# wang-xinyu/tensorrtx

Hardware: NVIDIA B200
Metric: end_to_end_fps_yolov8n_640_b32 (pre-process + fused decode + NMS); decode+NMS us/frame alongside (higher is better)
Workload: dtype f32

## Files before the change

include/trtx_hot.h:

```cpp
#ifndef TRTX_HOT_H
#define TRTX_HOT_H

#include <stddef.h>
#include <stdint.h>

#ifdef __cplusplus
extern "C" {
#endif

#if defined(_WIN32)
#define TRTX_API __declspec(dllexport)
#else
#define TRTX_API __attribute__((visibility("default")))
#endif

typedef void* trtx_stream_t;

enum {
    TRTX_OK = 0,
    TRTX_ERR_INVALID = 1,
    TRTX_ERR_WORKSPACE = 2,
    TRTX_ERR_CUDA = 3,
    TRTX_ERR_UNSUPPORTED = 4,
};

#define TRTX_MAX_LEVELS 8

TRTX_API const char* trtx_version(void);
TRTX_API int trtx_last_cuda_error(void);
TRTX_API size_t trtx_abi_sizeof(int which);

enum {
    TRTX_YOLO_V8 = 0,
    TRTX_YOLO_V5 = 1,
    TRTX_YOLO_V3 = 2,
    TRTX_YOLO_V26 = 3,
};
enum { TRTX_F32 = 0, TRTX_F16 = 1 };

typedef struct trtx_yolo_params {
    int32_t variant;
    int32_t num_classes;
    int32_t net_w;
    int32_t net_h;
    int32_t max_out;
    int32_t det_floats;
    int32_t num_levels;
    int32_t grid_h[TRTX_MAX_LEVELS];
    int32_t grid_w[TRTX_MAX_LEVELS];
    int32_t strides[TRTX_MAX_LEVELS];
    float anchors[TRTX_MAX_LEVELS][6];
    int32_t is_seg;
    int32_t is_pose;
    int32_t is_obb;
    int32_t num_kpts;
    float kpt_thresh;
    float gate;
    int32_t in_dtype;
    int32_t tune_class_slices;
    int32_t tune_rows_in_flight;
    int32_t tune_tma_pipeline;
    int32_t tune_tma_stages;
    int32_t tune_box_prefetch;
} trtx_yolo_params;

TRTX_API int trtx_yolo_params_init_v8(trtx_yolo_params* p, int num_classes, int net_w, int net_h, int max_out,
                                      const int* strides, int num_levels);

TRTX_API size_t trtx_yolo_workspace_size(const trtx_yolo_params* p, int batch);

TRTX_API int trtx_yolo_decode_enqueue(const trtx_yolo_params* p, int batch, const void* const* inputs_dev,
                                      float* output_dev, void* workspace_dev, size_t workspace_bytes,
                                      trtx_stream_t stream);

enum {
    TRTX_BOX_LTRB = 0,
    TRTX_BOX_CXCYWH = 1,
    TRTX_BOX_RETINA = 2,
    TRTX_BOX_OBB = 3,
};
enum {
    TRTX_NMS_GREEDY = 0,
    TRTX_NMS_ONESHOT = 1,
};

#define TRTX_NMS_MAX_ROWS 2048

typedef struct trtx_nms_params {
    int32_t box_format;
    int32_t mode;
    float conf_thresh;
    float nms_thresh;
    int32_t max_det;
    int32_t class_aware;
    int32_t tie_break_x0;
    int32_t extra_floats;
    int32_t extra_offset;
} trtx_nms_params;


TRTX_API size_t trtx_nms_workspace_size(const trtx_nms_params* p, int batch, int max_rows);
TRTX_API int trtx_nms_enqueue(const trtx_nms_params* p, int batch, const float* plugin_out_dev, int max_rows,
                              int det_floats, float* compact_out_dev, int32_t* keep_index_dev, void* workspace_dev,
                              size_t workspace_bytes, trtx_stream_t stream);

TRTX_API int trtx_yolo_decode_nms_enqueue(const trtx_yolo_params* p, const trtx_nms_params* q, int batch,
                                          const void* const* inputs_dev, float* compact_out_dev,
                                          int32_t* keep_index_dev, void* workspace_dev, size_t workspace_bytes,
                                          trtx_stream_t stream);

TRTX_API int trtx_yolo_scan_enqueue(const trtx_yolo_params* p, int batch, const void* const* inputs_dev,
                                    void* workspace_dev, size_t workspace_bytes, trtx_stream_t stream);
TRTX_API int trtx_yolo_nms_after_scan_enqueue(const trtx_yolo_params* p, const trtx_nms_params* q, int batch,
                                              const void* const* inputs_dev, float* compact_out_dev,
                                              int32_t* keep_index_dev, void* workspace_dev, size_t workspace_bytes,
                                              trtx_stream_t stream);

typedef struct trtx_gather {
    int32_t world, rank, slots, slot;
    float* out_dev[8];
    uint32_t* flags_dev[8];
    uint32_t* ctrl_dev;
} trtx_gather;
TRTX_API int trtx_yolo_decode_nms_gather_enqueue(const trtx_yolo_params* p, const trtx_nms_params* q, int batch,
                                                 const void* const* inputs_dev, float* compact_out_dev,
                                                 int32_t* keep_index_dev, void* workspace_dev, size_t workspace_bytes,
                                                 const trtx_gather* gather, trtx_stream_t stream);
TRTX_API int trtx_gather_push_enqueue(const trtx_gather* gather, const float* compact_out_dev, int batch, int max_det,
                                      int extra_floats, trtx_stream_t stream);
TRTX_API int trtx_gather_wait_enqueue(const trtx_gather* gather, trtx_stream_t stream);
TRTX_API int trtx_gather_push_many_enqueue(const trtx_gather* gather, const float* const* compact_outs_dev, int n, int batch,
                                           int max_det, int extra_floats, trtx_stream_t stream);
TRTX_API int trtx_gather_wait_many_enqueue(const trtx_gather* gather, int nslots, trtx_stream_t stream);
TRTX_API int trtx_peer_alloc(size_t bytes, void** dev_ptr, unsigned char handle[64]);
TRTX_API int trtx_peer_open(const unsigned char handle[64], void** dev_ptr);
TRTX_API int trtx_peer_close(void* dev_ptr);
TRTX_API int trtx_peer_free(void* dev_ptr);

enum {
    TRTX_RETINA_FACE = 0,
    TRTX_RETINA_ANTICOV = 1,
};
typedef struct trtx_retina_params {
    int32_t in_h, in_w;
    float gate;
    int32_t variant;
} trtx_retina_params;

TRTX_API int trtx_retina_total_priors(const trtx_retina_params* p);
TRTX_API size_t trtx_retina_workspace_size(const trtx_retina_params* p, int batch);
TRTX_API int trtx_retina_decode_enqueue(const trtx_retina_params* p, int batch, const void* const* inputs_dev,
                                        float* output_dev, void* workspace_dev, size_t workspace_bytes,
                                        trtx_stream_t stream);

TRTX_API int64_t trtx_rpn_decode(int batch, const float* scores_dev, const float* deltas_dev, float* out_scores_dev,
                                 float* out_boxes_dev, int height, int width, int image_height, int image_width,
                                 float stride, const float* anchors_host, int num_anchors, int top_n,
                                 void* workspace_dev, size_t workspace_bytes, trtx_stream_t stream);
TRTX_API int64_t trtx_rpn_nms(int batch, const float* scores_dev, const float* boxes_dev, float* out_boxes_dev,
                              int pre_nms_topk, int post_nms_topk, float nms_thresh, void* workspace_dev,
                              size_t workspace_bytes, trtx_stream_t stream);
TRTX_API int64_t trtx_predictor_decode(int batch, const float* scores_dev, const float* deltas_dev,
                                       const float* proposals_dev, float* out_scores_dev, float* out_boxes_dev,
                                       float* out_classes_dev, int num_boxes, int num_classes, int image_height,
                                       int image_width, const float* bbox_reg_weights_host, void* workspace_dev,
                                       size_t workspace_bytes, trtx_stream_t stream);
TRTX_API int64_t trtx_batched_nms(int nms_method, int batch, const float* scores_dev, const float* boxes_dev,
                                  const float* classes_dev, float* out_scores_dev, float* out_boxes_dev,
                                  float* out_classes_dev, int count, int detections_per_im, float nms_thresh,
                                  void* workspace_dev, size_t workspace_bytes, trtx_stream_t stream);

typedef struct trtx_image_desc {
    const uint8_t* data_dev;
    int32_t width, height;
    int32_t pitch;
    int32_t reserved;
} trtx_image_desc;

TRTX_API int trtx_preprocess_batch_enqueue(const trtx_image_desc* images_host, int batch, void* dst_dev, int dst_w,
                                           int dst_h, int out_dtype, trtx_stream_t stream);
TRTX_API void trtx_letterbox_matrix(int src_w, int src_h, int dst_w, int dst_h, float d2s[6]);
TRTX_API int trtx_get_rect(int variant, int net_w, int net_h, int img_w, int img_h, const float bbox[4], int rect[4]);

TRTX_API int trtx_get_rect_adapt_landmark(int net_w, int net_h, int img_w, int img_h, const float bbox[4], float* lmk,
                                          int num_kpts, int rect[4]);
TRTX_API int trtx_retina_get_rect_adapt_landmark(int input_w, int input_h, int img_w, int img_h, const float bbox[4], float lmk[10],
                                                 int rect[4]);
TRTX_API int trtx_process_decode_ptr_host(const float* decode_ptr_host, int bbox_element, int count, float* rows_out);
TRTX_API int trtx_process_decode_ptr_host_obb(const float* decode_ptr_host, int bbox_element, int count, float* rows_out);
TRTX_API int trtx_scale_mask_rect(int net_w, int net_h, int img_w, int img_h, int rect[4]);
TRTX_API int trtx_scale_mask_enqueue(const float* masks_dev, int n, int net_w, int net_h, int img_w, int img_h, float* out_dev,
                                     trtx_stream_t stream);

TRTX_API int trtx_roi_align(int batch, const float* rois_dev, const float* features_dev, float* out_dev, int pooler_resolution,
                            float spatial_scale, int sampling_ratio, int num_proposals, int out_channels, int feature_h,
                            int feature_w, trtx_stream_t stream);
#define TRTX_ROI_WINDOW 0
#define TRTX_ROI_DIRECT 1
TRTX_API int trtx_roi_align_ex(int batch, const float* rois_dev, const float* features_dev, float* out_dev, int pooler_resolution,
                               float spatial_scale, int sampling_ratio, int num_proposals, int out_channels, int feature_h,
                               int feature_w, int mode, trtx_stream_t stream);
TRTX_API int trtx_mask_rcnn_inference(int batch, const float* indices_dev, const float* masks_dev, float* out_dev,
                                      int detections_per_im, int output_size, int num_classes, trtx_stream_t stream);

TRTX_API int trtx_calib_letterbox_rect(int src_w, int src_h, int net_w, int net_h, int rect[4]);
TRTX_API int trtx_calib_letterbox_host(const uint8_t* bgr, int src_w, int src_h, size_t src_pitch, int net_w, int net_h, float* out_chw);

typedef struct trtx_mask_params {
    int32_t variant;
    int32_t net_w, net_h;
    int32_t mask_w, mask_h;
    int32_t num_coeffs;
    int32_t row_floats;
    int32_t coeff_offset;
    int32_t max_masks;
} trtx_mask_params;

TRTX_API int trtx_process_mask_enqueue(const trtx_mask_params* p, int batch, const float* proto_dev, const float* dets_dev,
                                       int max_rows, float* masks_dev, trtx_stream_t stream);

#ifdef __cplusplus
}
#endif
#endif
```

tensorrtx_b200/_lib.py:

```python
from __future__ import annotations

import ctypes as C
import os
from pathlib import Path

MAX_LEVELS = 8

OK, ERR_INVALID, ERR_WORKSPACE, ERR_CUDA, ERR_UNSUPPORTED = range(5)
YOLO_V8, YOLO_V5, YOLO_V3, YOLO_V26 = 0, 1, 2, 3
F32, F16 = 0, 1
BOX_LTRB, BOX_CXCYWH, BOX_RETINA, BOX_OBB = 0, 1, 2, 3
NMS_GREEDY, NMS_ONESHOT = 0, 1
ROI_WINDOW, ROI_DIRECT = 0, 1
RETINA_FACE, RETINA_ANTICOV = 0, 1

_ERR = {1: "TRTX_ERR_INVALID", 2: "TRTX_ERR_WORKSPACE", 3: "TRTX_ERR_CUDA", 4: "TRTX_ERR_UNSUPPORTED"}


class TrtxError(RuntimeError):
    pass


class YoloParams(C.Structure):
    _fields_ = [
        ("variant", C.c_int32),
        ("num_classes", C.c_int32),
        ("net_w", C.c_int32),
        ("net_h", C.c_int32),
        ("max_out", C.c_int32),
        ("det_floats", C.c_int32),
        ("num_levels", C.c_int32),
        ("grid_h", C.c_int32 * MAX_LEVELS),
        ("grid_w", C.c_int32 * MAX_LEVELS),
        ("strides", C.c_int32 * MAX_LEVELS),
        ("anchors", (C.c_float * 6) * MAX_LEVELS),
        ("is_seg", C.c_int32),
        ("is_pose", C.c_int32),
        ("is_obb", C.c_int32),
        ("num_kpts", C.c_int32),
        ("kpt_thresh", C.c_float),
        ("gate", C.c_float),
        ("in_dtype", C.c_int32),
        ("tune_class_slices", C.c_int32),
        ("tune_rows_in_flight", C.c_int32),
        ("tune_tma_pipeline", C.c_int32),
        ("tune_tma_stages", C.c_int32),
        ("tune_box_prefetch", C.c_int32),
    ]


class NmsParams(C.Structure):
    _fields_ = [
        ("box_format", C.c_int32),
        ("mode", C.c_int32),
        ("conf_thresh", C.c_float),
        ("nms_thresh", C.c_float),
        ("max_det", C.c_int32),
        ("class_aware", C.c_int32),
        ("tie_break_x0", C.c_int32),
        ("extra_floats", C.c_int32),
        ("extra_offset", C.c_int32),
    ]


class Gather(C.Structure):
    _fields_ = [("world", C.c_int32), ("rank", C.c_int32), ("slots", C.c_int32), ("slot", C.c_int32),
                ("out_dev", C.c_void_p * 8), ("flags_dev", C.c_void_p * 8), ("ctrl_dev", C.c_void_p)]


class RetinaParams(C.Structure):
    _fields_ = [("in_h", C.c_int32), ("in_w", C.c_int32), ("gate", C.c_float), ("variant", C.c_int32)]


class ImageDesc(C.Structure):
    _fields_ = [
        ("data_dev", C.c_void_p),
        ("width", C.c_int32),
        ("height", C.c_int32),
        ("pitch", C.c_int32),
        ("reserved", C.c_int32),
    ]


class MaskParams(C.Structure):
    _fields_ = [(n, C.c_int32) for n in ("variant", "net_w", "net_h", "mask_w", "mask_h", "num_coeffs", "row_floats",
                                         "coeff_offset", "max_masks")]


LIB_PATH = Path(os.environ.get("TRTX_LIB") or Path(__file__).resolve().parent / "lib" / "libtrtx_hot.so")

_vp, _sz, _i, _f = C.c_void_p, C.c_size_t, C.c_int, C.c_float
_pp = C.POINTER(C.c_void_p)
SYMBOLS = {
    "trtx_version": (C.c_char_p, []),
    "trtx_last_cuda_error": (_i, []),
    "trtx_yolo_params_init_v8": (_i, [C.POINTER(YoloParams), _i, _i, _i, _i, C.POINTER(C.c_int), _i]),
    "trtx_yolo_workspace_size": (_sz, [C.POINTER(YoloParams), _i]),
    "trtx_yolo_decode_enqueue": (_i, [C.POINTER(YoloParams), _i, _pp, _vp, _vp, _sz, _vp]),
    "trtx_nms_workspace_size": (_sz, [C.POINTER(NmsParams), _i, _i]),
    "trtx_nms_enqueue": (_i, [C.POINTER(NmsParams), _i, _vp, _i, _i, _vp, _vp, _vp, _sz, _vp]),
    "trtx_yolo_decode_nms_enqueue": (_i, [C.POINTER(YoloParams), C.POINTER(NmsParams), _i, _pp, _vp, _vp, _vp, _sz, _vp]),
    "trtx_yolo_scan_enqueue": (_i, [C.POINTER(YoloParams), _i, _pp, _vp, _sz, _vp]),
    "trtx_yolo_nms_after_scan_enqueue": (_i, [C.POINTER(YoloParams), C.POINTER(NmsParams), _i, _pp, _vp, _vp, _vp, _sz, _vp]),
    "trtx_retina_total_priors": (_i, [C.POINTER(RetinaParams)]),
    "trtx_retina_workspace_size": (_sz, [C.POINTER(RetinaParams), _i]),
    "trtx_retina_decode_enqueue": (_i, [C.POINTER(RetinaParams), _i, _pp, _vp, _vp, _sz, _vp]),
    "trtx_rpn_decode": (C.c_int64, [_i, _vp, _vp, _vp, _vp, _i, _i, _i, _i, _f, C.POINTER(C.c_float), _i, _i, _vp, _sz, _vp]),
    "trtx_rpn_nms": (C.c_int64, [_i, _vp, _vp, _vp, _i, _i, _f, _vp, _sz, _vp]),
    "trtx_predictor_decode": (C.c_int64, [_i, _vp, _vp, _vp, _vp, _vp, _vp, _i, _i, _i, _i, C.POINTER(C.c_float), _vp, _sz, _vp]),
    "trtx_batched_nms": (C.c_int64, [_i, _i, _vp, _vp, _vp, _vp, _vp, _vp, _i, _i, _f, _vp, _sz, _vp]),
    "trtx_preprocess_batch_enqueue": (_i, [C.POINTER(ImageDesc), _i, _vp, _i, _i, _i, _vp]),
    "trtx_get_rect": (_i, [_i, _i, _i, _i, _i, C.POINTER(C.c_float), C.POINTER(C.c_int)]),
    "trtx_roi_align": (_i, [_i, _vp, _vp, _vp, _i, C.c_float, _i, _i, _i, _i, _i, _vp]),
    "trtx_calib_letterbox_rect": (_i, [_i, _i, _i, _i, C.POINTER(C.c_int)]),
    "trtx_calib_letterbox_host": (_i, [_vp, _i, _i, C.c_size_t, _i, _i, _vp]),
    "trtx_roi_align_ex": (_i, [_i, _vp, _vp, _vp, _i, C.c_float, _i, _i, _i, _i, _i, _i, _vp]),
    "trtx_mask_rcnn_inference": (_i, [_i, _vp, _vp, _vp, _i, _i, _i, _vp]),
    "trtx_process_mask_enqueue": (_i, [C.POINTER(MaskParams), _i, _vp, _vp, _i, _vp, _vp]),
    "trtx_letterbox_matrix": (None, [_i, _i, _i, _i, C.POINTER(C.c_float)]),
    "trtx_abi_sizeof": (_sz, [_i]),
    "trtx_get_rect_adapt_landmark": (_i, [_i, _i, _i, _i, C.POINTER(C.c_float), C.POINTER(C.c_float), _i, C.POINTER(C.c_int)]),
    "trtx_retina_get_rect_adapt_landmark": (_i, [_i, _i, _i, _i, C.POINTER(C.c_float), C.POINTER(C.c_float), C.POINTER(C.c_int)]),
    "trtx_process_decode_ptr_host": (_i, [C.POINTER(C.c_float), _i, _i, C.POINTER(C.c_float)]),
    "trtx_process_decode_ptr_host_obb": (_i, [C.POINTER(C.c_float), _i, _i, C.POINTER(C.c_float)]),
    "trtx_scale_mask_rect": (_i, [_i, _i, _i, _i, C.POINTER(C.c_int)]),
    "trtx_scale_mask_enqueue": (_i, [_vp, _i, _i, _i, _i, _i, _vp, _vp]),
    "trtx_yolo_decode_nms_gather_enqueue": (_i, [C.POINTER(YoloParams), C.POINTER(NmsParams), _i, _pp, _vp, _vp, _vp, _sz,
                                                 C.POINTER(Gather), _vp]),
    "trtx_gather_wait_enqueue": (_i, [C.POINTER(Gather), _vp]),
    "trtx_gather_push_enqueue": (_i, [C.POINTER(Gather), _vp, _i, _i, _i, _vp]),
    "trtx_gather_push_many_enqueue": (_i, [C.POINTER(Gather), _pp, _i, _i, _i, _i, _vp]),
    "trtx_gather_wait_many_enqueue": (_i, [C.POINTER(Gather), _i, _vp]),
    "trtx_peer_alloc": (_i, [_sz, C.POINTER(C.c_void_p), C.POINTER(C.c_ubyte)]),
    "trtx_peer_open": (_i, [C.POINTER(C.c_ubyte), C.POINTER(C.c_void_p)]),
    "trtx_peer_close": (_i, [_vp]),
    "trtx_peer_free": (_i, [_vp]),
}

_lib = None


def load() -> C.CDLL:
    global _lib
    if _lib is not None:
        return _lib
    if not LIB_PATH.exists():
        raise TrtxError(
            f"{LIB_PATH} is missing: build it with `python -m tensorrtx_b200.build` "
            "(or __graft_entry__.build()). There is no CPU/PyTorch fallback for this path."
        )
    lib = C.CDLL(str(LIB_PATH))
    for name, (res, args) in SYMBOLS.items():
        fn = getattr(lib, name)
        fn.restype = res
        fn.argtypes = args
    for which, st in enumerate((YoloParams, NmsParams, RetinaParams, ImageDesc, MaskParams)):
        if lib.trtx_abi_sizeof(which) != C.sizeof(st):
            raise TrtxError(f"{LIB_PATH} was built from a different trtx_hot.h: sizeof({st.__name__}) = "
                            f"{lib.trtx_abi_sizeof(which)} in the library, {C.sizeof(st)} in the binding (rebuild)")
    _lib = lib
    return lib


def check(rc: int, what: str) -> None:
    if rc != 0:
        extra = ""
        if rc == ERR_CUDA:
            extra = f" (cudaError {load().trtx_last_cuda_error()})"
        raise TrtxError(f"{what} failed: {_ERR.get(rc, rc)}{extra}")


def ptr_array(ptrs) -> "C.Array":
    arr = (C.c_void_p * len(ptrs))()
    for i, p in enumerate(ptrs):
        arr[i] = p
    return arr
```

tensorrtx_b200/csrc/common.cuh:

```cuda
#pragma once
#include <cuda_fp16.h>
#include <cuda_runtime.h>
#include <stdint.h>

#include "trtx_hot.h"

namespace trtx {

constexpr int kWarp = 32;
constexpr size_t kAlign = 256;

__host__ __device__ inline size_t align_up(size_t v, size_t a = kAlign) { return (v + a - 1) / a * a; }

extern thread_local int g_last_cuda_error;
inline int check_launch() {
    cudaError_t e = cudaGetLastError();
    if (e != cudaSuccess) {
        g_last_cuda_error = (int)e;
        return TRTX_ERR_CUDA;
    }
    return TRTX_OK;
}

__device__ __forceinline__ float4 ldg_stream_f4(const float* p) {
    float4 r;
    asm volatile("ld.global.nc.L1::no_allocate.v4.f32 {%0,%1,%2,%3}, [%4];"
                 : "=f"(r.x), "=f"(r.y), "=f"(r.z), "=f"(r.w)
                 : "l"(p));
    return r;
}
__device__ __forceinline__ float ldg_stream_f1(const float* p) {
    float r;
    asm volatile("ld.global.nc.L1::no_allocate.f32 %0, [%1];" : "=f"(r) : "l"(p));
    return r;
}
__device__ __forceinline__ float4 ldg_stream_h4(const __half* p) {
    uint32_t a, b;
    asm volatile("ld.global.nc.L1::no_allocate.v2.u32 {%0,%1}, [%2];" : "=r"(a), "=r"(b) : "l"(p));
    __half2 h0 = *reinterpret_cast<__half2*>(&a);
    __half2 h1 = *reinterpret_cast<__half2*>(&b);
    float2 f0 = __half22float2(h0), f1 = __half22float2(h1);
    return make_float4(f0.x, f0.y, f1.x, f1.y);
}
__device__ __forceinline__ uint4 ldg_stream_h8(const __half* p) {
    uint4 r;
    asm volatile("ld.global.nc.L1::no_allocate.v4.u32 {%0,%1,%2,%3}, [%4];" : "=r"(r.x), "=r"(r.y), "=r"(r.z), "=r"(r.w) : "l"(p));
    return r;
}
__device__ __forceinline__ float ldg_stream_h1(const __half* p) {
    unsigned short r;
    asm volatile("ld.global.nc.L1::no_allocate.u16 %0, [%1];" : "=h"(r) : "l"(p));
    return __half2float(__ushort_as_half(r));
}

template <typename T>
struct Elem;
template <>
struct Elem<float> {
    static __device__ __forceinline__ float4 ld4(const float* p) { return ldg_stream_f4(p); }
    static __device__ __forceinline__ float ld1(const float* p) { return ldg_stream_f1(p); }
    static __device__ __forceinline__ float ld1_cached(const float* p) { return __ldg(p); }
};
template <>
struct Elem<__half> {
    static __device__ __forceinline__ float4 ld4(const __half* p) { return ldg_stream_h4(p); }
    static __device__ __forceinline__ float ld1(const __half* p) { return ldg_stream_h1(p); }
    static __device__ __forceinline__ float ld1_cached(const __half* p) { return __half2float(__ldg(p)); }
};

__device__ __forceinline__ float logist(float x) { return 1.0f / (1.0f + expf(-x)); }

__device__ __forceinline__ uint32_t float_key(float f) {
    uint32_t b = __float_as_uint(f);
    return (b & 0x80000000u) ? ~b : (b | 0x80000000u);
}

__device__ __forceinline__ int warp_excl_scan(int v, int lane, int* total) {
    int x = v;
#pragma unroll
    for (int d = 1; d < 32; d <<= 1) {
        int y = __shfl_up_sync(0xffffffffu, x, d);
        if (lane >= d) x += y;
    }
    *total = __shfl_sync(0xffffffffu, x, 31);
    return x - v;
}

}
```

tensorrtx_b200/csrc/nms.cu:

```cuda
#include <string.h>

#include "yolo_layout.cuh"

namespace trtx {

#ifdef TRTX_NMS_PROBE
static thread_local long long* t_nms_stamps = nullptr;
#define TRTX_STAMP(k) do { if (a.dbg && threadIdx.x == 0) a.dbg[blockIdx.x * 16 + (k)] = clock64(); } while (0)
#else
#define TRTX_STAMP(k) do { } while (0)
#endif

constexpr int kNmsThreads = 1024;
constexpr int kMaxSort = TRTX_NMS_MAX_ROWS;
constexpr int kClassBins = kNmsThreads;
constexpr int kMaxBucket = 256;
constexpr int kShortSeg = 96;

struct NmsArgs {
    const float* rows;
    int max_rows;
    int det_floats;
    int from_tiles;
    int tiles_per_image, slots_per_image, tile_slots;
    int num_levels;
    int lv_tile_begin[TRTX_MAX_LEVELS];
    int lv_slot_begin[TRTX_MAX_LEVELS];
    const int* tile_count;
    const float4* cand;
    uint2* list;
    int list_stride;
    int box_format, mode, class_aware, tie_break_x0;
    float conf_thresh, nms_thresh;
    int pre_topk;
    int max_det;
    int extra_floats, extra_offset;
#ifdef TRTX_NMS_PROBE
    long long* dbg;
#endif
    float* out;
    int32_t* keep_index;
    struct Gather {
        float* out[8];
        unsigned* flags[8];
        unsigned* ctrl;
        int world, rank, slots, slot;
    } g;
};

__device__ __forceinline__ unsigned ld_relaxed_sys(const unsigned* p) {
    unsigned v;
    asm volatile("ld.relaxed.sys.global.u32 %0, [%1];" : "=r"(v) : "l"(p) : "memory");
    return v;
}
__device__ __forceinline__ void st_relaxed_sys(unsigned* p, unsigned v) {
    asm volatile("st.relaxed.sys.global.u32 [%0], %1;" ::"l"(p), "r"(v) : "memory");
}

__device__ __forceinline__ float iou_oneshot(const float4 a, const float4 b) {
    float cl = fmaxf(a.x, b.x), ct = fmaxf(a.y, b.y), cr = fminf(a.z, b.z), cb = fminf(a.w, b.w);
    float c_area = __fmul_rn(fmaxf(__fsub_rn(cr, cl), 0.0f), fmaxf(__fsub_rn(cb, ct), 0.0f));
    if (c_area == 0.0f) return 0.0f;
    float a_area = __fmul_rn(fmaxf(0.0f, __fsub_rn(a.z, a.x)), fmaxf(0.0f, __fsub_rn(a.w, a.y)));
    float b_area = __fmul_rn(fmaxf(0.0f, __fsub_rn(b.z, b.x)), fmaxf(0.0f, __fsub_rn(b.w, b.y)));
    return __fdiv_rn(c_area, __fsub_rn(__fadd_rn(a_area, b_area), c_area));
}
__device__ __forceinline__ void obb_cov_host(float w, float h, float r, float& a, float& b, float& c) {
    const float A = (float)((double)__fmul_rn(w, w) / 12.0), B = (float)((double)__fmul_rn(h, h) / 12.0);
    const float cr = cosf(r), sr = sinf(r);
    const float cr2 = __fmul_rn(cr, cr), sr2 = __fmul_rn(sr, sr);
    a = __fadd_rn(__fmul_rn(A, cr2), __fmul_rn(B, sr2));
    b = __fadd_rn(__fmul_rn(A, sr2), __fmul_rn(B, cr2));
    c = __fmul_rn(__fmul_rn(__fsub_rn(A, B), cr), sr);
}
__device__ __forceinline__ float obb_probiou_host(const float4 p1, float c1, const float4 p2, float c2) {
    const float eps = 1e-7;
    const float x1 = p1.x, y1 = p1.y, a1 = p1.z, b1 = p1.w, x2 = p2.x, y2 = p2.y, a2 = p2.z, b2 = p2.w;
    const float sa = __fadd_rn(a1, a2), sb = __fadd_rn(b1, b2), sc = __fadd_rn(c1, c2);
    const double dy = (double)__fsub_rn(y1, y2), dx = (double)__fsub_rn(x1, x2), dc = (double)sc;
    const double py = __dmul_rn(dy, dy), px = __dmul_rn(dx, dx), pc = __dmul_rn(dc, dc);
    const double den = __dadd_rn(__dsub_rn((double)__fmul_rn(sa, sb), pc), (double)eps);
    const float t1 = (float)__ddiv_rn(__dadd_rn(__dmul_rn((double)sa, py), __dmul_rn((double)sb, px)), den);
    const float t2 = (float)__ddiv_rn((double)__fmul_rn(__fmul_rn(sc, __fsub_rn(x2, x1)), __fsub_rn(y1, y2)), den);
    const float s1 = sqrtf(fmaxf(__fsub_rn(__fmul_rn(a1, b1), __fmul_rn(c1, c1)), 0.0f));
    const float s2 = sqrtf(fmaxf(__fsub_rn(__fmul_rn(a2, b2), __fmul_rn(c2, c2)), 0.0f));
    const float d3 = __fadd_rn(__fmul_rn(__fmul_rn(4.0f, s1), s2), eps);
    const float t3 = (float)log(__dadd_rn(__ddiv_rn(__dsub_rn((double)__fmul_rn(sa, sb), pc), (double)d3), (double)eps));
    float bd = __fadd_rn(__fadd_rn(__fmul_rn(0.25f, t1), __fmul_rn(0.5f, t2)), __fmul_rn(0.5f, t3));
    bd = fmaxf(fminf(bd, 100.0f), eps);
    const float hd = (float)sqrt(__dadd_rn(__dsub_rn(1.0, (double)expf(-bd)), (double)eps));
    return __fsub_rn(1.0f, hd);
}
__device__ __forceinline__ void obb_cov_dev(float w, float h, float r, float& a, float& b, float& c) {
    float a_val = w * w / 12.0f;
    float b_val = h * h / 12.0f;
    float cos_r = cosf(r);
    float sin_r = sinf(r);
    a = a_val * cos_r * cos_r + b_val * sin_r * sin_r;
    b = a_val * sin_r * sin_r + b_val * cos_r * cos_r;
    c = (a_val - b_val) * sin_r * cos_r;
}
__device__ __forceinline__ float obb_probiou_dev(const float4 p1, float c1, const float4 p2, float c2) {
    const float eps = 1e-7;
    const float cx1 = p1.x, cy1 = p1.y, a1 = p1.z, b1 = p1.w, cx2 = p2.x, cy2 = p2.y, a2 = p2.z, b2 = p2.w;
    float t1 = ((a1 + a2) * powf(cy1 - cy2, 2) + (b1 + b2) * powf(cx1 - cx2, 2)) /
               ((a1 + a2) * (b1 + b2) - powf(c1 + c2, 2) + eps);
    float t2 = ((c1 + c2) * (cx2 - cx1) * (cy1 - cy2)) / ((a1 + a2) * (b1 + b2) - powf(c1 + c2, 2) + eps);
    float t3 = logf(((a1 + a2) * (b1 + b2) - powf(c1 + c2, 2)) /
                            (4 * sqrtf(fmaxf(a1 * b1 - c1 * c1, 0.0f)) * sqrtf(fmaxf(a2 * b2 - c2 * c2, 0.0f)) + eps) +
                    eps);
    float bd = 0.25f * t1 + 0.5f * t2 + 0.5f * t3;
    bd = fmaxf(fminf(bd, 100.0f), eps);
    float hd = sqrtf(1.0f - expf(-bd) + eps);
    return 1 - hd;
}

__device__ __forceinline__ float4 to_corners(int fmt, const float4 b) {
    if (fmt != TRTX_BOX_CXCYWH) return b;
    const float hw = __fmul_rn(b.z, 0.5f), hh = __fmul_rn(b.w, 0.5f);
    return make_float4(__fsub_rn(b.x, hw), __fsub_rn(b.y, hh), __fadd_rn(b.x, hw), __fadd_rn(b.y, hh));
}
__device__ __forceinline__ float box_area(int fmt, const float4 b) {
    if (fmt == TRTX_BOX_CXCYWH) return __fmul_rn(b.z, b.w);
    return __fmul_rn(__fsub_rn(b.z, b.x), __fsub_rn(b.w, b.y));
}
struct IouTest {
    float thr;
    bool obb;
    bool retina;
    bool zero_hit;
    bool fast_ok;
};
__device__ __forceinline__ bool overlaps(const IouTest& q, const float4 l, float la, const float4 r, float ra) {
    if (q.obb) return obb_probiou_host(l, la, r, ra) >= q.thr;
    const float ib0 = l.x < r.x ? r.x : l.x;
    const float ib1 = r.z < l.z ? r.z : l.z;
    const float ib2 = l.y < r.y ? r.y : l.y;
    const float ib3 = r.w < l.w ? r.w : l.w;
    if (ib2 > ib3 || ib0 > ib1) return q.zero_hit;
    const float inter = __fmul_rn(__fsub_rn(ib1, ib0), __fsub_rn(ib3, ib2));
    float denom = __fsub_rn(__fadd_rn(la, ra), inter);
    if (q.retina) denom = __fadd_rn(denom, 0.000001f);
    const float t = __fmaf_rn(-q.thr, denom, inter);
    if (q.fast_ok && denom > 0.0f && fabsf(t) > __fmul_rn(1e-5f, denom)) return t > 0.0f;
    return __fdiv_rn(inter, denom) > q.thr;
}

struct Row {
    float4 box;
    float conf;
    float cls;
    int anchor;
};
__device__ __forceinline__ Row fetch_row(const NmsArgs& a, int b, uint32_t id) {
    Row r;
    if (a.from_tiles) {
        const float4* c = a.cand + 2 * ((size_t)b * a.slots_per_image + id);
        r.box = c[0];
        float4 m = c[1];
        r.conf = m.x;
        r.cls = m.y;
        r.anchor = __float_as_int(m.z);
    } else {
        const float* p = a.rows + (size_t)b * (1 + (size_t)a.max_rows * a.det_floats) + 1 + (size_t)id * a.det_floats;
        r.box = make_float4(p[0], p[1], p[2], p[3]);
        r.conf = p[4];
        r.cls = a.box_format == TRTX_BOX_RETINA ? 0.0f : p[5];
        r.anchor = (int)id;
    }
    return r;
}

__device__ __forceinline__ void pick_bucket(const int* hist, bool descending, int* need_io, int* bucket_out) {
    int need = *need_io, c = 0, d;
    if (descending) {
        for (d = 255; d > 0; --d) {
            if (c + hist[d] >= need) break;
            c += hist[d];
        }
    } else {
        for (d = 0; d < 255; ++d) {
            if (c + hist[d] >= need) break;
            c += hist[d];
        }
    }
    *need_io = need - c;
    *bucket_out = d;
}

__device__ __forceinline__ int seg_units(int m) {
    const int G = (m + 6) >> 3;
    return G * (m - 1) - 4 * G * (G - 1);
}

__global__ void __launch_bounds__(kNmsThreads, 1) nms_kernel(const __grid_constant__ NmsArgs a) {
    extern __shared__ __align__(16) unsigned char smem_raw[];
    const int S = a.pre_topk <= 1024 ? 1024 : kMaxSort;
    float4* u_box = reinterpret_cast<float4*>(smem_raw);
    float4* s_box = u_box + S;
    unsigned long long* k64 = reinterpret_cast<unsigned long long*>(s_box + S);
    float* u_conf = reinterpret_cast<float*>(k64 + S);
    int* u_cls = reinterpret_cast<int*>(u_conf + S);
    uint32_t* u_id = reinterpret_cast<uint32_t*>(u_cls + S);
    float* s_conf = reinterpret_cast<float*>(u_id + S);
    int* s_cls = reinterpret_cast<int*>(s_conf + S);
    uint32_t* s_id = reinterpret_cast<uint32_t*>(s_cls + S);
    int* s_seg = reinterpret_cast<int*>(s_id + S);
    int* s_long = s_seg + S;
    unsigned short* s_pos = reinterpret_cast<unsigned short*>(s_long + S / 2);
    unsigned char* s_keep = reinterpret_cast<unsigned char*>(s_pos + S);
    unsigned short* s_unit = reinterpret_cast<unsigned short*>(s_keep + S);
    float* s_area = reinterpret_cast<float*>(s_unit + S * (kShortSeg / 8));
    int* s_tpre = reinterpret_cast<int*>(s_area + S);
    unsigned short* s_krow = reinterpret_cast<unsigned short*>(u_box);
    unsigned* s_mask = reinterpret_cast<unsigned*>(u_conf);
    int* s_rowseg = reinterpret_cast<int*>(k64);
    unsigned long long* k_hi = reinterpret_cast<unsigned long long*>(s_box);
    unsigned long long* k_lo = k_hi + S;

    __shared__ int s_hist[256];
    __shared__ int s_chist[kClassBins], s_cstart[kClassBins];
    __shared__ int s_n, s_need, s_bucket, s_nkept, s_nshort, s_nmed, s_nlong, s_cursor, s_bad, s_nunit;
    __shared__ unsigned s_rem;
    __shared__ unsigned s_sup[32];
    __shared__ int s_wsum[32];

    const int b = blockIdx.x;
    const int tid = threadIdx.x, lane = tid & 31, warp = tid >> 5;
    uint2* list = a.list + (size_t)b * a.list_stride;

    TRTX_STAMP(0);
    if (tid == 0) {
        s_n = 0;
        s_bad = 0;
    }
    auto stash = [&](const Row& r, uint32_t id) {
        const int pos = atomicAdd(&s_n, 1);
        list[pos] = make_uint2(float_key(r.conf), id);
        if (pos < S) {
            const int c = a.class_aware ? (int)r.cls : 0;
            u_box[pos] = r.box;
            u_conf[pos] = r.conf;
            u_cls[pos] = c;
            u_id[pos] = id;
            if (c < 0 || c > 0xffff) s_bad = 1;
        }
    };
    if (a.from_tiles) {
        const int T = a.tiles_per_image;
        const int* cnt = a.tile_count + (size_t)b * T;
        int carry = 0;
        for (int base = 0; base < T; base += kNmsThreads) {
            const int t = base + tid;
            const int v = t < T ? cnt[t] : 0;
            int tot;
            const int ex = warp_excl_scan(v, lane, &tot);
            if (lane == 0) s_wsum[warp] = tot;
            __syncthreads();
            if (warp == 0) {
                int w = s_wsum[lane], wt;
                const int wex = warp_excl_scan(w, lane, &wt);
                s_wsum[lane] = wex;
                if (lane == 0) s_need = wt;
            }
            __syncthreads();
            if (t < T) s_tpre[t] = carry + s_wsum[warp] + ex;
            carry += s_need;
            __syncthreads();
        }
        if (tid == 0) s_tpre[T] = carry;
        __syncthreads();
        const int n_in = min(carry, a.pre_topk);
        for (int r = tid; r < n_in; r += kNmsThreads) {
            int lo = 0, hi = T;
            while (hi - lo > 1) {
                const int mid = (lo + hi) >> 1;
                if (s_tpre[mid] <= r) lo = mid; else hi = mid;
            }
            const int t = lo;
            int l = 0;
            while (l + 1 < a.num_levels && t >= a.lv_tile_begin[l + 1]) ++l;
            const uint32_t id = a.lv_slot_begin[l] + (uint32_t)(t - a.lv_tile_begin[l]) * a.tile_slots + (uint32_t)(r - s_tpre[t]);
            const Row row = fetch_row(a, b, id);
            if (a.mode == TRTX_NMS_ONESHOT ? row.conf >= a.conf_thresh : row.conf > a.conf_thresh) stash(row, id);
        }
    } else {
        __syncthreads();
        const float* img = a.rows + (size_t)b * (1 + (size_t)a.max_rows * a.det_floats);
        int n_in = (int)img[0];
        n_in = max(0, min(n_in, a.max_rows));
        for (int i = tid; i < n_in; i += kNmsThreads) {
            const Row row = fetch_row(a, b, (uint32_t)i);
            if (a.mode == TRTX_NMS_ONESHOT ? row.conf >= a.conf_thresh : row.conf > a.conf_thresh) stash(row, (uint32_t)i);
        }
    }
    __syncthreads();
    const int n_valid = s_n;
    const int M = min(n_valid, a.pre_topk);

    if (n_valid > a.pre_topk) {
        uint32_t key_cut = 0, id_cut = 0xffffffffu;
        uint32_t prefix = 0, mask = 0;
        if (tid == 0) s_need = a.pre_topk;
        for (int pass = 0; pass < 4; ++pass) {
            const int shift = 24 - 8 * pass;
            if (tid < 256) s_hist[tid] = 0;
            __syncthreads();
            for (int i = tid; i < n_valid; i += kNmsThreads) {
                uint32_t k = list[i].x;
                if ((k & mask) == prefix) atomicAdd(&s_hist[(k >> shift) & 255], 1);
            }
            __syncthreads();
            if (tid == 0) {
                int need = s_need, d;
                pick_bucket(s_hist, true, &need, &d);
                s_need = need;
                s_bucket = d;
            }
            __syncthreads();
            prefix |= (uint32_t)s_bucket << shift;
            mask |= 255u << shift;
        }
        key_cut = prefix;
        const int need_eq = s_need;
        uint32_t ip = 0, im = 0;
        __syncthreads();
        if (tid == 0) s_need = need_eq;
        for (int pass = 0; pass < 4; ++pass) {
            const int shift = 24 - 8 * pass;
            if (tid < 256) s_hist[tid] = 0;
            __syncthreads();
            for (int i = tid; i < n_valid; i += kNmsThreads) {
                uint2 e = list[i];
                if (e.x == key_cut && (e.y & im) == ip) atomicAdd(&s_hist[(e.y >> shift) & 255], 1);
            }
            __syncthreads();
            if (tid == 0) {
                int need = s_need, d;
                pick_bucket(s_hist, false, &need, &d);
                s_need = need;
                s_bucket = d;
            }
            __syncthreads();
            ip |= (uint32_t)s_bucket << shift;
            im |= 255u << shift;
        }
        id_cut = ip;
        if (tid == 0) {
            s_n = 0;
            s_bad = 0;
        }
        __syncthreads();
        for (int i = tid; i < n_valid; i += kNmsThreads) {
            const uint2 e = list[i];
            if (e.x > key_cut || (e.x == key_cut && e.y <= id_cut)) {
                const Row r = fetch_row(a, b, e.y);
                const int pos = atomicAdd(&s_n, 1);
                const int c = a.class_aware ? (int)r.cls : 0;
                u_box[pos] = r.box;
                u_conf[pos] = r.conf;
                u_cls[pos] = c;
                u_id[pos] = e.y;
                if (c < 0 || c > 0xffff) s_bad = 1;
            }
        }
        __syncthreads();
    }

    TRTX_STAMP(1);
    int S_eff = 32;
    while (S_eff < M) S_eff <<= 1;
    bool generic = s_bad != 0;
    bool bucketed = false;
    if (!generic) {
        unsigned long long* kb = reinterpret_cast<unsigned long long*>(s_box);
        s_chist[tid] = 0;
        __syncthreads();
        bool big = false;
        for (int base = 0; base < M; base += kNmsThreads) {
            const int i = base + tid;
            const int c = i < M ? u_cls[i] : -1;
            const unsigned peers = __match_any_sync(0xffffffffu, c);
            const int leader = __ffs(peers) - 1;
            int first = 0;
            if (c >= kClassBins) big = true;
            if (lane == leader && c >= 0 && c < kClassBins) first = atomicAdd(&s_chist[c], __popc(peers));
            first = __shfl_sync(0xffffffffu, first, leader);
            if (i < M) s_pos[i] = (unsigned short)(first + __popc(peers & ((1u << lane) - 1u)));
        }
        __syncthreads();
        const int h = s_chist[tid];
        int tot;
        const int ex = warp_excl_scan(h, lane, &tot);
        if (lane == 0) s_wsum[warp] = tot;
        if (!__syncthreads_or(big || h > kMaxBucket ? 1 : 0)) {
            if (warp == 0) {
                int w = s_wsum[lane], wt;
                const int wex = warp_excl_scan(w, lane, &wt);
                s_wsum[lane] = wex;
            }
            __syncthreads();
            s_cstart[tid] = s_wsum[warp] + ex;
            __syncthreads();
            for (int i = tid; i < M; i += kNmsThreads) {
                const int c = u_cls[i];
                kb[s_cstart[c] + s_pos[i]] =
                    ((unsigned long long)(uint32_t)c << 48) | ((unsigned long long)(uint32_t)(~float_key(u_conf[i])) << 16) | (uint32_t)i;
            }
            __syncthreads();
            for (int p = tid; p < M; p += kNmsThreads) {
                const unsigned long long mk = kb[p];
                const int c = (int)(mk >> 48);
                const int s0 = s_cstart[c], m = s_chist[c];
                int rank = 0;
#pragma unroll 4
                for (int k = 0; k < m; ++k) rank += kb[s0 + k] < mk ? 1 : 0;
                k64[s0 + rank] = mk;
            }
            __syncthreads();
            bool tie = false;
            for (int i = tid; i < M; i += kNmsThreads)
                if (i > 0 && (k64[i] >> 16) == (k64[i - 1] >> 16)) tie = true;
            generic = __syncthreads_or(tie ? 1 : 0) != 0;
            bucketed = !generic;
        }
    }
    if (!generic && !bucketed) {
        for (int i = tid; i < S_eff; i += kNmsThreads)
            k64[i] = i < M ? ((unsigned long long)(uint32_t)u_cls[i] << 48) | ((unsigned long long)(uint32_t)(~float_key(u_conf[i])) << 16) | (uint32_t)i
                           : ~0ull;
        __syncthreads();
        if (S_eff <= kNmsThreads) {
            unsigned long long* ex = reinterpret_cast<unsigned long long*>(s_box);
            unsigned long long mk = tid < S_eff ? k64[tid] : ~0ull;
            int pp = 0;
            for (int k = 2; k <= S_eff; k <<= 1) {
                for (int jj = k >> 1; jj > 0; jj >>= 1) {
                    unsigned long long ok;
                    if (jj >= 32) {
                        ex[pp * kNmsThreads + tid] = mk;
                        __syncthreads();
                        ok = ex[pp * kNmsThreads + (tid ^ jj)];
                        pp ^= 1;
                    } else {
                        ok = __shfl_xor_sync(0xffffffffu, mk, jj);
                    }
                    const bool want_min = (((tid & k) == 0) == ((tid & jj) == 0));
                    if (want_min == (ok < mk)) mk = ok;
                }
            }
            __syncthreads();
            if (tid < S_eff) k64[tid] = mk;
            __syncthreads();
        } else {
            for (int k = 2; k <= S_eff; k <<= 1) {
                for (int jj = k >> 1; jj > 0; jj >>= 1) {
                    for (int i = tid; i < S_eff; i += kNmsThreads) {
                        const int ixj = i ^ jj;
                        if (ixj > i) {
                            const unsigned long long x = k64[i], y = k64[ixj];
                            if ((x > y) == ((i & k) == 0)) {
                                k64[i] = y;
                                k64[ixj] = x;
                            }
                        }
                    }
                    __syncthreads();
                }
            }
        }
        bool tie = false;
        for (int i = tid; i < M; i += kNmsThreads)
            if (i > 0 && (k64[i] >> 16) == (k64[i - 1] >> 16)) tie = true;
        generic = __syncthreads_or(tie ? 1 : 0) != 0;
    }
    if (generic) {
        for (int i = tid; i < S_eff; i += kNmsThreads) {
            if (i < M) {
                k_hi[i] = ((unsigned long long)(uint32_t)u_cls[i] << 32) | (uint32_t)(~float_key(u_conf[i]));
                k_lo[i] = ((unsigned long long)(a.tie_break_x0 ? float_key(u_box[i].x) : 0u) << 32) | u_id[i];
            } else {
                k_hi[i] = ~0ull;
                k_lo[i] = ~0ull;
            }
            s_pos[i] = (unsigned short)i;
        }
        __syncthreads();
        for (int k = 2; k <= S_eff; k <<= 1) {
            for (int jj = k >> 1; jj > 0; jj >>= 1) {
                for (int i = tid; i < S_eff; i += kNmsThreads) {
                    const int ixj = i ^ jj;
                    if (ixj > i) {
                        const unsigned long long ah = k_hi[i], al = k_lo[i], bh = k_hi[ixj], bl = k_lo[ixj];
                        const bool gt = ah > bh || (ah == bh && al > bl);
                        if (gt == ((i & k) == 0)) {
                            k_hi[i] = bh;
                            k_lo[i] = bl;
                            k_hi[ixj] = ah;
                            k_lo[ixj] = al;
                            const unsigned short t0 = s_pos[i];
                            s_pos[i] = s_pos[ixj];
                            s_pos[ixj] = t0;
                        }
                    }
                }
                __syncthreads();
            }
        }
        for (int i = tid; i < M; i += kNmsThreads) k64[i] = s_pos[i];
        __syncthreads();
    }

    TRTX_STAMP(2);
    const bool greedy = a.mode == TRTX_NMS_GREEDY;
    IouTest iq;
    iq.thr = a.nms_thresh;
    iq.obb = a.box_format == TRTX_BOX_OBB;
    iq.retina = a.box_format == TRTX_BOX_RETINA;
    iq.zero_hit = 0.0f > a.nms_thresh;
    iq.fast_ok = fabsf(a.nms_thresh) <= 4.0f;
    for (int i = tid; i < M; i += kNmsThreads) {
        const int pos = (int)(k64[i] & 0xffffull);
        const float4 bx = u_box[pos];
        if (a.box_format == TRTX_BOX_OBB) {
            const float ang = a.rows[(size_t)b * (1 + (size_t)a.max_rows * a.det_floats) + 1 + (size_t)u_id[pos] * a.det_floats +
                                     a.extra_offset];
            float ca, cb, cc;
            if (greedy)
                obb_cov_host(bx.z, bx.w, ang, ca, cb, cc);
            else
                obb_cov_dev(bx.z, bx.w, ang, ca, cb, cc);
            s_box[i] = make_float4(bx.x, bx.y, ca, cb);
            s_area[i] = cc;
        } else if (greedy) {
            s_box[i] = to_corners(a.box_format, bx);
            s_area[i] = box_area(a.box_format, bx);
        } else {
            s_box[i] = bx;
        }
        s_conf[i] = u_conf[pos];
        s_cls[i] = u_cls[pos];
        s_id[i] = u_id[pos];
        s_keep[i] = 0;
    }
    if (tid == 0) {
        s_nkept = 0;
        s_rem = 0;
        s_nshort = 0;
        s_nmed = 0;
        s_nlong = 0;
        s_cursor = 0;
        s_nunit = 0;
    }
    __syncthreads();
    TRTX_STAMP(8);

    const int R = 7 + a.extra_floats;
    float* o = a.out + (size_t)b * (1 + (size_t)a.max_det * R);
    int32_t* oidx = a.keep_index ? a.keep_index + (size_t)b * a.max_det : nullptr;
    const int gworld = a.g.world;
    const size_t goff = gworld ? ((size_t)a.g.slot * gworld * gridDim.x + (size_t)a.g.rank * gridDim.x + b) * (1 + (size_t)a.max_det * R) : 0;

    if (greedy) {
        if (bucketed) {
            for (int i = tid; i < M; i += kNmsThreads) {
                const int c = s_cls[i], m = s_chist[c];
                s_rowseg[i] = m > kShortSeg ? 0 : ((s_cstart[c] << 16) | m);
            }
            const int m = s_chist[tid], p0 = s_cstart[tid];
            if (m > kShortSeg)
                s_long[atomicAdd(&s_nlong, 1)] = (p0 << 16) | m;
            else if (m > 32)
                s_seg[S - 1 - atomicAdd(&s_nmed, 1)] = (p0 << 16) | m;
            else if (m > 0)
                s_seg[atomicAdd(&s_nshort, 1)] = (p0 << 16) | m;
            if (m > 1 && m <= kShortSeg) s_pos[p0] = (unsigned short)atomicAdd(&s_nunit, seg_units(m));
        } else
        for (int i = tid; i < M; i += kNmsThreads) {
            if (i == 0 || s_cls[i] != s_cls[i - 1]) {
                int e = i + 1;
                while (e < M && s_cls[e] == s_cls[i]) ++e;
                const int m = e - i;
                for (int r = i; r < e; ++r) s_rowseg[r] = m > kShortSeg ? 0 : ((i << 16) | m);
                if (m > kShortSeg)
                    s_long[atomicAdd(&s_nlong, 1)] = (i << 16) | m;
                else if (m > 32)
                    s_seg[S - 1 - atomicAdd(&s_nmed, 1)] = (i << 16) | m;
                else
                    s_seg[atomicAdd(&s_nshort, 1)] = (i << 16) | m;
                if (m > 1 && m <= kShortSeg) s_pos[i] = (unsigned short)atomicAdd(&s_nunit, seg_units(m));
            }
        }
        __syncthreads();
        TRTX_STAMP(3);
        const int n_long = s_nlong;
        for (int ls = 0; ls < n_long; ++ls) {
            const int p0 = s_long[ls] >> 16, m = s_long[ls] & 0xffff;
            int n_kept = 0;
            for (int c0 = 0; c0 < m; c0 += 32) {
                const int nchunk = min(32, m - c0);
                const int P = 32 * n_kept;
                for (int p = tid; p < P; p += kNmsThreads) {
                    const int i = p & 31, k = p >> 5;
                    const int kr = s_krow[k];
                    if (i < nchunk && overlaps(iq, s_box[kr], s_area[kr], s_box[p0 + c0 + i], s_area[p0 + c0 + i]))
                        atomicOr(&s_rem, 1u << i);
                }
                {
                    const int i = warp, jx = lane;
                    bool hit = false;
                    if (i < nchunk && jx < i)
                        hit = overlaps(iq, s_box[p0 + c0 + jx], s_area[p0 + c0 + jx], s_box[p0 + c0 + i], s_area[p0 + c0 + i]);
                    const unsigned mm = __ballot_sync(0xffffffffu, hit);
                    if (lane == 0) s_sup[i] = mm;
                }
                __syncthreads();
                if (warp == 0) {
                    const unsigned my = s_sup[lane];
                    unsigned alive = ~s_rem & (nchunk == 32 ? 0xffffffffu : ((1u << nchunk) - 1u));
                    for (unsigned rem = alive; rem != 0u;) {
                        const int jx = __ffs(rem) - 1;
                        const unsigned kill = __ballot_sync(0xffffffffu, (my >> jx) & 1u);
                        alive &= ~kill;
                        rem = alive & ~((2u << jx) - 1u);
                    }
                    if ((alive >> lane) & 1u) {
                        const int pos = n_kept + __popc(alive & ((1u << lane) - 1u));
                        s_krow[pos] = (unsigned short)(p0 + c0 + lane);
                        s_keep[p0 + c0 + lane] = 1;
                    }
                    if (lane == 0) {
                        s_nkept = n_kept + __popc(alive);
                        s_rem = 0;
                    }
                }
                __syncthreads();
                n_kept = s_nkept;
            }
        }
        TRTX_STAMP(4);
        for (int i = tid; i < M; i += kNmsThreads) {
            const int rs = s_rowseg[i];
            if (rs == 0) continue;
            const int p0 = rs >> 16, m = rs & 0xffff, li = i - p0;
#pragma unroll
            for (int w = 0; w < kShortSeg / 32; ++w) s_mask[i * (kShortSeg / 32) + w] = 0u;
            const int ub = s_pos[p0] + li - 1;
            for (int g = 0; g * 8 < li; ++g)
                s_unit[ub + g * (m - 1) - 4 * g * (g - 1) - 8 * g] = (unsigned short)((i << 4) | g);
        }
        __syncthreads();
        TRTX_STAMP(9);
        {
            const int n_unit = s_nunit;
            unsigned char* mask_bytes = reinterpret_cast<unsigned char*>(s_mask);
            for (int u = tid; u < n_unit; u += kNmsThreads) {
                const int e = s_unit[u], i = e >> 4, g = e & 15;
                const int p0 = s_rowseg[i] >> 16, li = i - p0;
                const float4 bi = s_box[i];
                const float ai = s_area[i];
                unsigned bits = 0u;
#pragma unroll
                for (int k = 0; k < 8; ++k) {
                    const int jx = g * 8 + k;
                    if (jx < li && overlaps(iq, s_box[p0 + jx], s_area[p0 + jx], bi, ai)) bits |= 1u << k;
                }
                mask_bytes[i * (kShortSeg / 8) + g] = (unsigned char)bits;
            }
        }
        __syncthreads();
        TRTX_STAMP(7);
        const int n_short = s_nshort, n_med = s_nmed;
        for (;;) {
            int sidx = 0;
            if (lane == 0) sidx = atomicAdd(&s_cursor, 1);
            sidx = __shfl_sync(0xffffffffu, sidx, 0);
            if (sidx >= n_med + n_short) break;
            const int ent = sidx < n_med ? s_seg[S - 1 - sidx] : s_seg[sidx - n_med];
            const int p0 = ent >> 16, m = ent & 0xffff;
            unsigned kept[kShortSeg / 32] = {0u, 0u, 0u};
#pragma unroll
            for (int c = 0; c < kShortSeg / 32; ++c) {
                if (c * 32 >= m) break;
                const int nchunk = min(32, m - c * 32);
                const bool in = lane < nchunk;
                const int row = p0 + c * 32 + lane;
                unsigned mw[kShortSeg / 32] = {0u, 0u, 0u};
                if (in) {
#pragma unroll
                    for (int w = 0; w <= c; ++w) mw[w] = s_mask[row * (kShortSeg / 32) + w];
                }
                bool removed = false;
#pragma unroll
                for (int w = 0; w < c; ++w) removed |= (mw[w] & kept[w]) != 0u;
                unsigned alive = __ballot_sync(0xffffffffu, in && !removed);
                const unsigned mymask = mw[c];
                for (unsigned rem = alive; rem != 0u;) {
                    const int jx = __ffs(rem) - 1;
                    const unsigned kill = __ballot_sync(0xffffffffu, (mymask >> jx) & 1u);
                    alive &= ~kill;
                    rem = alive & ~((2u << jx) - 1u);
                }
                kept[c] = alive;
                if ((alive >> lane) & 1u) s_keep[row] = 1;
            }
        }
        __syncthreads();
    } else {
        for (int i = tid; i < M; i += kNmsThreads) {
            const int ci = s_cls[i];
            const float4 bi = s_box[i];
            bool keep = true;
            for (int jx = i - 1; jx >= 0 && s_cls[jx] == ci; --jx) {
                if (iq.obb ? obb_probiou_dev(bi, s_area[i], s_box[jx], s_area[jx]) > a.nms_thresh
                           : iou_oneshot(bi, s_box[jx]) > a.nms_thresh) {
                    keep = false;
                    break;
                }
            }
            s_keep[i] = keep ? 1 : 0;
        }
        __syncthreads();
    }

    TRTX_STAMP(5);
    int carry = 0;
    for (int base = 0; base < M; base += kNmsThreads) {
        const int i = base + tid;
        const bool emit = i < M && (a.mode == TRTX_NMS_ONESHOT || s_keep[i]);
        const unsigned bal = __ballot_sync(0xffffffffu, emit);
        if (lane == 0) s_wsum[warp] = __popc(bal);
        __syncthreads();
        if (warp == 0) {
            int v = s_wsum[lane], tot;
            const int ex = warp_excl_scan(v, lane, &tot);
            s_wsum[lane] = ex;
            if (lane == 0) s_nkept = tot;
        }
        __syncthreads();
        const int k = carry + s_wsum[warp] + __popc(bal & ((1u << lane) - 1u));
        if (emit && k < a.max_det) {
            const float4 bx = a.box_format == TRTX_BOX_OBB || (greedy && a.box_format == TRTX_BOX_CXCYWH)
                                  ? fetch_row(a, b, s_id[i]).box
                                  : s_box[i];
            float* row = o + 1 + (size_t)k * R;
            row[0] = bx.x;
            row[1] = bx.y;
            row[2] = bx.z;
            row[3] = bx.w;
            row[4] = s_conf[i];
            row[5] = (float)s_cls[i];
            row[6] = s_keep[i] ? 1.0f : 0.0f;
            if (oidx) oidx[k] = a.from_tiles ? __float_as_int(a.cand[2 * ((size_t)b * a.slots_per_image + s_id[i]) + 1].z)
                                             : (int)s_id[i];
            if (a.extra_floats && !a.from_tiles) {
                const float* src = a.rows + (size_t)b * (1 + (size_t)a.max_rows * a.det_floats) + 1 +
                                   (size_t)s_id[i] * a.det_floats + a.extra_offset;
                for (int e = 0; e < a.extra_floats; ++e) row[7 + e] = src[e];
            }
        }
        carry += s_nkept;
        __syncthreads();
    }
    const int n_rows_out = min(carry, a.max_det);
    if (tid == 0) o[0] = (float)n_rows_out;
    for (int i = n_rows_out * R + tid; i < a.max_det * R; i += kNmsThreads) o[1 + i] = 0.0f;
    if (oidx)
        for (int i = n_rows_out + tid; i < a.max_det; i += kNmsThreads) oidx[i] = -1;
    if (gworld) {
        __syncthreads();
        const int live = 1 + n_rows_out * R;
        for (int p = 0; p < gworld; ++p) {
            float* dstp = a.g.out[p] + goff;
            for (int i = tid; i < live; i += kNmsThreads) dstp[i] = i == 0 ? (float)n_rows_out : o[i];
        }
        __syncthreads();
        if (tid == 0) {
            __threadfence();
            if (atomicAdd(&a.g.ctrl[1], 1u) == gridDim.x - 1) {
                a.g.ctrl[1] = 0u;
                __threadfence_system();
                const size_t fi = (size_t)a.g.rank * a.g.slots + a.g.slot;
                const unsigned v = *reinterpret_cast<volatile unsigned*>(a.g.flags[a.g.rank] + fi) + 1u;
                for (int p = 0; p < gworld; ++p) st_relaxed_sys(a.g.flags[p] + fi, v);
            }
        }
    }
    TRTX_STAMP(6);
}

__global__ void __launch_bounds__(64) gather_wait_kernel(NmsArgs::Gather g, int nslots) {
    const int lane = threadIdx.x;
    const unsigned* fl = g.flags[g.rank];
    bool ok = true;
    if (lane < g.world * nslots) {
        const int r = lane / nslots, sl = g.slot + lane - r * nslots;
        const unsigned expected = ld_relaxed_sys(fl + (size_t)g.rank * g.slots + sl);
        const unsigned* f = fl + (size_t)r * g.slots + sl;
        const long long t0 = clock64();
        while ((int)(ld_relaxed_sys(f) - expected) < 0) {
            __nanosleep(200);
            if (clock64() - t0 > 4000000000ll) {
                ok = false;
                break;
            }
        }
    }
    if (!ok) g.ctrl[2] = 1u;
}

struct PushSrc {
    const float* src[8];
    int n;
};
__global__ void __launch_bounds__(256) gather_copy_kernel(NmsArgs::Gather g, PushSrc ps, int batch, int cols, int max_det, int R) {
    const int tid = threadIdx.x;
    const int w = blockIdx.x;
    const int k = w / batch, b = w - k * batch;
    const float* src = ps.src[k] + (size_t)b * cols;
    const int n = min(max((int)src[0], 0), max_det);
    const int live = 1 + n * R;
    const size_t off = (((size_t)(g.slot + k) * g.world + g.rank) * batch + b) * cols;
    constexpr int U = 4;
    for (int i0 = tid; i0 < live; i0 += 256 * U) {
        float v[U];
#pragma unroll
        for (int u = 0; u < U; ++u) v[u] = (i0 + u * 256 < live) ? src[i0 + u * 256] : 0.0f;
        for (int p = 0; p < g.world; ++p) {
            float* dst = g.out[p] + off;
#pragma unroll
            for (int u = 0; u < U; ++u)
                if (i0 + u * 256 < live) dst[i0 + u * 256] = v[u];
        }
    }
}
__global__ void __launch_bounds__(64) gather_publish_kernel(NmsArgs::Gather g, int nslots) {
    const int lane = threadIdx.x;
    if (lane >= g.world * nslots) return;
    const int p = lane / nslots, k = lane - p * nslots;
    const size_t fi = (size_t)g.rank * g.slots + g.slot + k;
    const unsigned v = ld_relaxed_sys(g.flags[g.rank] + fi) + 1u;
    __syncwarp();
    __syncthreads();
    st_relaxed_sys(g.flags[p] + fi, v);
}

static size_t nms_smem_bytes(int pre_topk, int tiles = 0) {
    const size_t S = pre_topk <= 1024 ? 1024 : kMaxSort;
    return S * (16 + 16 + 8 + 6 * 4 + 4 + 2 + 2 + 1 + 2 * (kShortSeg / 8) + 4) + 64 + sizeof(int) * (size_t)(tiles + 1);
}

static int nms_validate(const trtx_nms_params* q) {
    if (!q) return TRTX_ERR_INVALID;
    if (q->box_format < 0 || q->box_format > TRTX_BOX_OBB) return TRTX_ERR_INVALID;
    if (q->box_format == TRTX_BOX_OBB && q->extra_floats < 1) return TRTX_ERR_INVALID;
    if (q->mode != TRTX_NMS_GREEDY && q->mode != TRTX_NMS_ONESHOT) return TRTX_ERR_INVALID;
    if (q->max_det <= 0 || q->extra_floats < 0 || q->extra_offset < 0) return TRTX_ERR_INVALID;
    return TRTX_OK;
}

static int nms_launch(NmsArgs& a, int batch, cudaStream_t st) {
#ifdef TRTX_NMS_PROBE
    a.dbg = t_nms_stamps;
#endif
    if (a.pre_topk > kMaxSort) return TRTX_ERR_UNSUPPORTED;
    const size_t smem = nms_smem_bytes(a.pre_topk, a.from_tiles ? a.tiles_per_image : 0);
    constexpr size_t kMaxDynSmem = (227 - 20) * 1024;
    if (smem > kMaxDynSmem) return TRTX_ERR_UNSUPPORTED;
    cudaFuncSetAttribute(nms_kernel, cudaFuncAttributeMaxDynamicSharedMemorySize, (int)kMaxDynSmem);
    nms_kernel<<<batch, kNmsThreads, smem, st>>>(a);
    return check_launch();
}

}

using namespace trtx;

extern "C" {

#ifdef TRTX_NMS_PROBE
TRTX_API int trtx_probe_set_nms_stamps(void* p) {
    t_nms_stamps = static_cast<long long*>(p);
    return TRTX_OK;
}
#endif

TRTX_API size_t trtx_nms_workspace_size(const trtx_nms_params* p, int batch, int max_rows) {
    if (nms_validate(p) || batch <= 0 || max_rows <= 0) return 0;
    return align_up(sizeof(uint2) * (size_t)batch * max_rows);
}

TRTX_API int trtx_nms_enqueue(const trtx_nms_params* p, int batch, const float* plugin_out_dev, int max_rows,
                              int det_floats, float* compact_out_dev, int32_t* keep_index_dev, void* workspace_dev,
                              size_t workspace_bytes, trtx_stream_t stream) {
    int rc = nms_validate(p);
    if (rc) return rc;
    if (batch <= 0 || max_rows <= 0 || det_floats < 5 || !plugin_out_dev || !compact_out_dev || !workspace_dev)
        return TRTX_ERR_INVALID;
    if (p->extra_floats && p->extra_offset + p->extra_floats > det_floats) return TRTX_ERR_INVALID;
    if (p->box_format != TRTX_BOX_RETINA && det_floats < 6) return TRTX_ERR_INVALID;
    if (workspace_bytes < trtx_nms_workspace_size(p, batch, max_rows)) return TRTX_ERR_WORKSPACE;
    NmsArgs a{};
    a.rows = plugin_out_dev;
    a.max_rows = max_rows;
    a.det_floats = det_floats;
    a.from_tiles = 0;
    a.list = static_cast<uint2*>(workspace_dev);
    a.list_stride = max_rows;
    a.box_format = p->box_format;
    a.mode = p->mode;
    a.class_aware = p->class_aware && p->box_format != TRTX_BOX_RETINA;
    a.tie_break_x0 = p->tie_break_x0;
    a.conf_thresh = p->conf_thresh;
    a.nms_thresh = p->nms_thresh;
    a.pre_topk = max_rows < kMaxSort ? max_rows : kMaxSort;
    a.max_det = p->max_det;
    a.extra_floats = p->extra_floats;
    a.extra_offset = p->extra_offset;
    a.out = compact_out_dev;
    a.keep_index = keep_index_dev;
    return nms_launch(a, batch, static_cast<cudaStream_t>(stream));
}

static int fill_gather(const trtx_gather* g, NmsArgs::Gather* o) {
    memset(o, 0, sizeof(*o));
    if (!g) return TRTX_OK;
    if (g->world < 1 || g->world > 8 || g->rank < 0 || g->rank >= g->world || g->slots < 1 || g->slot < 0 || g->slot >= g->slots ||
        !g->ctrl_dev)
        return TRTX_ERR_INVALID;
    for (int r = 0; r < g->world; ++r) {
        if (!g->out_dev[r] || !g->flags_dev[r]) return TRTX_ERR_INVALID;
        o->out[r] = g->out_dev[r];
        o->flags[r] = g->flags_dev[r];
    }
    o->ctrl = g->ctrl_dev;
    o->world = g->world;
    o->rank = g->rank;
    o->slots = g->slots;
    o->slot = g->slot;
    return TRTX_OK;
}

static int yolo_nms_tiles(const trtx_yolo_params* p, const trtx_nms_params* q, int batch, const YoloArgs& ya,
                          const YoloLayout& L, float* compact_out_dev, int32_t* keep_index_dev, void* workspace_dev,
                          cudaStream_t st, const trtx_gather* gather = nullptr) {
    if (q->box_format == TRTX_BOX_OBB) return TRTX_ERR_UNSUPPORTED;
    NmsArgs a{};
    a.from_tiles = 1;
    a.tiles_per_image = L.tiles_per_image;
    a.slots_per_image = L.slots_per_image;
    a.tile_slots = L.tile_cells * L.apc;
    a.num_levels = p->num_levels;
    for (int l = 0; l < p->num_levels; ++l) {
        a.lv_tile_begin[l] = L.level_tile_begin[l];
        a.lv_slot_begin[l] = L.level_slot_begin[l];
    }
    a.tile_count = ya.tile_count;
    a.cand = ya.cand;
    a.list = reinterpret_cast<uint2*>(static_cast<char*>(workspace_dev) + L.off_list);
    a.list_stride = L.slots_per_image;
    a.box_format = q->box_format;
    a.mode = q->mode;
    a.class_aware = q->class_aware;
    a.tie_break_x0 = q->tie_break_x0;
    a.conf_thresh = q->conf_thresh;
    a.nms_thresh = q->nms_thresh;
    a.pre_topk = p->max_out;
    a.max_det = q->max_det;
    a.out = compact_out_dev;
    a.keep_index = keep_index_dev;
    const int rc = fill_gather(gather, &a.g);
    if (rc) return rc;
    return nms_launch(a, batch, st);
}

TRTX_API int trtx_yolo_decode_nms_enqueue(const trtx_yolo_params* p, const trtx_nms_params* q, int batch,
                                          const void* const* inputs_dev, float* compact_out_dev,
                                          int32_t* keep_index_dev, void* workspace_dev, size_t workspace_bytes,
                                          trtx_stream_t stream) {
    int rc = nms_validate(q);
    if (rc) return rc;
    if (!compact_out_dev) return TRTX_ERR_INVALID;
    if (q->extra_floats) return TRTX_ERR_UNSUPPORTED;
    YoloArgs ya;
    YoloLayout L;
    rc = yolo_fill_args(p, batch, inputs_dev, workspace_dev, workspace_bytes, &ya, &L);
    if (rc) return rc;
    if (p->max_out > kMaxSort) return TRTX_ERR_UNSUPPORTED;
    cudaStream_t st = static_cast<cudaStream_t>(stream);
    rc = yolo_scan_launch(ya, L, p->in_dtype, batch, st);
    if (rc) return rc;
    return yolo_nms_tiles(p, q, batch, ya, L, compact_out_dev, keep_index_dev, workspace_dev, st);
}

TRTX_API int trtx_yolo_decode_nms_gather_enqueue(const trtx_yolo_params* p, const trtx_nms_params* q, int batch,
                                                 const void* const* inputs_dev, float* compact_out_dev, int32_t* keep_index_dev,
                                                 void* workspace_dev, size_t workspace_bytes, const trtx_gather* gather,
                                                 trtx_stream_t stream) {
    int rc = nms_validate(q);
    if (rc) return rc;
    if (!compact_out_dev || !gather) return TRTX_ERR_INVALID;
    if (q->extra_floats) return TRTX_ERR_UNSUPPORTED;
    YoloArgs ya;
    YoloLayout L;
    rc = yolo_fill_args(p, batch, inputs_dev, workspace_dev, workspace_bytes, &ya, &L);
    if (rc) return rc;
    if (p->max_out > kMaxSort) return TRTX_ERR_UNSUPPORTED;
    cudaStream_t st = static_cast<cudaStream_t>(stream);
    rc = yolo_scan_launch(ya, L, p->in_dtype, batch, st);
    if (rc) return rc;
    return yolo_nms_tiles(p, q, batch, ya, L, compact_out_dev, keep_index_dev, workspace_dev, st, gather);
}

TRTX_API int trtx_gather_wait_many_enqueue(const trtx_gather* gather, int nslots, trtx_stream_t stream) {
    NmsArgs::Gather g;
    int rc = fill_gather(gather, &g);
    if (rc || !gather) return rc ? rc : TRTX_ERR_INVALID;
    if (nslots < 1 || nslots > 8 || gather->slot + nslots > gather->slots) return TRTX_ERR_INVALID;
    gather_wait_kernel<<<1, 64, 0, static_cast<cudaStream_t>(stream)>>>(g, nslots);
    return check_launch();
}
TRTX_API int trtx_gather_wait_enqueue(const trtx_gather* gather, trtx_stream_t stream) {
    return trtx_gather_wait_many_enqueue(gather, 1, stream);
}

TRTX_API int trtx_gather_push_many_enqueue(const trtx_gather* gather, const float* const* compact_outs_dev, int n, int batch, int max_det,
                                           int extra_floats, trtx_stream_t stream) {
    NmsArgs::Gather g;
    int rc = fill_gather(gather, &g);
    if (rc || !gather || !compact_outs_dev || batch <= 0 || max_det <= 0 || extra_floats < 0) return rc ? rc : TRTX_ERR_INVALID;
    if (n < 1 || n > 8 || gather->slot + n > gather->slots) return TRTX_ERR_INVALID;
    PushSrc ps{};
    ps.n = n;
    for (int k = 0; k < n; ++k) {
        if (!compact_outs_dev[k]) return TRTX_ERR_INVALID;
        ps.src[k] = compact_outs_dev[k];
    }
    if (n * g.world > 64) return TRTX_ERR_UNSUPPORTED;
    const int R = 7 + extra_floats;
    const int work = n * batch;
    gather_copy_kernel<<<work, 256, 0, static_cast<cudaStream_t>(stream)>>>(g, ps, batch, 1 + max_det * R, max_det, R);
    gather_publish_kernel<<<1, 64, 0, static_cast<cudaStream_t>(stream)>>>(g, n);
    return check_launch();
}
TRTX_API int trtx_gather_push_enqueue(const trtx_gather* gather, const float* compact_out_dev, int batch, int max_det,
                                      int extra_floats, trtx_stream_t stream) {
    return trtx_gather_push_many_enqueue(gather, &compact_out_dev, 1, batch, max_det, extra_floats, stream);
}

TRTX_API int trtx_peer_alloc(size_t bytes, void** dev_ptr, unsigned char handle[64]) {
    if (!bytes || !dev_ptr || !handle) return TRTX_ERR_INVALID;
    static_assert(sizeof(cudaIpcMemHandle_t) == 64, "IPC handle size");
    void* p = nullptr;
    cudaError_t e = cudaMalloc(&p, bytes);
    if (e == cudaSuccess) e = cudaMemset(p, 0, bytes);
    cudaIpcMemHandle_t h;
    if (e == cudaSuccess) e = cudaIpcGetMemHandle(&h, p);
    if (e != cudaSuccess) {
        g_last_cuda_error = (int)e;
        if (p) cudaFree(p);
        return TRTX_ERR_CUDA;
    }
    memcpy(handle, &h, 64);
    *dev_ptr = p;
    return TRTX_OK;
}
TRTX_API int trtx_peer_open(const unsigned char handle[64], void** dev_ptr) {
    if (!handle || !dev_ptr) return TRTX_ERR_INVALID;
    cudaIpcMemHandle_t h;
    memcpy(&h, handle, 64);
    const cudaError_t e = cudaIpcOpenMemHandle(dev_ptr, h, cudaIpcMemLazyEnablePeerAccess);
    if (e != cudaSuccess) {
        g_last_cuda_error = (int)e;
        return TRTX_ERR_CUDA;
    }
    return TRTX_OK;
}
TRTX_API int trtx_peer_close(void* dev_ptr) { return cudaIpcCloseMemHandle(dev_ptr) == cudaSuccess ? TRTX_OK : TRTX_ERR_CUDA; }
TRTX_API int trtx_peer_free(void* dev_ptr) { return cudaFree(dev_ptr) == cudaSuccess ? TRTX_OK : TRTX_ERR_CUDA; }

TRTX_API int trtx_yolo_scan_enqueue(const trtx_yolo_params* p, int batch, const void* const* inputs_dev,
                                    void* workspace_dev, size_t workspace_bytes, trtx_stream_t stream) {
    YoloArgs ya;
    YoloLayout L;
    int rc = yolo_fill_args(p, batch, inputs_dev, workspace_dev, workspace_bytes, &ya, &L);
    if (rc) return rc;
    return yolo_scan_launch(ya, L, p->in_dtype, batch, static_cast<cudaStream_t>(stream));
}

TRTX_API int trtx_yolo_nms_after_scan_enqueue(const trtx_yolo_params* p, const trtx_nms_params* q, int batch,
                                              const void* const* inputs_dev, float* compact_out_dev,
                                              int32_t* keep_index_dev, void* workspace_dev, size_t workspace_bytes,
                                              trtx_stream_t stream) {
    int rc = nms_validate(q);
    if (rc) return rc;
    if (!compact_out_dev) return TRTX_ERR_INVALID;
    if (q->extra_floats) return TRTX_ERR_UNSUPPORTED;
    YoloArgs ya;
    YoloLayout L;
    rc = yolo_fill_args(p, batch, inputs_dev, workspace_dev, workspace_bytes, &ya, &L);
    if (rc) return rc;
    if (p->max_out > kMaxSort) return TRTX_ERR_UNSUPPORTED;
    return yolo_nms_tiles(p, q, batch, ya, L, compact_out_dev, keep_index_dev, workspace_dev,
                          static_cast<cudaStream_t>(stream));
}

}
```

tensorrtx_b200/csrc/preprocess.cu:

```cuda
#include <limits.h>
#include <math.h>
#include <string.h>

#include "tma.cuh"

namespace trtx {

constexpr int kMaxImagesPerLaunch = 128;

struct PreImage {
    const uint8_t* src;
    int sw, sh, pitch;
    int dst_idx;
    float m[6];
};
struct PreArgs {
    PreImage img[kMaxImagesPerLaunch];
    int dw, dh;
};

__device__ __forceinline__ float div255(float x) {
    const float r = 1.0f / 255.0f;
    const float q0 = __fmul_rn(x, r);
    return __fmaf_rn(__fmaf_rn(-255.0f, q0, x), r, q0);
}


__device__ __forceinline__ float u8_to_float_alu(uint32_t i) { return __uint_as_float(0x4B000000u | i) - 8388608.0f; }

constexpr int kRowsPerThread = 4;

template <typename OutT>
__global__ void __launch_bounds__(256, 8) letterbox_kernel(const __grid_constant__ PreArgs a, OutT* __restrict__ dst) {
    constexpr int R = kRowsPerThread;
    const int b = blockIdx.z;
    const PreImage& im = a.img[b];
    const int dx = blockIdx.x * blockDim.x + threadIdx.x;
    const int dy0 = (blockIdx.y * blockDim.y + threadIdx.y) * R;
    if (dx >= a.dw || dy0 >= a.dh) return;
    const size_t area = (size_t)a.dw * a.dh;
    OutT* base = dst + (size_t)im.dst_idx * 3 * area + (size_t)dy0 * a.dw + dx;
    const float cv = 128.0f;
    const uint8_t* __restrict__ img = im.src;
    const int sw = im.sw, sh = im.sh;

    const float src_x = im.m[0] * (float)dx + im.m[1] * (float)dy0 + im.m[2] + 0.5f;
    const bool x_out = src_x <= -1 || src_x >= sw;
    const int x_low = (int)floorf(src_x);
    const int x_high = x_low + 1;
    const float lx = src_x - (float)x_low, hx = 1 - lx;
    const bool xl = x_low >= 0, xh = x_high < sw;
    const float xm = im.m[3] * (float)dx;

    auto emit = [&](int r, float c0, float c1, float c2) {
        OutT* o = base + (size_t)r * a.dw;
        if constexpr (sizeof(OutT) == 4) {
            o[0] = div255(c2);
            o[area] = div255(c1);
            o[2 * area] = div255(c0);
        } else {
            o[0] = __float2half_rn(div255(c2));
            o[area] = __float2half_rn(div255(c1));
            o[2 * area] = __float2half_rn(div255(c0));
        }
    };

    float src_y[R];
    int y_low[R];
#pragma unroll
    for (int r = 0; r < R; ++r) {
        src_y[r] = xm + im.m[4] * (float)(dy0 + r) + im.m[5] + 0.5f;
        y_low[r] = (int)floorf(src_y[r]);
    }
    bool fast = dy0 + R <= a.dh && xl && xh && y_low[0] >= 0 && y_low[0] + R < sh;
#pragma unroll
    for (int r = 1; r < R; ++r) fast = fast && y_low[r] == y_low[0] + r;
    if (fast) {
        const uint8_t* p = img + (size_t)y_low[0] * (size_t)im.pitch + (uint32_t)x_low * 3u;
        float t[R + 1][6];
#pragma unroll
        for (int s = 0; s <= R; ++s) {
#pragma unroll
            for (int k = 0; k < 6; ++k) {
                const uint32_t v = __ldg(p + k);
                t[s][k] = ((s * 6 + k) & 1) ? u8_to_float_alu(v) : (float)v;
            }
            p += im.pitch;
        }
#pragma unroll
        for (int r = 0; r < R; ++r) {
            const float ly = src_y[r] - (float)y_low[r], hy = 1 - ly;
            const float w1 = hy * hx, w2 = hy * lx, w3 = ly * hx, w4 = ly * lx;
            emit(r, w1 * t[r][0] + w2 * t[r][3] + w3 * t[r + 1][0] + w4 * t[r + 1][3],
                 w1 * t[r][1] + w2 * t[r][4] + w3 * t[r + 1][1] + w4 * t[r + 1][4],
                 w1 * t[r][2] + w2 * t[r][5] + w3 * t[r + 1][2] + w4 * t[r + 1][5]);
        }
        return;
    }

    const uint32_t o1 = (uint32_t)min(max(x_low, 0), sw - 1) * 3u, o2 = (uint32_t)min(max(x_high, 0), sw - 1) * 3u;
#pragma unroll
    for (int r = 0; r < R; ++r) {
        if (dy0 + r >= a.dh) break;
        float c0 = cv, c1 = cv, c2 = cv;
        if (!(x_out || src_y[r] <= -1 || src_y[r] >= sh)) {
            const int y_high = y_low[r] + 1;
            const float ly = src_y[r] - (float)y_low[r], hy = 1 - ly;
            const float w1 = hy * hx, w2 = hy * lx, w3 = ly * hx, w4 = ly * lx;
            const bool r0ok = y_low[r] >= 0, r1ok = y_high < sh;
            const uint32_t row0 = (uint32_t)max(y_low[r], 0) * (uint32_t)im.pitch;
            const uint32_t row1 = (uint32_t)min(y_high, sh - 1) * (uint32_t)im.pitch;
            const bool k1 = r0ok && xl, k2 = r0ok && xh, k3 = r1ok && xl, k4 = r1ok && xh;
            const uint8_t* p1 = img + (row0 + o1);
            const uint8_t* p2 = img + (row0 + o2);
            const uint8_t* p3 = img + (row1 + o1);
            const uint8_t* p4 = img + (row1 + o2);
            float v1[3], v2[3], v3[3], v4[3];
#pragma unroll
            for (int k = 0; k < 3; ++k) {
                const float t1 = (float)(uint32_t)__ldg(p1 + k);
                const float t2 = (float)(uint32_t)__ldg(p2 + k);
                const float t3 = (float)(uint32_t)__ldg(p3 + k);
                const float t4 = (float)(uint32_t)__ldg(p4 + k);
                v1[k] = k1 ? t1 : cv;
                v2[k] = k2 ? t2 : cv;
                v3[k] = k3 ? t3 : cv;
                v4[k] = k4 ? t4 : cv;
            }
            c0 = w1 * v1[0] + w2 * v2[0] + w3 * v3[0] + w4 * v4[0];
            c1 = w1 * v1[1] + w2 * v2[1] + w3 * v3[1] + w4 * v4[1];
            c2 = w1 * v1[2] + w2 * v2[2] + w3 * v3[2] + w4 * v4[2];
        }
        emit(r, c0, c1, c2);
    }
}


constexpr int kUnitTW = 64;
constexpr int kUnitBoxBytes = 208;
constexpr int kMaxUnitImages = 64;

struct UnitImage {
    int ox, oy;
    int sw, sh;
    int map, z;
    int dst_idx;
    float lx, ly;
};
struct alignas(64) UnitArgs {
    CUtensorMap map[kMaxUnitImages];
    UnitImage img[kMaxUnitImages];
    int dw, dh;
};

template <typename OutT, int WARPS>
__global__ void __launch_bounds__(WARPS * 32) letterbox_unit_kernel(const __grid_constant__ UnitArgs a, OutT* __restrict__ dst) {
    constexpr int TW = kUnitTW, TH = WARPS * 8, BOXW = kUnitBoxBytes, ROWS = TH + 1;
    __shared__ __align__(128) uint8_t box[ROWS * BOXW];
    __shared__ uint64_t bar;
    const int tid = threadIdx.x;
    const UnitImage& im = a.img[blockIdx.z];
    const int dx0 = blockIdx.x * TW, dy0 = blockIdx.y * TH;
    const int sx0 = dx0 + im.ox, sy0 = dy0 + im.oy;
    const int sw = im.sw, sh = im.sh;
    const bool all_out = sx0 + TW < 0 || sx0 >= sw || sy0 + TH < 0 || sy0 >= sh;
    const bool interior = sx0 >= 0 && sx0 + TW < sw && sy0 >= 0 && sy0 + TH < sh;

    if (tid == 0) {
        mbar_init(&bar, 1);
        mbar_fence_init();
    }
    __syncthreads();
    if (!all_out) {
        if (tid == 0) {
            mbar_arrive_expect_tx(&bar, ROWS * BOXW);
            tma_load_3d(box, &a.map[im.map], sx0 * 3, sy0, im.z, &bar);
        }
        mbar_wait(&bar, 0);
        if (!interior) {
            for (int i = tid; i < ROWS * (TW + 1); i += WARPS * 32) {
                const int r = i / (TW + 1), c = i - r * (TW + 1);
                const int y = sy0 + r, x = sx0 + c;
                if (y < 0 || y >= sh || x < 0 || x >= sw) {
                    uint8_t* q = box + r * BOXW + c * 3;
                    q[0] = 128;
                    q[1] = 128;
                    q[2] = 128;
                }
            }
            __syncthreads();
        }
    } else {
        for (int i = tid; i < ROWS * BOXW / 4; i += WARPS * 32) reinterpret_cast<uint32_t*>(box)[i] = 0x80808080u;
        __syncthreads();
    }

    const int lane = tid & 31, warp = tid >> 5;
    const int k = lane & 15;
    const int r0 = warp * 8 + (lane >> 4) * 4;
    const int dx = dx0 + 4 * k;
    if (dx >= a.dw) return;
    const float lx = im.lx, ly = im.ly, hx = 1 - lx, hy = 1 - ly;
    const float w1 = hy * hx, w2 = hy * lx, w3 = ly * hx, w4 = ly * lx;
    const size_t area = (size_t)a.dw * a.dh;
    OutT* o = dst + (size_t)im.dst_idx * 3 * area + (size_t)(dy0 + r0) * a.dw + dx;
    const uint8_t* p = box + r0 * BOXW + 12 * k;

    auto load_row = [&](const uint8_t* q, float (&t)[15]) {
        uint32_t w[4];
#pragma unroll
        for (int j = 0; j < 4; ++j) w[j] = reinterpret_cast<const uint32_t*>(q)[j];
#pragma unroll
        for (int i = 0; i < 15; ++i)
            t[i] = __uint_as_float(__byte_perm(w[i >> 2], 0x4B000000u, 0x7650u + (i & 3))) - 8388608.0f;
    };
    float top[15], bot[15];
    load_row(p, top);
    const int rows = a.dh - (dy0 + r0);
#pragma unroll
    for (int r = 0; r < 4; ++r) {
        load_row(p + (r + 1) * BOXW, bot);
        if (r < rows) {
            float v[3][4];
#pragma unroll
            for (int j = 0; j < 4; ++j)
#pragma unroll
                for (int c = 0; c < 3; ++c)
                    v[c][j] = div255(w1 * top[3 * j + c] + w2 * top[3 * j + 3 + c] + w3 * bot[3 * j + c] + w4 * bot[3 * j + 3 + c]);
            OutT* orow = o + (size_t)r * a.dw;
#pragma unroll
            for (int c = 0; c < 3; ++c) {
                OutT* q = orow + (size_t)(2 - c) * area;
                if constexpr (sizeof(OutT) == 4) {
                    *reinterpret_cast<float4*>(q) = make_float4(v[c][0], v[c][1], v[c][2], v[c][3]);
                } else {
                    const __half2 h0 = __floats2half2_rn(v[c][0], v[c][1]), h1 = __floats2half2_rn(v[c][2], v[c][3]);
                    uint2 u;
                    u.x = *reinterpret_cast<const uint32_t*>(&h0);
                    u.y = *reinterpret_cast<const uint32_t*>(&h1);
                    *reinterpret_cast<uint2*>(q) = u;
                }
            }
        }
#pragma unroll
        for (int i = 0; i < 15; ++i) top[i] = bot[i];
    }
}

static bool unit_scale_image(const trtx_image_desc& d, const float m[6], UnitImage* u) {
    if (!(m[0] == 1.0f && m[4] == 1.0f && m[1] == 0.0f && m[3] == 0.0f)) return false;
    const float tx = m[2] + 0.5f, ty = m[5] + 0.5f;
    if (!(fabsf(tx) < 1048576.0f && fabsf(ty) < 1048576.0f)) return false;
    if (2.0f * tx != rintf(2.0f * tx) || 2.0f * ty != rintf(2.0f * ty)) return false;
    if (reinterpret_cast<uintptr_t>(d.data_dev) % 16 != 0 || d.pitch % 16 != 0) return false;
    u->ox = (int)floorf(tx);
    u->oy = (int)floorf(ty);
    if (u->ox % 16 != 0) return false;
    u->lx = tx - floorf(tx);
    u->ly = ty - floorf(ty);
    u->sw = d.width;
    u->sh = d.height;
    return true;
}

static bool encode_image_map(CUtensorMap* map, const uint8_t* base, int sw, int sh, int pitch, int n, size_t image_stride,
                             int box_rows) {
    EncodeTiledFn enc = tma_encoder();
    if (!enc) return false;
    const cuuint64_t gdim[3] = {(cuuint64_t)sw * 3u, (cuuint64_t)sh, (cuuint64_t)n};
    const cuuint64_t gstr[2] = {(cuuint64_t)pitch, (cuuint64_t)image_stride};
    const cuuint32_t bdim[3] = {(cuuint32_t)kUnitBoxBytes, (cuuint32_t)box_rows, 1u};
    const cuuint32_t estr[3] = {1u, 1u, 1u};
    return enc(map, CU_TENSOR_MAP_DATA_TYPE_UINT8, 3, const_cast<uint8_t*>(base), gdim, gstr, bdim, estr,
               CU_TENSOR_MAP_INTERLEAVE_NONE, CU_TENSOR_MAP_SWIZZLE_NONE, CU_TENSOR_MAP_L2_PROMOTION_L2_128B,
               CU_TENSOR_MAP_FLOAT_OOB_FILL_NONE) == CUDA_SUCCESS;
}

constexpr int kUnitWarps = 4;

static int launch_unit(const trtx_image_desc* const* d, UnitImage* u, int n, void* dst, int dw, int dh, int out_dtype,
                       cudaStream_t st) {
    UnitArgs a;
    a.dw = dw;
    a.dh = dh;
    constexpr int box_rows = kUnitWarps * 8 + 1;
    bool uniform = n > 1;
    const ptrdiff_t step = n > 1 ? d[1]->data_dev - d[0]->data_dev : 0;
    for (int i = 1; i < n && uniform; ++i)
        uniform = d[i]->width == d[0]->width && d[i]->height == d[0]->height && d[i]->pitch == d[0]->pitch &&
                  d[i]->data_dev - d[i - 1]->data_dev == step;
    uniform = uniform && step > 0 && step % 16 == 0 && (size_t)step >= (size_t)d[0]->pitch * (size_t)d[0]->height;
    if (uniform) {
        if (!encode_image_map(&a.map[0], d[0]->data_dev, d[0]->width, d[0]->height, d[0]->pitch, n, (size_t)step, box_rows))
            return TRTX_ERR_UNSUPPORTED;
    }
    for (int i = 0; i < n; ++i) {
        if (uniform) {
            u[i].map = 0;
            u[i].z = i;
        } else {
            if (!encode_image_map(&a.map[i], d[i]->data_dev, d[i]->width, d[i]->height, d[i]->pitch, 1,
                                  (size_t)d[i]->pitch * (size_t)d[i]->height, box_rows))
                return TRTX_ERR_UNSUPPORTED;
            u[i].map = i;
            u[i].z = 0;
        }
        a.img[i] = u[i];
    }
    dim3 grid((dw + kUnitTW - 1) / kUnitTW, (dh + kUnitWarps * 8 - 1) / (kUnitWarps * 8), n);
    if (out_dtype == TRTX_F32)
        letterbox_unit_kernel<float, kUnitWarps><<<grid, kUnitWarps * 32, 0, st>>>(a, static_cast<float*>(dst));
    else
        letterbox_unit_kernel<__half, kUnitWarps><<<grid, kUnitWarps * 32, 0, st>>>(a, static_cast<__half*>(dst));
    return check_launch();
}

}

using namespace trtx;

extern "C" {

TRTX_API void trtx_letterbox_matrix(int sw, int sh, int dw, int dh, float d2s[6]) {
    float a = dh / (float)sh, b = dw / (float)sw;
    float scale = a < b ? a : b;
    float s2d[6];
    s2d[0] = scale;
    s2d[1] = 0;
    s2d[2] = (float)(-scale * sw * 0.5 + dw * 0.5);
    s2d[3] = 0;
    s2d[4] = scale;
    s2d[5] = (float)(-scale * sh * 0.5 + dh * 0.5);
    float p0 = s2d[0] * s2d[4], p1 = s2d[1] * s2d[3];
    float det = p0 - p1;
    double D = (double)det;
    D = D != 0 ? 1. / D : 0;
    float Df = (float)D;
    float fA11 = s2d[4] * Df, fA22 = s2d[0] * Df, fA12 = (-s2d[1]) * Df, fA21 = (-s2d[3]) * Df;
    double A11 = fA11, A22 = fA22, A12 = fA12, A21 = fA21;
    double b1 = -A11 * s2d[2] - A12 * s2d[5];
    double b2 = -A21 * s2d[2] - A22 * s2d[5];
    d2s[0] = (float)A11;
    d2s[1] = (float)A12;
    d2s[2] = (float)b1;
    d2s[3] = (float)A21;
    d2s[4] = (float)A22;
    d2s[5] = (float)b2;
}

TRTX_API int trtx_get_rect(int variant, int net_w, int net_h, int img_w, int img_h, const float bbox[4], int rect[4]) {
    if (!bbox || !rect || net_w <= 0 || net_h <= 0 || img_w <= 0 || img_h <= 0) return TRTX_ERR_INVALID;
    if (variant != TRTX_YOLO_V8 && variant != TRTX_YOLO_V5) return TRTX_ERR_INVALID;
    float l, r, t, b;
    const float r_w = (float)(net_w / (img_w * 1.0));
    const float r_h = (float)(net_h / (img_h * 1.0));
    const bool by_w = r_h > r_w;
    const float ratio = by_w ? r_w : r_h;
    const float pad = by_w ? (net_h - r_w * img_h) / 2 : (net_w - r_h * img_w) / 2;
    if (variant == TRTX_YOLO_V8) {
        l = bbox[0];
        r = bbox[2];
        t = bbox[1];
        b = bbox[3];
    } else {
        l = bbox[0] - bbox[2] / 2.f;
        r = bbox[0] + bbox[2] / 2.f;
        t = bbox[1] - bbox[3] / 2.f;
        b = bbox[1] + bbox[3] / 2.f;
    }
    if (by_w) {
        t = t - pad;
        b = b - pad;
    } else {
        l = l - pad;
        r = r - pad;
    }
    l = l / ratio;
    r = r / ratio;
    t = t / ratio;
    b = b / ratio;
    if (variant == TRTX_YOLO_V8) {
        l = 0.0f > l ? 0.0f : l;
        t = 0.0f > t ? 0.0f : t;
        const int rw = (int)round((double)(r - l)), rl = (int)round((double)l);
        const int rh = (int)round((double)(b - t)), rt = (int)round((double)t);
        const int width = rw < img_w - rl ? rw : img_w - rl, height = rh < img_h - rt ? rh : img_h - rt;
        rect[0] = rl;
        rect[1] = rt;
        rect[2] = width > 0 ? width : 0;
        rect[3] = height > 0 ? height : 0;
    } else {
        rect[0] = (int)round((double)l);
        rect[1] = (int)round((double)t);
        rect[2] = (int)round((double)(r - l));
        rect[3] = (int)round((double)(b - t));
    }
    return TRTX_OK;
}

TRTX_API int trtx_get_rect_adapt_landmark(int net_w, int net_h, int img_w, int img_h, const float bbox[4], float* lmk,
                                          int num_kpts, int rect[4]) {
    if (!bbox || !rect || (num_kpts > 0 && !lmk) || num_kpts < 0 || net_w <= 0 || net_h <= 0 || img_w <= 0 || img_h <= 0)
        return TRTX_ERR_INVALID;
    float l, r, t, b;
    const float r_w = (float)(net_w / (img_w * 1.0));
    const float r_h = (float)(net_h / (img_h * 1.0));
    if (r_h > r_w) {
        l = bbox[0] / r_w;
        r = bbox[2] / r_w;
        t = (bbox[1] - (net_h - r_w * img_h) / 2) / r_w;
        b = (bbox[3] - (net_h - r_w * img_h) / 2) / r_w;
        for (int i = 0; i < num_kpts * 3; i += 3) {
            lmk[i] /= r_w;
            lmk[i + 1] = (lmk[i + 1] - (net_h - r_w * img_h) / 2) / r_w;
        }
    } else {
        l = (bbox[0] - (net_w - r_h * img_w) / 2) / r_h;
        r = (bbox[2] - (net_w - r_h * img_w) / 2) / r_h;
        t = bbox[1] / r_h;
        b = bbox[3] / r_h;
        for (int i = 0; i < num_kpts * 3; i += 3) {
            lmk[i] = (lmk[i] - (net_w - r_h * img_w) / 2) / r_h;
            lmk[i + 1] /= r_h;
        }
    }
    l = 0.0f > l ? 0.0f : l;
    t = 0.0f > t ? 0.0f : t;
    const int rw = (int)round((double)(r - l)), rl = (int)round((double)l);
    const int rh = (int)round((double)(b - t)), rt = (int)round((double)t);
    const int width = rw < img_w - rl ? rw : img_w - rl, height = rh < img_h - rt ? rh : img_h - rt;
    rect[0] = rl;
    rect[1] = rt;
    rect[2] = width > 0 ? width : 0;
    rect[3] = height > 0 ? height : 0;
    return TRTX_OK;
}

TRTX_API int trtx_retina_get_rect_adapt_landmark(int input_w, int input_h, int img_w, int img_h, const float bbox[4], float lmk[10],
                                                 int rect[4]) {
    if (!bbox || !lmk || !rect || input_w <= 0 || input_h <= 0 || img_w <= 0 || img_h <= 0) return TRTX_ERR_INVALID;
    int l, r, t, b;
    float r_w = input_w / (img_w * 1.0);
    float r_h = input_h / (img_h * 1.0);
    if (r_h > r_w) {
        l = bbox[0] / r_w;
        r = bbox[2] / r_w;
        t = (bbox[1] - (input_h - r_w * img_h) / 2) / r_w;
        b = (bbox[3] - (input_h - r_w * img_h) / 2) / r_w;
        for (int i = 0; i < 10; i += 2) {
            lmk[i] /= r_w;
            lmk[i + 1] = (lmk[i + 1] - (input_h - r_w * img_h) / 2) / r_w;
        }
    } else {
        l = (bbox[0] - (input_w - r_h * img_w) / 2) / r_h;
        r = (bbox[2] - (input_w - r_h * img_w) / 2) / r_h;
        t = bbox[1] / r_h;
        b = bbox[3] / r_h;
        for (int i = 0; i < 10; i += 2) {
            lmk[i] = (lmk[i] - (input_w - r_h * img_w) / 2) / r_h;
            lmk[i + 1] /= r_h;
        }
    }
    rect[0] = l, rect[1] = t, rect[2] = r - l, rect[3] = b - t;
    return TRTX_OK;
}

TRTX_API int trtx_process_decode_ptr_host(const float* decode_ptr_host, int bbox_element, int count, float* rows_out) {
    if (!decode_ptr_host || !rows_out || bbox_element < 7 || count < 0) return -TRTX_ERR_INVALID;
    int n = 0;
    for (int i = 0; i < count; ++i) {
        const float* p = decode_ptr_host + 1 + (size_t)i * bbox_element;
        if ((int)p[6] == 1) {
            for (int k = 0; k < 6; ++k) rows_out[(size_t)n * 6 + k] = p[k];
            ++n;
        }
    }
    return n;
}

TRTX_API int trtx_process_decode_ptr_host_obb(const float* decode_ptr_host, int bbox_element, int count, float* rows_out) {
    if (!decode_ptr_host || !rows_out || bbox_element < 8 || count < 0) return -TRTX_ERR_INVALID;
    int n = 0;
    for (int i = 0; i < count; ++i) {
        const float* p = decode_ptr_host + 1 + (size_t)i * bbox_element;
        if ((int)p[6] == 1) {
            for (int k = 0; k < 6; ++k) rows_out[(size_t)n * 7 + k] = p[k];
            rows_out[(size_t)n * 7 + 6] = p[7];
            ++n;
        }
    }
    return n;
}

TRTX_API int trtx_preprocess_batch_enqueue(const trtx_image_desc* images_host, int batch, void* dst_dev, int dst_w,
                                           int dst_h, int out_dtype, trtx_stream_t stream) {
    if (!images_host || batch <= 0 || !dst_dev || dst_w <= 0 || dst_h <= 0) return TRTX_ERR_INVALID;
    if (out_dtype != TRTX_F32 && out_dtype != TRTX_F16) return TRTX_ERR_INVALID;
    cudaStream_t st = static_cast<cudaStream_t>(stream);
    for (int i = 0; i < batch; ++i) {
        const trtx_image_desc& d = images_host[i];
        if (!d.data_dev || d.width <= 0 || d.height <= 0 || d.pitch < 3 * d.width) return TRTX_ERR_INVALID;
    }
    const bool unit_ok = dst_w % 4 == 0 && reinterpret_cast<uintptr_t>(dst_dev) % 16 == 0;
    PreArgs g;
    g.dw = dst_w;
    g.dh = dst_h;
    int ng = 0;
    const trtx_image_desc* ud[kMaxUnitImages];
    UnitImage uu[kMaxUnitImages];
    int nu = 0;
    auto flush_general = [&]() -> int {
        if (!ng) return TRTX_OK;
        constexpr int R = kRowsPerThread;
        dim3 block(128, 2, 1);
        dim3 grid((dst_w + 127) / 128, (dst_h + 2 * R - 1) / (2 * R), ng);
        if (out_dtype == TRTX_F32)
            letterbox_kernel<float><<<grid, block, 0, st>>>(g, static_cast<float*>(dst_dev));
        else
            letterbox_kernel<__half><<<grid, block, 0, st>>>(g, static_cast<__half*>(dst_dev));
        ng = 0;
        return check_launch();
    };
    auto add_general = [&](int i) -> int {
        const trtx_image_desc& d = images_host[i];
        PreImage& im = g.img[ng++];
        im.src = d.data_dev;
        im.sw = d.width;
        im.sh = d.height;
        im.pitch = d.pitch;
        im.dst_idx = i;
        trtx_letterbox_matrix(d.width, d.height, dst_w, dst_h, im.m);
        return ng == kMaxImagesPerLaunch ? flush_general() : TRTX_OK;
    };
    auto flush_unit = [&]() -> int {
        if (!nu) return TRTX_OK;
        int rc = launch_unit(ud, uu, nu, dst_dev, dst_w, dst_h, out_dtype, st);
        if (rc == TRTX_ERR_UNSUPPORTED) {
            rc = TRTX_OK;
            for (int j = 0; j < nu && rc == TRTX_OK; ++j) rc = add_general(uu[j].dst_idx);
        }
        nu = 0;
        return rc;
    };
    for (int i = 0; i < batch; ++i) {
        const trtx_image_desc& d = images_host[i];
        float m[6];
        trtx_letterbox_matrix(d.width, d.height, dst_w, dst_h, m);
        int rc = TRTX_OK;
        if (unit_ok && unit_scale_image(d, m, &uu[nu])) {
            ud[nu] = &d;
            uu[nu].dst_idx = i;
            if (++nu == kMaxUnitImages) rc = flush_unit();
        } else {
            rc = add_general(i);
        }
        if (rc) return rc;
    }
    int rc = flush_unit();
    if (rc) return rc;
    return flush_general();
}

}
```

tensorrtx_b200/csrc/yolo_decode.cu:

```cuda
#include <math.h>

#include "yolo_layout.cuh"

namespace trtx {

thread_local int g_last_cuda_error = 0;

template <typename T, int VEC, int U>
__device__ __forceinline__ void scan_classes(const T* __restrict__ row0, size_t g, int nrows, int cls0, Best<VEC>& s) {
    const T* p = row0;
#pragma unroll 1
    for (int r = 0; r < nrows; r += U) {
        if constexpr (VEC == 4) {
            float4 v[U];
#pragma unroll
            for (int u = 0; u < U; ++u) {
                if (r + u < nrows)
                    v[u] = Elem<T>::ld4(p + (size_t)u * g);
                else
                    v[u] = make_float4(-INFINITY, -INFINITY, -INFINITY, -INFINITY);
            }
            float4 m = v[0];
#pragma unroll
            for (int u = 1; u < U; ++u) {
                m.x = fmaxf(m.x, v[u].x);
                m.y = fmaxf(m.y, v[u].y);
                m.z = fmaxf(m.z, v[u].z);
                m.w = fmaxf(m.w, v[u].w);
            }
#if defined(TRTX_SCAN_PROBE) && TRTX_SCAN_PROBE == 2
            if (true) {
                s.bx[0] = fmaxf(s.bx[0], m.x), s.bx[1] = fmaxf(s.bx[1], m.y), s.bx[2] = fmaxf(s.bx[2], m.z), s.bx[3] = fmaxf(s.bx[3], m.w);
                p += (size_t)U * g;
                continue;
            }
#endif
            if (!((m.x > s.bx[0]) | (m.y > s.bx[1]) | (m.z > s.bx[2]) | (m.w > s.bx[3]))) {
                p += (size_t)U * g;
                continue;
            }
            if (m.x > s.bx[0]) {
#pragma unroll
                for (int u = 0; u < U; ++u) update_one<VEC>(s, 0, v[u].x, cls0 + r + u);
            }
            if (m.y > s.bx[1]) {
#pragma unroll
                for (int u = 0; u < U; ++u) update_one<VEC>(s, 1, v[u].y, cls0 + r + u);
            }
            if (m.z > s.bx[2]) {
#pragma unroll
                for (int u = 0; u < U; ++u) update_one<VEC>(s, 2, v[u].z, cls0 + r + u);
            }
            if (m.w > s.bx[3]) {
#pragma unroll
                for (int u = 0; u < U; ++u) update_one<VEC>(s, 3, v[u].w, cls0 + r + u);
            }
        } else {
            float v[U];
#pragma unroll
            for (int u = 0; u < U; ++u) v[u] = (r + u < nrows) ? Elem<T>::ld1(p + (size_t)u * g) : -INFINITY;
            float m = v[0];
#pragma unroll
            for (int u = 1; u < U; ++u) m = fmaxf(m, v[u]);
            if (m > s.bx[0]) {
#pragma unroll
                for (int u = 0; u < U; ++u) update_one<VEC>(s, 0, v[u], cls0 + r + u);
            }
        }
        p += (size_t)U * g;
    }
}

__device__ __forceinline__ __half2 u32_as_h2(uint32_t u) { return *reinterpret_cast<__half2*>(&u); }

template <int U>
__device__ __forceinline__ void scan_classes_h8(const __half* __restrict__ row0, size_t g, int nrows, int cls0, Best<8>& s) {
    __half2 bxh[4];
#pragma unroll
    for (int k = 0; k < 4; ++k) bxh[k] = __halves2half2(__float2half_rd(s.bx[2 * k]), __float2half_rd(s.bx[2 * k + 1]));
    const __half* p = row0;
#pragma unroll 1
    for (int r = 0; r < nrows; r += U) {
        uint4 v[U];
#pragma unroll
        for (int u = 0; u < U; ++u) {
            if (r + u < nrows)
                v[u] = ldg_stream_h8(p + (size_t)u * g);
            else
                v[u] = make_uint4(0xFC00FC00u, 0xFC00FC00u, 0xFC00FC00u, 0xFC00FC00u);
        }
        __half2 m[4] = {u32_as_h2(v[0].x), u32_as_h2(v[0].y), u32_as_h2(v[0].z), u32_as_h2(v[0].w)};
#pragma unroll
        for (int u = 1; u < U; ++u) {
            m[0] = __hmax2(m[0], u32_as_h2(v[u].x));
            m[1] = __hmax2(m[1], u32_as_h2(v[u].y));
            m[2] = __hmax2(m[2], u32_as_h2(v[u].z));
            m[3] = __hmax2(m[3], u32_as_h2(v[u].w));
        }
        unsigned hit[4];
#pragma unroll
        for (int k = 0; k < 4; ++k) hit[k] = __hgt2_mask(m[k], bxh[k]);
        p += (size_t)U * g;
        if (!(hit[0] | hit[1] | hit[2] | hit[3])) continue;
#pragma unroll
        for (int k = 0; k < 4; ++k) {
            if (!hit[k]) continue;
            if (hit[k] & 0xffffu) {
#pragma unroll
                for (int u = 0; u < U; ++u) {
                    const uint32_t w = k == 0 ? v[u].x : (k == 1 ? v[u].y : (k == 2 ? v[u].z : v[u].w));
                    update_one<8>(s, 2 * k, __low2float(u32_as_h2(w)), cls0 + r + u);
                }
            }
            if (hit[k] >> 16) {
#pragma unroll
                for (int u = 0; u < U; ++u) {
                    const uint32_t w = k == 0 ? v[u].x : (k == 1 ? v[u].y : (k == 2 ? v[u].z : v[u].w));
                    update_one<8>(s, 2 * k + 1, __high2float(u32_as_h2(w)), cls0 + r + u);
                }
            }
            bxh[k] = __halves2half2(__float2half_rd(s.bx[2 * k]), __float2half_rd(s.bx[2 * k + 1]));
        }
    }
}

template <typename T, int VEC, int SLICES, int U>
__global__ void __launch_bounds__(32 * SLICES) yolo_v8_scan_kernel(const __grid_constant__ YoloArgs a) {
    constexpr int TILE = 32 * VEC;
    __shared__ float s_m[SLICES > 1 ? SLICES - 1 : 1][TILE];
    __shared__ float s_m2[SLICES > 1 ? SLICES - 1 : 1][TILE];
    __shared__ int s_c[SLICES > 1 ? SLICES - 1 : 1][TILE];

    const int b = blockIdx.x / a.tiles_per_image;
    const int t = blockIdx.x - b * a.tiles_per_image;
    int l = 0;
    while (l + 1 < a.num_levels && t >= a.lv[l + 1].tile_begin) ++l;
    const LevelArg& L = a.lv[l];
    const int tile = t - L.tile_begin;
    const int lane = threadIdx.x & 31;
    const int warp = threadIdx.x >> 5;
    const int a0 = tile * TILE + lane * VEC;
    const size_t g = (size_t)L.g;
    const bool active = a0 < L.g;
    const T* base = reinterpret_cast<const T*>(L.in) + (size_t)b * a.C * g;

    Best<VEC> s;
#pragma unroll
    for (int j = 0; j < VEC; ++j) {
        s.bx[j] = a.x_lo;
        s.b2[j] = a.x_lo;
        s.bc[j] = 0;
    }
    const int per = (a.nc + SLICES - 1) / SLICES;
    const int c0 = warp * per;
    const int c1 = min(a.nc, c0 + per);
    float d[4][VEC];
#pragma unroll
    for (int k = 0; k < 4; ++k)
#pragma unroll
        for (int j = 0; j < VEC; ++j) d[k][j] = 0.0f;
    auto load_box = [&]() {
#pragma unroll
        for (int k = 0; k < 4; ++k) {
            if constexpr (VEC == 8) {
                const uint4 v = ldg_stream_h8(reinterpret_cast<const __half*>(base) + (size_t)k * g + a0);
                const float2 f0 = __half22float2(u32_as_h2(v.x)), f1 = __half22float2(u32_as_h2(v.y));
                const float2 f2 = __half22float2(u32_as_h2(v.z)), f3 = __half22float2(u32_as_h2(v.w));
                d[k][0] = f0.x, d[k][1] = f0.y, d[k][2] = f1.x, d[k][3] = f1.y;
                d[k][4] = f2.x, d[k][5] = f2.y, d[k][6] = f3.x, d[k][7] = f3.y;
            } else if constexpr (VEC == 4) {
                float4 v = Elem<T>::ld4(base + (size_t)k * g + a0);
                d[k][0] = v.x;
                d[k][1] = v.y;
                d[k][2] = v.z;
                d[k][3] = v.w;
            } else {
                d[k][0] = Elem<T>::ld1(base + (size_t)k * g + a0);
            }
        }
    };
    if (warp == 0 && active) {
        if (a.prefetch_box == 3) {
            load_box();
        } else if (a.prefetch_box == 2) {
#pragma unroll
            for (int k = 0; k < 4; ++k) asm volatile("prefetch.global.L2 [%0];" ::"l"(base + (size_t)k * g + a0));
        }
    }
    if (active && c1 > c0) {
        if constexpr (VEC == 8)
            scan_classes_h8<U>(reinterpret_cast<const __half*>(base) + (size_t)(4 + c0) * g + a0, g, c1 - c0, c0, s);
        else
            scan_classes<T, VEC, U>(base + (size_t)(4 + c0) * g + a0, g, c1 - c0, c0, s);
    }

    if constexpr (SLICES > 1) {
        bool mine = false;
#pragma unroll
        for (int j = 0; j < VEC; ++j) mine |= s.bx[j] > a.x_lo || !(0.0f < a.gate);
        if (warp > 0) {
#pragma unroll
            for (int j = 0; j < VEC; ++j) {
                s_m[warp - 1][lane * VEC + j] = s.bx[j];
                s_m2[warp - 1][lane * VEC + j] = s.b2[j];
                s_c[warp - 1][lane * VEC + j] = s.bc[j];
            }
        }
        int any = __syncthreads_or(mine ? 1 : 0);
        if (!any) {
            if (threadIdx.x == 0) a.tile_count[(size_t)b * a.tiles_per_image + t] = 0;
            return;
        }
        if (warp > 0) return;
#pragma unroll
        for (int w = 1; w < SLICES; ++w) {
#pragma unroll
            for (int j = 0; j < VEC; ++j)
                merge_one<VEC>(s, j, s_m[w - 1][lane * VEC + j], s_m2[w - 1][lane * VEC + j], s_c[w - 1][lane * VEC + j]);
        }
    }

    float bp[VEC];
    unsigned flags = 0;
#pragma unroll
    for (int j = 0; j < VEC; ++j) {
        bp[j] = 0.0f;
        if (active && (a0 + j < L.g)) {
            if (s.bx[j] > a.x_lo) {
                const T* cls_row0 = base + (size_t)4 * g + a0 + j;
                bp[j] = finish_best(s.bx[j], s.b2[j], s.bc[j], a.gate, [&](int i) { return Elem<T>::ld1(cls_row0 + (size_t)i * g); });
            }
            if (!(bp[j] < a.gate)) flags |= 1u << j;
        }
    }
    int total;
    int off = warp_excl_scan(__popc(flags), lane, &total);
    if (lane == 0) a.tile_count[(size_t)b * a.tiles_per_image + t] = total;
#if defined(TRTX_SCAN_PROBE) && TRTX_SCAN_PROBE == 1
    flags = 0;
#endif
    if (flags) {
        if (a.prefetch_box != 3) load_box();
        const size_t slot0 = (size_t)b * a.slots_per_image + L.slot_begin + (size_t)tile * TILE;
        const float fs = (float)L.stride;
        const int row0 = a0 / L.gw, col0 = a0 - row0 * L.gw;
#pragma unroll
        for (int j = 0; j < VEC; ++j) {
            if (flags & (1u << j)) {
                const int e = a0 + j;
                int row = row0, col = col0 + j;
                while (col >= L.gw) {
                    col -= L.gw;
                    ++row;
                }
                float x1 = ((float)col + 0.5f - d[0][j]) * fs;
                float y1 = ((float)row + 0.5f - d[1][j]) * fs;
                float x2 = ((float)col + 0.5f + d[2][j]) * fs;
                float y2 = ((float)row + 0.5f + d[3][j]) * fs;
                store_record(a.cand, slot0 + off, x1, y1, x2, y2, bp[j], s.bc[j], L.slot_begin + e);
                ++off;
            }
        }
    }
}

template <typename T, int VEC, int U>
__global__ void __launch_bounds__(128) yolo_v5_scan_kernel(const __grid_constant__ YoloArgs a) {
    constexpr int TILE = 32 * VEC;
    constexpr int SLICES = 4;
    __shared__ float s_obj[3][TILE];
    __shared__ float s_m[SLICES - 1][TILE];
    __shared__ float s_m2[SLICES - 1][TILE];
    __shared__ int s_c[SLICES - 1][TILE];
    __shared__ float s_fp[3][TILE];
    __shared__ int s_fc[3][TILE];
    __shared__ int s_anyk[3];

    const int b = blockIdx.x / a.tiles_per_image;
    const int t = blockIdx.x - b * a.tiles_per_image;
    int l = 0;
    while (l + 1 < a.num_levels && t >= a.lv[l + 1].tile_begin) ++l;
    const LevelArg& L = a.lv[l];
    const int tile = t - L.tile_begin;
    const int lane = threadIdx.x & 31;
    const int warp = threadIdx.x >> 5;
    const int a0 = tile * TILE + lane * VEC;
    const size_t g = (size_t)L.g;
    const bool active = a0 < L.g;
    const int ilen = a.info_len;
    const T* base = reinterpret_cast<const T*>(L.in) + (size_t)b * a.C * g;

    if (threadIdx.x < 3) s_anyk[threadIdx.x] = 0;
    __syncthreads();
    if (warp < 3) {
        float x[VEC];
#pragma unroll
        for (int j = 0; j < VEC; ++j) x[j] = -INFINITY;
        if (active) {
            const T* p = base + ((size_t)warp * ilen + 4) * g + a0;
            if constexpr (VEC == 4) {
                float4 v = Elem<T>::ld4(p);
                x[0] = v.x;
                x[1] = v.y;
                x[2] = v.z;
                x[3] = v.w;
            } else {
                x[0] = Elem<T>::ld1(p);
            }
        }
        bool anyp = false;
#pragma unroll
        for (int j = 0; j < VEC; ++j) {
            float pr = 0.0f;
            bool pass = false;
            if (active && (a0 + j < L.g) && x[j] > a.x_lo) {
                pr = logist(x[j]);
                pass = !(pr < a.gate);
            }
            s_obj[warp][lane * VEC + j] = pass ? pr : -1.0f;
            anyp |= pass;
        }
        if (__any_sync(0xffffffffu, anyp) && lane == 0) s_anyk[warp] = 1;
    }
    __syncthreads();
    const int anyk0 = s_anyk[0], anyk1 = s_anyk[1], anyk2 = s_anyk[2];
    if (!(anyk0 | anyk1 | anyk2)) {
        if (threadIdx.x == 0) a.tile_count[(size_t)b * a.tiles_per_image + t] = 0;
        return;
    }
    const int per = (a.nc + SLICES - 1) / SLICES;
    const int c0 = warp * per;
    const int c1 = min(a.nc, c0 + per);
#pragma unroll 1
    for (int k = 0; k < 3; ++k) {
        const int anyk = k == 0 ? anyk0 : (k == 1 ? anyk1 : anyk2);
        if (!anyk) continue;
        Best<VEC> s;
#pragma unroll
        for (int j = 0; j < VEC; ++j) {
            s.bx[j] = (s_obj[k][lane * VEC + j] >= 0.0f) ? -INFINITY : INFINITY;
            s.b2[j] = s.bx[j];
            s.bc[j] = 0;
        }
        if (active && c1 > c0)
            scan_classes<T, VEC, U>(base + ((size_t)k * ilen + 5 + c0) * g + a0, g, c1 - c0, c0, s);
        if (warp > 0) {
#pragma unroll
            for (int j = 0; j < VEC; ++j) {
                s_m[warp - 1][lane * VEC + j] = s.bx[j];
                s_m2[warp - 1][lane * VEC + j] = s.b2[j];
                s_c[warp - 1][lane * VEC + j] = s.bc[j];
            }
        }
        __syncthreads();
        if (warp == 0) {
#pragma unroll
            for (int w = 1; w < SLICES; ++w) {
#pragma unroll
                for (int j = 0; j < VEC; ++j)
                    merge_one<VEC>(s, j, s_m[w - 1][lane * VEC + j], s_m2[w - 1][lane * VEC + j], s_c[w - 1][lane * VEC + j]);
            }
#pragma unroll
            for (int j = 0; j < VEC; ++j) {
                float P = 0.0f;
                if (s_obj[k][lane * VEC + j] >= 0.0f && s.bx[j] > -INFINITY) {
                    const T* cls_row0 = base + ((size_t)k * ilen + 5) * g + a0 + j;
                    P = finish_best(s.bx[j], s.b2[j], s.bc[j], 0.0f, [&](int i) { return Elem<T>::ld1(cls_row0 + (size_t)i * g); });
                }
                s_fp[k][lane * VEC + j] = P;
                s_fc[k][lane * VEC + j] = s.bc[j];
            }
        }
        __syncthreads();
    }
    if (warp > 0) return;
    const bool v3 = a.variant == TRTX_YOLO_V3;
    unsigned flags = 0;
#pragma unroll
    for (int j = 0; j < VEC; ++j)
#pragma unroll
        for (int k = 0; k < 3; ++k)
            if (s_obj[k][lane * VEC + j] >= 0.0f && !(v3 && s_fp[k][lane * VEC + j] < a.gate)) flags |= 1u << (j * 3 + k);
    int total;
    int off = warp_excl_scan(__popc(flags), lane, &total);
    if (lane == 0) a.tile_count[(size_t)b * a.tiles_per_image + t] = total;
    if (flags) {
        const size_t slot0 = (size_t)b * a.slots_per_image + L.slot_begin + (size_t)tile * TILE * 3;
#pragma unroll
        for (int j = 0; j < VEC; ++j) {
#pragma unroll
            for (int k = 0; k < 3; ++k) {
                if (flags & (1u << (j * 3 + k))) {
                    const int e = a0 + j;
                    const int row = e / L.gw, col = e - row * L.gw;
                    const T* ck = base + (size_t)k * ilen * g + e;
                    if (v3) {
                        const float fs = (float)L.stride;
                        const float bx = ((float)col + logist(Elem<T>::ld1_cached(ck))) * fs;
                        const float by = ((float)row + logist(Elem<T>::ld1_cached(ck + g))) * fs;
                        const float bw = expf(Elem<T>::ld1_cached(ck + 2 * g)) * L.anc[2 * k];
                        const float bh = expf(Elem<T>::ld1_cached(ck + 3 * g)) * L.anc[2 * k + 1];
                        store_record(a.cand, slot0 + off, bx, by, bw, bh, s_obj[k][lane * VEC + j], s_fc[k][lane * VEC + j],
                                     L.slot_begin + e * 3 + k, s_fp[k][lane * VEC + j]);
                        ++off;
                        continue;
                    }
                    float t0 = logist(Elem<T>::ld1_cached(ck));
                    float t1 = logist(Elem<T>::ld1_cached(ck + g));
                    float t2 = logist(Elem<T>::ld1_cached(ck + 2 * g));
                    float t3 = logist(Elem<T>::ld1_cached(ck + 3 * g));
                    float cx = ((float)col - 0.5f + 2.0f * t0) * (float)a.net_w / (float)L.gw;
                    float cy = ((float)row - 0.5f + 2.0f * t1) * (float)a.net_h / (float)L.gh;
                    float w = 2.0f * t2;
                    w = w * w * L.anc[2 * k];
                    float h = 2.0f * t3;
                    h = h * h * L.anc[2 * k + 1];
                    float conf = s_obj[k][lane * VEC + j] * s_fp[k][lane * VEC + j];
                    store_record(a.cand, slot0 + off, cx, cy, w, h, conf, s_fc[k][lane * VEC + j],
                                 L.slot_begin + e * 3 + k);
                    ++off;
                }
            }
        }
    }
}

template <int VEC>
__global__ void __launch_bounds__(128) yolo26_gather_kernel(const __grid_constant__ YoloArgs a, int batch, int warps_per_cta) {
    extern __shared__ float s_rows[];
    const int lane = threadIdx.x & 31, warp = threadIdx.x >> 5;
    const int gw = blockIdx.x * warps_per_cta + warp;
    if (warp >= warps_per_cta || gw >= batch * a.tiles_per_image) return;
    const int b = gw / a.tiles_per_image, t = gw - b * a.tiles_per_image;
    const LevelArg& L = a.lv[0];
    const int C = a.C, Cp = C | 1;
    float* rows = s_rows + (size_t)warp * 32 * Cp;
    const int a0 = t * 32;
    const int n = min(32, L.g - a0);
    const float* src = static_cast<const float*>(L.in) + ((size_t)b * L.g + a0) * C;
    const int total = n * C;
    if constexpr (VEC == 4) {
        constexpr int U = 7;
        for (int i0 = lane; i0 < total / 4; i0 += 32 * U) {
            float4 v[U];
#pragma unroll
            for (int u = 0; u < U; ++u)
                if (i0 + 32 * u < total / 4) v[u] = ldg_stream_f4(src + 4 * (size_t)(i0 + 32 * u));
#pragma unroll
            for (int u = 0; u < U; ++u) {
                const int e = 4 * (i0 + 32 * u);
                if (e < total) {
                    const int r = e / C, c = e - r * C;
                    float* q = rows + r * Cp + c;
                    q[0] = v[u].x;
                    q[1] = v[u].y;
                    q[2] = v[u].z;
                    q[3] = v[u].w;
                }
            }
        }
    } else {
        for (int e = lane; e < total; e += 32) {
            const int r = e / C, c = e - r * C;
            rows[r * Cp + c] = ldg_stream_f1(src + e);
        }
    }
    __syncwarp();
    float score = 0.0f;
    int cls = -1;
    const float* mine = rows + lane * Cp;
    if (lane < n) {
        for (int c = 0; c < a.nc; ++c) {
            const float conf = mine[4 + c];
            if (conf > score) {
                score = conf;
                cls = c;
            }
        }
    }
    const bool keep = lane < n && !(score < a.gate);
    const unsigned bal = __ballot_sync(0xffffffffu, keep);
    if (lane == 0) a.tile_count[(size_t)b * a.tiles_per_image + t] = __popc(bal);
    if (keep) {
        const size_t slot = (size_t)b * a.slots_per_image + a0 + __popc(bal & ((1u << lane) - 1u));
        store_record(a.cand, slot, mine[0], mine[1], mine[2], mine[3], score, cls, a0 + lane, a.is_obb ? mine[4 + a.nc] : 0.0f);
    }
}

template <typename T>
__device__ void write_extras_v8(const YoloArgs& a, int b, int anchor_id, float* det) {
    int l = 0;
    while (l + 1 < a.num_levels && anchor_id >= a.lv[l + 1].slot_begin) ++l;
    const LevelArg& L = a.lv[l];
    const int e = anchor_id - L.slot_begin;
    const size_t g = (size_t)L.g;
    const T* cur = reinterpret_cast<const T*>(L.in) + (size_t)b * a.C * g + e;
    const int row = e / L.gw, col = e - row * L.gw;
    const int nc = a.nc, nk = a.num_kpts;
    if (a.is_seg) {
        for (int k = 0; k < 32; ++k)
            det[6 + k] = Elem<T>::ld1_cached(cur + (size_t)(4 + nc + (a.is_pose ? nk * 3 : 0) + (a.is_obb ? 1 : 0) + k) * g);
    }
    if (a.is_pose) {
        float* kp = det + 6 + 32;
        for (int k = 0; k < nk; ++k) {
            const size_t base = (size_t)(4 + nc + (a.is_seg ? 32 : 0) + (a.is_obb ? 1 : 0) + k * 3);
            float kc = logist(Elem<T>::ld1_cached(cur + (base + 2) * g));
            float kx = (float)(((double)Elem<T>::ld1_cached(cur + base * g) * 2.0 + col) * L.stride);
            float ky = (float)(((double)Elem<T>::ld1_cached(cur + (base + 1) * g) * 2.0 + row) * L.stride);
            bool inside = kx >= det[0] && kx <= det[2] && ky >= det[1] && ky <= det[3];
            if (kc < a.kpt_thresh || !inside) {
                kp[k * 3] = -1;
                kp[k * 3 + 1] = -1;
                kp[k * 3 + 2] = -1;
            } else {
                kp[k * 3] = kx;
                kp[k * 3 + 1] = ky;
                kp[k * 3 + 2] = kc;
            }
        }
    }
    if (a.is_obb) {
        const double pi = 3.14159265358979323846;
        float d0 = Elem<T>::ld1_cached(cur), d1 = Elem<T>::ld1_cached(cur + g);
        float d2 = Elem<T>::ld1_cached(cur + 2 * g), d3 = Elem<T>::ld1_cached(cur + 3 * g);
        float ain = Elem<T>::ld1_cached(cur + (size_t)(4 + nc + (a.is_seg ? 32 : 0) + (a.is_pose ? nk * 3 : 0)) * g);
        double angle = (double)(logist(ain) - 0.25f) * pi;
        double cos1 = cos(angle), sin1 = sin(angle);
        float xf = (d2 - d0) / 2;
        float yf = (d3 - d1) / 2;
        double x = xf * cos1 - yf * sin1;
        double y = xf * sin1 + yf * cos1;
        det[0] = (float)(((double)((float)col + 0.5f) + x) * L.stride);
        det[1] = (float)(((double)((float)row + 0.5f) + y) * L.stride);
        det[2] = (d0 + d2) * L.stride;
        det[3] = (d1 + d3) * L.stride;
        det[a.det_floats - 1] = (float)angle;
    }
}

template <typename T>
__device__ void write_extras_v5(const YoloArgs& a, int b, int anchor_id, float* det) {
    if (!a.is_seg) return;
    int l = 0;
    while (l + 1 < a.num_levels && anchor_id >= a.lv[l + 1].slot_begin) ++l;
    const LevelArg& L = a.lv[l];
    const int local = anchor_id - L.slot_begin;
    const int e = local / 3, k = local - e * 3;
    const size_t g = (size_t)L.g;
    const T* ck = reinterpret_cast<const T*>(L.in) + (size_t)b * a.C * g + (size_t)k * a.info_len * g + e;
    for (int i = 0; i < 32; ++i) det[6 + i] = Elem<T>::ld1_cached(ck + (size_t)(i + 5 + a.nc) * g);
}

template <typename T>
__global__ void __launch_bounds__(256) yolo_pack_rows_kernel(const __grid_constant__ YoloArgs a, float* __restrict__ out) {
    extern __shared__ int s_prefix[];
    const int b = blockIdx.x;
    const int T_ = a.tiles_per_image;
    const int lane = threadIdx.x & 31, warp = threadIdx.x >> 5, nwarps = blockDim.x >> 5;
    const int* cnt = a.tile_count + (size_t)b * T_;
    if (warp == 0) {
        int carry = 0;
        for (int base = 0; base < T_; base += 32) {
            int v = (base + lane < T_) ? cnt[base + lane] : 0;
            int tot;
            int ex = warp_excl_scan(v, lane, &tot);
            if (base + lane < T_) s_prefix[base + lane] = carry + ex;
            carry += tot;
        }
        if (lane == 0) s_prefix[T_] = carry;
    }
    __syncthreads();
    const int total = s_prefix[T_];
    const int out_elem = 1 + a.max_out * a.det_floats;
    float* o = out + (size_t)b * out_elem;
    if (threadIdx.x == 0) o[0] = (float)min(total, a.max_out);
    if (a.variant == TRTX_YOLO_V26)
        for (int i = min(total, a.max_out) * a.det_floats + threadIdx.x; i < a.max_out * a.det_floats; i += blockDim.x) o[1 + i] = 0.0f;
    const int tile_slots = a.tile_cells * a.apc;
    for (int t = warp; t < T_; t += nwarps) {
        const int n = s_prefix[t + 1] - s_prefix[t];
        if (n == 0) continue;
        int l = 0;
        while (l + 1 < a.num_levels && t >= a.lv[l + 1].tile_begin) ++l;
        const size_t slot0 =
                (size_t)b * a.slots_per_image + a.lv[l].slot_begin + (size_t)(t - a.lv[l].tile_begin) * tile_slots;
        for (int j = lane; j < n; j += 32) {
            const int rank = s_prefix[t] + j;
            if (rank >= a.max_out) continue;
            float4 r0 = a.cand[2 * (slot0 + j)];
            float4 r1 = a.cand[2 * (slot0 + j) + 1];
            float* det = o + 1 + (size_t)rank * a.det_floats;
            det[0] = r0.x;
            det[1] = r0.y;
            det[2] = r0.z;
            det[3] = r0.w;
            det[4] = r1.x;
            det[5] = r1.y;
            const int anchor_id = __float_as_int(r1.z);
            if (a.variant == TRTX_YOLO_V8) {
                if (a.is_seg | a.is_pose | a.is_obb) write_extras_v8<T>(a, b, anchor_id, det);
            } else if (a.variant == TRTX_YOLO_V5) {
                write_extras_v5<T>(a, b, anchor_id, det);
            } else if (a.variant == TRTX_YOLO_V3) {
                det[6] = r1.w;
            } else {
                for (int f = 6; f < a.det_floats; ++f) det[f] = 0.0f;
                if (a.is_obb) det[a.det_floats - 1] = r1.w;
            }
        }
    }
}

int yolo_pick_vec(const trtx_yolo_params* p, const void* const* inputs_dev) {
    if (p->in_dtype == TRTX_F16 && p->variant == TRTX_YOLO_V8) {
        bool ok8 = true;
        for (int l = 0; l < p->num_levels && ok8; ++l)
            ok8 = (p->grid_h[l] * p->grid_w[l]) % 8 == 0 && !(inputs_dev && reinterpret_cast<uintptr_t>(inputs_dev[l]) % 16 != 0);
        if (ok8) return 8;
    }
    const size_t need = (p->in_dtype == TRTX_F16) ? 8 : 16;
    for (int l = 0; l < p->num_levels; ++l) {
        int g = p->grid_h[l] * p->grid_w[l];
        if (g % 4 != 0) return 1;
        if (inputs_dev && (reinterpret_cast<uintptr_t>(inputs_dev[l]) % need) != 0) return 1;
    }
    return 4;
}

static int validate(const trtx_yolo_params* p, int batch) {
    if (!p || batch <= 0) return TRTX_ERR_INVALID;
    if (p->variant < TRTX_YOLO_V8 || p->variant > TRTX_YOLO_V26) return TRTX_ERR_INVALID;
    if (p->num_levels <= 0 || p->num_levels > TRTX_MAX_LEVELS) return TRTX_ERR_INVALID;
    if (p->num_classes <= 0 || p->max_out <= 0 || p->det_floats < 6) return TRTX_ERR_INVALID;
    if (p->in_dtype != TRTX_F32 && p->in_dtype != TRTX_F16) return TRTX_ERR_INVALID;
    for (int l = 0; l < p->num_levels; ++l)
        if (p->grid_h[l] <= 0 || p->grid_w[l] <= 0) return TRTX_ERR_INVALID;
    if (p->variant == TRTX_YOLO_V8) {
        int need = 6 + (p->is_seg || p->is_pose || p->is_obb ? 32 : 0);
        if (p->is_pose) need = 6 + 32 + p->num_kpts * 3;
        if (p->is_obb) need = (need > 7 ? need : 7);
        if (p->det_floats < need) return TRTX_ERR_INVALID;
        if (p->is_pose && p->num_kpts <= 0) return TRTX_ERR_INVALID;
    } else if (p->variant == TRTX_YOLO_V5) {
        if (p->is_seg && p->det_floats < 38) return TRTX_ERR_INVALID;
        if (p->is_pose || p->is_obb) return TRTX_ERR_UNSUPPORTED;
    } else if (p->variant == TRTX_YOLO_V3) {
        if (p->det_floats < 7) return TRTX_ERR_INVALID;
        if (p->is_seg || p->is_pose || p->is_obb) return TRTX_ERR_UNSUPPORTED;
        for (int l = 0; l < p->num_levels; ++l)
            if (p->strides[l] <= 0) return TRTX_ERR_INVALID;
    } else {
        if (p->num_levels != 1 || p->in_dtype != TRTX_F32) return TRTX_ERR_UNSUPPORTED;
        if (p->is_seg || p->is_pose) return TRTX_ERR_UNSUPPORTED;
        if (p->is_obb && p->det_floats < 7) return TRTX_ERR_INVALID;
    }
    return TRTX_OK;
}

int yolo_fill_args(const trtx_yolo_params* p, int batch, const void* const* inputs_dev, void* workspace_dev,
                   size_t workspace_bytes, YoloArgs* a, YoloLayout* Lo) {
    int rc = validate(p, batch);
    if (rc) return rc;
    if (!inputs_dev || !workspace_dev) return TRTX_ERR_INVALID;
    for (int l = 0; l < p->num_levels; ++l)
        if (!inputs_dev[l]) return TRTX_ERR_INVALID;
    const int vec = p->variant == TRTX_YOLO_V26 ? 1 : yolo_pick_vec(p, inputs_dev);
    if (p->tune_class_slices < 0 || p->tune_rows_in_flight < 0 || p->tune_tma_stages < 0 || p->tune_box_prefetch < 0 ||
        p->tune_box_prefetch > 3 || (p->tune_tma_pipeline != 0 && p->tune_tma_pipeline != 1))
        return TRTX_ERR_INVALID;
    const bool pipe = p->tune_tma_pipeline && p->variant == TRTX_YOLO_V8 && vec >= 4 && yolo_pipe_supported(p, inputs_dev);
    YoloLayout L = yolo_layout(p, batch, pipe ? 1 : vec);
    L.pipe = pipe ? 1 : 0;
    L.slices = p->tune_class_slices ? p->tune_class_slices : 2;
    L.unroll = p->tune_rows_in_flight ? p->tune_rows_in_flight : (vec == 8 ? 10 : 5);
    L.pipe_stages = p->tune_tma_stages;
    if (workspace_bytes < L.total_bytes) return TRTX_ERR_WORKSPACE;
    if (reinterpret_cast<uintptr_t>(workspace_dev) % 16 != 0) return TRTX_ERR_INVALID;
    memset(a, 0, sizeof(*a));
    for (int l = 0; l < p->num_levels; ++l) {
        LevelArg& v = a->lv[l];
        v.in = inputs_dev[l];
        v.gh = p->grid_h[l];
        v.gw = p->grid_w[l];
        v.g = v.gh * v.gw;
        v.stride = p->strides[l];
        v.tile_begin = L.level_tile_begin[l];
        v.slot_begin = L.level_slot_begin[l];
        for (int i = 0; i < 6; ++i) v.anc[i] = p->anchors[l][i];
    }
    a->num_levels = p->num_levels;
    a->variant = p->variant;
    a->tiles_per_image = L.tiles_per_image;
    a->slots_per_image = L.slots_per_image;
    a->tile_cells = L.tile_cells;
    a->apc = L.apc;
    a->nc = p->num_classes;
    if (p->variant == TRTX_YOLO_V8) {
        a->info_len = 4 + p->num_classes + (p->is_seg ? 32 : 0) + (p->is_pose ? p->num_kpts * 3 : 0) + (p->is_obb ? 1 : 0);
        a->C = a->info_len;
    } else if (p->variant == TRTX_YOLO_V26) {
        a->info_len = 4 + p->num_classes + (p->is_obb ? 1 : 0);
        a->C = a->info_len;
    } else if (p->variant == TRTX_YOLO_V3) {
        a->info_len = 5 + p->num_classes;
        a->C = 3 * a->info_len;
    } else {
        a->info_len = 5 + p->num_classes + (p->is_seg ? 32 : 0);
        a->C = 3 * a->info_len;
    }
    a->net_w = p->net_w;
    a->net_h = p->net_h;
    a->max_out = p->max_out;
    a->det_floats = p->det_floats;
    a->is_seg = p->is_seg;
    a->is_pose = p->is_pose;
    a->is_obb = p->is_obb;
    a->num_kpts = p->num_kpts;
    a->kpt_thresh = p->kpt_thresh;
    a->gate = p->gate;
    if (p->gate <= 0.0f)
        a->x_lo = -INFINITY;
    else if (p->gate >= 1.0f)
        a->x_lo = 10.0f;
    else
        a->x_lo = logf(p->gate / (1.0f - p->gate)) - 0.05f;
    a->prefetch_box = p->tune_box_prefetch ? p->tune_box_prefetch : 2;
    a->tile_count = reinterpret_cast<int*>(static_cast<char*>(workspace_dev) + L.off_tile_count);
    a->cand = reinterpret_cast<float4*>(static_cast<char*>(workspace_dev) + L.off_cand);
    *Lo = L;
    return TRTX_OK;
}

template <typename T, int VEC>
static int launch_v8(const YoloArgs& a, const YoloLayout& L, int grid, cudaStream_t st) {
#define TRTX_V8_CASE(S, UU)                                                        \
    if (L.slices == S && L.unroll == UU) {                                         \
        yolo_v8_scan_kernel<T, VEC, S, UU><<<grid, 32 * S, 0, st>>>(a);            \
        return TRTX_OK;                                                            \
    }
    TRTX_V8_CASE(1, 8)
    TRTX_V8_CASE(1, 16)
    TRTX_V8_CASE(2, 4)
    TRTX_V8_CASE(2, 5)
    TRTX_V8_CASE(2, 8)
    TRTX_V8_CASE(2, 10)
    TRTX_V8_CASE(2, 20)
    TRTX_V8_CASE(4, 4)
    TRTX_V8_CASE(4, 5)
    TRTX_V8_CASE(4, 10)
    TRTX_V8_CASE(4, 20)
    TRTX_V8_CASE(8, 5)
    TRTX_V8_CASE(8, 10)
#undef TRTX_V8_CASE
    return TRTX_ERR_UNSUPPORTED;
}

int yolo_scan_launch(const YoloArgs& a, const YoloLayout& L, int in_dtype, int batch, cudaStream_t st) {
    const int grid = batch * L.tiles_per_image;
    if (L.pipe) {
        const int rc = yolo_scan_pipe_launch(a, L, in_dtype, batch, st);
        if (rc != TRTX_ERR_UNSUPPORTED) return rc;
    }
    if (a.variant == TRTX_YOLO_V26) {
        const int Cp = a.C | 1;
        int wpc = 4;
        while (wpc > 1 && (size_t)wpc * 32 * Cp * sizeof(float) > 200 * 1024) wpc >>= 1;
        const size_t smem = (size_t)wpc * 32 * Cp * sizeof(float);
        if (smem > 200 * 1024) return TRTX_ERR_UNSUPPORTED;
        const bool v4 = a.C % 4 == 0 && reinterpret_cast<uintptr_t>(a.lv[0].in) % 16 == 0;
        auto kern = v4 ? yolo26_gather_kernel<4> : yolo26_gather_kernel<1>;
        if (smem > 48 * 1024) cudaFuncSetAttribute(kern, cudaFuncAttributeMaxDynamicSharedMemorySize, (int)smem);
        kern<<<(grid + wpc - 1) / wpc, 128, smem, st>>>(a, batch, wpc);
    } else if (a.variant == TRTX_YOLO_V8) {
        int rc;
        if (in_dtype == TRTX_F32)
            rc = L.vec == 4 ? launch_v8<float, 4>(a, L, grid, st) : launch_v8<float, 1>(a, L, grid, st);
        else
            rc = L.vec == 8 ? launch_v8<__half, 8>(a, L, grid, st)
                            : (L.vec == 4 ? launch_v8<__half, 4>(a, L, grid, st) : launch_v8<__half, 1>(a, L, grid, st));
        if (rc) return rc;
    } else {
        if (in_dtype == TRTX_F32) {
            if (L.vec == 4)
                yolo_v5_scan_kernel<float, 4, 10><<<grid, 128, 0, st>>>(a);
            else
                yolo_v5_scan_kernel<float, 1, 10><<<grid, 128, 0, st>>>(a);
        } else {
            if (L.vec == 4)
                yolo_v5_scan_kernel<__half, 4, 10><<<grid, 128, 0, st>>>(a);
            else
                yolo_v5_scan_kernel<__half, 1, 10><<<grid, 128, 0, st>>>(a);
        }
    }
    return check_launch();
}

}

using namespace trtx;

extern "C" {

TRTX_API const char* trtx_version(void) { return "trtx_hot 0.1 (sm_100a)"; }
TRTX_API int trtx_last_cuda_error(void) { return g_last_cuda_error; }
TRTX_API size_t trtx_abi_sizeof(int which) {
    switch (which) {
        case 0: return sizeof(trtx_yolo_params);
        case 1: return sizeof(trtx_nms_params);
        case 2: return sizeof(trtx_retina_params);
        case 3: return sizeof(trtx_image_desc);
        case 4: return sizeof(trtx_mask_params);
        default: return 0;
    }
}

TRTX_API int trtx_yolo_params_init_v8(trtx_yolo_params* p, int num_classes, int net_w, int net_h, int max_out,
                                      const int* strides, int num_levels) {
    if (!p || !strides || num_levels <= 0 || num_levels > TRTX_MAX_LEVELS) return TRTX_ERR_INVALID;
    memset(p, 0, sizeof(*p));
    p->variant = TRTX_YOLO_V8;
    p->num_classes = num_classes;
    p->net_w = net_w;
    p->net_h = net_h;
    p->max_out = max_out;
    p->det_floats = 90;
    p->num_levels = num_levels;
    for (int i = 0; i < num_levels; ++i) {
        if (strides[i] <= 0) return TRTX_ERR_INVALID;
        p->strides[i] = strides[i];
        p->grid_h[i] = net_h / strides[i];
        p->grid_w[i] = net_w / strides[i];
    }
    p->num_kpts = 17;
    p->gate = 0.1f;
    p->in_dtype = TRTX_F32;
    return TRTX_OK;
}

TRTX_API size_t trtx_yolo_workspace_size(const trtx_yolo_params* p, int batch) {
    if (validate(p, batch)) return 0;
    return yolo_layout(p, batch, 1).total_bytes;
}

TRTX_API int trtx_yolo_decode_enqueue(const trtx_yolo_params* p, int batch, const void* const* inputs_dev,
                                      float* output_dev, void* workspace_dev, size_t workspace_bytes,
                                      trtx_stream_t stream) {
    if (!output_dev) return TRTX_ERR_INVALID;
    YoloArgs a;
    YoloLayout L;
    int rc = yolo_fill_args(p, batch, inputs_dev, workspace_dev, workspace_bytes, &a, &L);
    if (rc) return rc;
    cudaStream_t st = static_cast<cudaStream_t>(stream);
    rc = yolo_scan_launch(a, L, p->in_dtype, batch, st);
    if (rc) return rc;
    const size_t smem = sizeof(int) * (size_t)(L.tiles_per_image + 1);
    if (smem > 200 * 1024) return TRTX_ERR_UNSUPPORTED;
    if (p->in_dtype == TRTX_F32) {
        if (smem > 48 * 1024)
            cudaFuncSetAttribute(yolo_pack_rows_kernel<float>, cudaFuncAttributeMaxDynamicSharedMemorySize, (int)smem);
        yolo_pack_rows_kernel<float><<<batch, 256, smem, st>>>(a, output_dev);
    } else {
        if (smem > 48 * 1024)
            cudaFuncSetAttribute(yolo_pack_rows_kernel<__half>, cudaFuncAttributeMaxDynamicSharedMemorySize, (int)smem);
        yolo_pack_rows_kernel<__half><<<batch, 256, smem, st>>>(a, output_dev);
    }
    return check_launch();
}

}
```

tensorrtx_b200/csrc/yolo_layout.cuh:

```cuda
#pragma once
#include "common.cuh"

namespace trtx {

struct LevelArg {
    const void* in;
    int g;
    int gw;
    int gh;
    int stride;
    int tile_begin;
    int slot_begin;
    float anc[6];
};

struct YoloArgs {
    LevelArg lv[TRTX_MAX_LEVELS];
    int num_levels;
    int variant;
    int tiles_per_image;
    int slots_per_image;
    int tile_cells;
    int apc;
    int C;
    int info_len;
    int nc;
    int net_w, net_h;
    int max_out, det_floats;
    int is_seg, is_pose, is_obb, num_kpts;
    float kpt_thresh;
    float gate;
    float x_lo;
    int prefetch_box;
    int* tile_count;
    float4* cand;
};

struct YoloLayout {
    int vec;
    int pipe;
    int slices, unroll, pipe_stages;
    int tile_cells;
    int apc;
    int tiles_per_image;
    int slots_per_image;
    int level_tile_begin[TRTX_MAX_LEVELS];
    int level_slot_begin[TRTX_MAX_LEVELS];
    size_t off_tile_count;
    size_t off_cand;
    size_t off_list;
    size_t total_bytes;
};

inline YoloLayout yolo_layout(const trtx_yolo_params* p, int batch, int vec) {
    YoloLayout L{};
    L.vec = vec;
    L.tile_cells = 32 * vec;
    L.apc = (p->variant == TRTX_YOLO_V5 || p->variant == TRTX_YOLO_V3) ? 3 : 1;
    int tiles = 0, slots = 0;
    for (int l = 0; l < p->num_levels; ++l) {
        int g = p->grid_h[l] * p->grid_w[l];
        L.level_tile_begin[l] = tiles;
        L.level_slot_begin[l] = slots;
        tiles += (g + L.tile_cells - 1) / L.tile_cells;
        slots += g * L.apc;
    }
    L.tiles_per_image = tiles;
    L.slots_per_image = slots;
    L.off_tile_count = 0;
    L.off_cand = align_up(sizeof(int) * (size_t)batch * tiles);
    L.off_list = L.off_cand + align_up(sizeof(float4) * 2 * (size_t)batch * slots);
    L.total_bytes = L.off_list + align_up(sizeof(uint2) * (size_t)batch * slots);
    return L;
}

template <int VEC>
struct Best {
    float bx[VEC];
    float b2[VEC];
    int bc[VEC];
};

template <int VEC>
__device__ __forceinline__ void update_one(Best<VEC>& s, int j, float x, int cls) {
    const bool up = x > s.bx[j];
    s.b2[j] = up ? s.bx[j] : s.b2[j];
    s.bc[j] = up ? cls : s.bc[j];
    s.bx[j] = up ? x : s.bx[j];
}

template <int VEC>
__device__ __forceinline__ void merge_one(Best<VEC>& s, int j, float m, float m2, int c) {
    if (m > s.bx[j]) {
        s.b2[j] = fmaxf(s.bx[j], m2);
        s.bx[j] = m;
        s.bc[j] = c;
    }
}

template <typename LoadRow>
__device__ __forceinline__ float finish_best(float bx, float b2, int& cls, float gate, LoadRow ld) {
    const float P = logist(bx), P2 = logist(b2);
    if (P < gate) return P;
    if (P == 0.0f) {
        cls = 0;
        return P;
    }
    if (P2 == P) {
        for (int i = 0; i < cls; ++i) {
            if (logist(ld(i)) == P) {
                cls = i;
                break;
            }
        }
    }
    return P;
}

__device__ __forceinline__ void store_record(float4* cand, size_t slot, float b0, float b1, float b2, float b3,
                                             float conf, int cls, int anchor_id, float spare = 0.0f) {
    cand[2 * slot] = make_float4(b0, b1, b2, b3);
    cand[2 * slot + 1] = make_float4(conf, (float)cls, __int_as_float(anchor_id), spare);
}

int yolo_pick_vec(const trtx_yolo_params* p, const void* const* inputs_dev);
int yolo_fill_args(const trtx_yolo_params* p, int batch, const void* const* inputs_dev, void* workspace_dev,
                   size_t workspace_bytes, YoloArgs* a, YoloLayout* L);
int yolo_scan_launch(const YoloArgs& a, const YoloLayout& L, int in_dtype, int batch, cudaStream_t stream);
int yolo_scan_pipe_launch(const YoloArgs& a, const YoloLayout& L, int in_dtype, int batch, cudaStream_t stream);
bool yolo_pipe_supported(const trtx_yolo_params* p, const void* const* inputs_dev);

}
```

tensorrtx_b200/csrc/yolo_scan_pipe.cu:

```cuda
#include "tma.cuh"
#include "yolo_layout.cuh"

namespace trtx {

constexpr int kTileAnchors = 64;
constexpr int kMaxStages = 15;

struct alignas(64) TmaMaps {
    CUtensorMap m[TRTX_MAX_LEVELS];
};
template <typename T>
__device__ __forceinline__ float4 lds4(const T* p);
template <>
__device__ __forceinline__ float4 lds4<float>(const float* p) {
    return *reinterpret_cast<const float4*>(p);
}
template <>
__device__ __forceinline__ float4 lds4<__half>(const __half* p) {
    const uint2 u = *reinterpret_cast<const uint2*>(p);
    const float2 a = __half22float2(*reinterpret_cast<const __half2*>(&u.x));
    const float2 b = __half22float2(*reinterpret_cast<const __half2*>(&u.y));
    return make_float4(a.x, a.y, b.x, b.y);
}

constexpr int kSubWarps = kTileAnchors / 32;

struct PipeGeom {
    int stile_begin[TRTX_MAX_LEVELS];
    int stiles_per_image;
};

template <typename T>
__device__ __forceinline__ float lds1(const T* p);
template <>
__device__ __forceinline__ float lds1<float>(const float* p) {
    return *p;
}
template <>
__device__ __forceinline__ float lds1<__half>(const __half* p) {
    return __half2float(*p);
}

template <typename T>
__global__ void __launch_bounds__(1024, 1)
        yolo_v8_scan_pipe_kernel(const __grid_constant__ YoloArgs a, const __grid_constant__ TmaMaps maps,
                                 const __grid_constant__ PipeGeom geo, int total_stiles, int stages, int stage_bytes) {
    extern __shared__ __align__(128) unsigned char smem[];
    unsigned char* stage_base = smem;
    uint64_t* full_bar = reinterpret_cast<uint64_t*>(smem + (size_t)stages * stage_bytes);
    uint64_t* empty_bar = full_bar + kMaxStages;

    const int lane = threadIdx.x & 31;
    const int warp = threadIdx.x >> 5;
    if (threadIdx.x == 0) {
        for (int s = 0; s < stages; ++s) {
            mbar_init(&full_bar[s], 1);
            mbar_init(&empty_bar[s], kSubWarps);
        }
        mbar_fence_init();
    }
    __syncthreads();

    if (warp == stages * kSubWarps) {
        if (lane == 0) {
            int it = 0;
            for (int Tg = blockIdx.x; Tg < total_stiles; Tg += gridDim.x, ++it) {
                const int s = it % stages;
                const uint32_t ph = (uint32_t)(it / stages) & 1u;
                mbar_wait(&empty_bar[s], ph ^ 1u);
                const int b = Tg / geo.stiles_per_image, t = Tg - b * geo.stiles_per_image;
                int l = 0;
                while (l + 1 < a.num_levels && t >= geo.stile_begin[l + 1]) ++l;
                const int col0 = (t - geo.stile_begin[l]) * kTileAnchors;
                unsigned char* dst = stage_base + (size_t)s * stage_bytes;
                mbar_arrive_expect_tx(&full_bar[s], (uint32_t)stage_bytes);
                for (int ch = 0; ch < a.C; ch += 256)
                    tma_load_3d(dst + (size_t)ch * kTileAnchors * sizeof(T), &maps.m[l], col0, ch, b, &full_bar[s]);
            }
        }
        return;
    }

    const int s = warp / kSubWarps;
    const int sub = warp - s * kSubWarps;
    const T* tile = reinterpret_cast<const T*>(stage_base + (size_t)s * stage_bytes) + sub * 32 + lane;
    int it = s;
    for (int Tg = blockIdx.x + s * gridDim.x; Tg < total_stiles; Tg += stages * gridDim.x, it += stages) {
        const uint32_t ph = (uint32_t)(it / stages) & 1u;
        const int b = Tg / geo.stiles_per_image, t = Tg - b * geo.stiles_per_image;
        int l = 0;
        while (l + 1 < a.num_levels && t >= geo.stile_begin[l + 1]) ++l;
        const LevelArg& L = a.lv[l];
        const int cell0 = (t - geo.stile_begin[l]) * kTileAnchors + sub * 32;
        const int e = cell0 + lane;
        const bool active = e < L.g;

        mbar_wait(&full_bar[s], ph);
        Best<1> st;
        st.bx[0] = active ? a.x_lo : INFINITY;
        st.b2[0] = st.bx[0];
        st.bc[0] = 0;
        if (cell0 < L.g) {
            const T* p = tile + (size_t)4 * kTileAnchors;
            constexpr int U = 10;
            int c = 0;
            for (; c + U <= a.nc; c += U, p += U * kTileAnchors) {
                float v[U];
#pragma unroll
                for (int u = 0; u < U; ++u) v[u] = lds1<T>(p + u * kTileAnchors);
                float m = v[0];
#pragma unroll
                for (int u = 1; u < U; ++u) m = fmaxf(m, v[u]);
                if (m > st.bx[0]) {
#pragma unroll
                    for (int u = 0; u < U; ++u) update_one<1>(st, 0, v[u], c + u);
                }
            }
            for (; c < a.nc; ++c, p += kTileAnchors) update_one<1>(st, 0, lds1<T>(p), c);
            float bp = 0.0f;
            if (active && st.bx[0] > a.x_lo)
                bp = finish_best(st.bx[0], st.b2[0], st.bc[0], a.gate,
                                 [&](int i) { return lds1<T>(tile + (size_t)(4 + i) * kTileAnchors); });
            const bool keep = active && !(bp < a.gate);
            const unsigned bal = __ballot_sync(0xffffffffu, keep);
            if (lane == 0) a.tile_count[(size_t)b * a.tiles_per_image + L.tile_begin + (cell0 >> 5)] = __popc(bal);
            if (keep) {
                const float d0 = lds1<T>(tile + 0 * kTileAnchors), d1 = lds1<T>(tile + 1 * kTileAnchors);
                const float d2 = lds1<T>(tile + 2 * kTileAnchors), d3 = lds1<T>(tile + 3 * kTileAnchors);
                const int row = e / L.gw, col = e - row * L.gw;
                const float fs = (float)L.stride;
                const float x1 = ((float)col + 0.5f - d0) * fs;
                const float y1 = ((float)row + 0.5f - d1) * fs;
                const float x2 = ((float)col + 0.5f + d2) * fs;
                const float y2 = ((float)row + 0.5f + d3) * fs;
                const size_t slot = (size_t)b * a.slots_per_image + L.slot_begin + cell0 + __popc(bal & ((1u << lane) - 1u));
                store_record(a.cand, slot, x1, y1, x2, y2, bp, st.bc[0], L.slot_begin + e);
            }
        }
        __syncwarp();
        if (lane == 0) mbar_arrive(&empty_bar[s]);
    }
}


template <typename T>
static int launch_pipe(const YoloArgs& a, const YoloLayout& L, int batch, cudaStream_t st) {
    EncodeTiledFn enc = tma_encoder();
    if (!enc) return TRTX_ERR_UNSUPPORTED;
    int dev = 0, sms = 0, max_smem = 0;
    cudaGetDevice(&dev);
    cudaDeviceGetAttribute(&sms, cudaDevAttrMultiProcessorCount, dev);
    cudaDeviceGetAttribute(&max_smem, cudaDevAttrMaxSharedMemoryPerBlockOptin, dev);
    const int stage_bytes = a.C * kTileAnchors * (int)sizeof(T);
    const int fixed = 2 * kMaxStages * (int)sizeof(uint64_t);
    int stages = L.pipe_stages >= 2 && L.pipe_stages < kMaxStages ? L.pipe_stages : kMaxStages;
    if (stages * kSubWarps + 1 > 32) stages = 31 / kSubWarps;
    while (stages >= 2 && (size_t)stages * stage_bytes + fixed + 128 > (size_t)max_smem) --stages;
    if (stages < 2) return TRTX_ERR_UNSUPPORTED;
    const size_t smem = (size_t)stages * stage_bytes + fixed;
    TmaMaps maps;
    memset(&maps, 0, sizeof(maps));
    for (int l = 0; l < a.num_levels; ++l) {
        const cuuint64_t gdim[3] = {(cuuint64_t)a.lv[l].g, (cuuint64_t)a.C, (cuuint64_t)batch};
        const cuuint64_t gstr[2] = {(cuuint64_t)a.lv[l].g * sizeof(T), (cuuint64_t)a.C * a.lv[l].g * sizeof(T)};
        const cuuint32_t box[3] = {(cuuint32_t)kTileAnchors, (cuuint32_t)(a.C < 256 ? a.C : 256), 1u};
        const cuuint32_t estr[3] = {1u, 1u, 1u};
        const CUresult r = enc(&maps.m[l], sizeof(T) == 4 ? CU_TENSOR_MAP_DATA_TYPE_FLOAT32 : CU_TENSOR_MAP_DATA_TYPE_FLOAT16, 3,
                               const_cast<void*>(a.lv[l].in), gdim, gstr, box, estr, CU_TENSOR_MAP_INTERLEAVE_NONE,
                               CU_TENSOR_MAP_SWIZZLE_NONE, CU_TENSOR_MAP_L2_PROMOTION_L2_256B, CU_TENSOR_MAP_FLOAT_OOB_FILL_NONE);
        if (r != CUDA_SUCCESS) return TRTX_ERR_UNSUPPORTED;
    }
    PipeGeom geo;
    memset(&geo, 0, sizeof(geo));
    for (int l = 0; l < a.num_levels; ++l) {
        geo.stile_begin[l] = geo.stiles_per_image;
        geo.stiles_per_image += (a.lv[l].g + kTileAnchors - 1) / kTileAnchors;
    }
    const int total_stiles = batch * geo.stiles_per_image;
    const int grid = total_stiles < sms ? total_stiles : sms;
    auto kern = yolo_v8_scan_pipe_kernel<T>;
    cudaFuncSetAttribute(kern, cudaFuncAttributeMaxDynamicSharedMemorySize, (int)smem);
    kern<<<grid, 32 * (stages * kSubWarps + 1), smem, st>>>(a, maps, geo, total_stiles, stages, stage_bytes);
    return check_launch();
}

bool yolo_pipe_supported(const trtx_yolo_params* p, const void* const* inputs_dev) {
    if (p->variant != TRTX_YOLO_V8) return false;
    const int C = 4 + p->num_classes + (p->is_seg ? 32 : 0) + (p->is_pose ? p->num_kpts * 3 : 0) + (p->is_obb ? 1 : 0);
    if (C > 256 && (C % 256) != 0) return false;
    for (int l = 0; l < p->num_levels; ++l) {
        const int g = p->grid_h[l] * p->grid_w[l];
        if (inputs_dev && reinterpret_cast<uintptr_t>(inputs_dev[l]) % 16 != 0) return false;
        if (g % (p->in_dtype == TRTX_F16 ? 8 : 4) != 0) return false;
    }
    return tma_encoder() != nullptr;
}

int yolo_scan_pipe_launch(const YoloArgs& a, const YoloLayout& L, int in_dtype, int batch, cudaStream_t st) {
    if (a.variant != TRTX_YOLO_V8 || !L.pipe || L.tile_cells != 32) return TRTX_ERR_UNSUPPORTED;
    if (in_dtype == TRTX_F32) return launch_pipe<float>(a, L, batch, st);
    return launch_pipe<__half>(a, L, batch, st);
}

}
```

tensorrtx_b200/plugins.py:

```python
from __future__ import annotations

import ctypes as C
import math
import struct
from typing import Sequence

import torch

from . import _lib as L


def _ptr(t) -> int:
    if isinstance(t, torch.Tensor):
        if not t.is_cuda:
            raise L.TrtxError("expected a CUDA tensor (device pointer); host buffers are not accepted here")
        if not t.is_contiguous():
            raise L.TrtxError("tensor must be contiguous (TensorFormat::kLINEAR)")
        return t.data_ptr()
    return int(t)


def _stream(stream=None) -> int:
    if stream is None:
        return torch.cuda.current_stream().cuda_stream
    if isinstance(stream, torch.cuda.Stream):
        return stream.cuda_stream
    return int(stream)


def _tune(params, slices: int = 0, rows: int = 0, tma: int = 0, stages: int = 0, box: int = 0) -> None:
    params.tune_class_slices, params.tune_rows_in_flight = int(slices), int(rows)
    params.tune_tma_pipeline, params.tune_tma_stages, params.tune_box_prefetch = int(tma), int(stages), int(box)


def float_le_threshold(x: float) -> float:
    t = struct.unpack("f", struct.pack("f", x))[0]
    if t > x:
        t = float(torch.nextafter(torch.tensor(t, dtype=torch.float32), torch.tensor(-math.inf)).item())
    return t


class YoloLayerPlugin:
    PLUGIN_TYPE = "YoloLayer_TRT"
    PLUGIN_VERSION = "1"
    DET_FLOATS = 90

    def __init__(self, classCount: int, numberofpoints: int, confthreshkeypoints: float, netWidth: int,
                 netHeight: int, maxOut: int, is_segmentation: bool, is_pose: bool, is_obb: bool,
                 strides: Sequence[int], in_dtype: int = L.F32):
        self.mClassCount = int(classCount)
        self.mNumberofpoints = int(numberofpoints)
        self.mConfthreshkeypoints = float(confthreshkeypoints)
        self.mYoloV8NetWidth = int(netWidth)
        self.mYoloV8netHeight = int(netHeight)
        self.mMaxOutObject = int(maxOut)
        self.is_segmentation_ = bool(is_segmentation)
        self.is_pose_ = bool(is_pose)
        self.is_obb_ = bool(is_obb)
        self.mStrides = [int(s) for s in strides]
        self.mThreadCount = 256
        self.mPluginNamespace = ""
        self.in_dtype = in_dtype
        self._lib = L.load()
        p = L.YoloParams()
        arr = (C.c_int * len(self.mStrides))(*self.mStrides)
        L.check(self._lib.trtx_yolo_params_init_v8(C.byref(p), self.mClassCount, self.mYoloV8NetWidth,
                                                  self.mYoloV8netHeight, self.mMaxOutObject, arr, len(self.mStrides)),
                "trtx_yolo_params_init_v8")
        p.det_floats = self.DET_FLOATS
        p.is_seg, p.is_pose, p.is_obb = int(self.is_segmentation_), int(self.is_pose_), int(self.is_obb_)
        p.num_kpts = self.mNumberofpoints
        p.kpt_thresh = self.mConfthreshkeypoints
        p.gate = 0.1
        p.in_dtype = in_dtype
        self.params = p

    def tune(self, **kw) -> "YoloLayerPlugin":
        _tune(self.params, **kw)
        return self

    def getNbOutputs(self) -> int:
        return 1

    def getOutputDimensions(self, index=0, inputs=None, nbInputDims=0):
        total = self.mMaxOutObject * self.DET_FLOATS
        return (total + 1, 1, 1)

    def output_elems(self) -> int:
        return 1 + self.mMaxOutObject * self.DET_FLOATS

    def initialize(self) -> int:
        return 0

    def terminate(self) -> None:
        pass

    def getWorkspaceSize(self, maxBatchSize: int) -> int:
        return int(self._lib.trtx_yolo_workspace_size(C.byref(self.params), int(maxBatchSize)))

    def enqueue(self, batchSize: int, inputs, outputs, workspace, stream=None) -> int:
        ptrs = L.ptr_array([_ptr(t) for t in inputs])
        ws_bytes = workspace.numel() * workspace.element_size() if isinstance(workspace, torch.Tensor) else self.getWorkspaceSize(batchSize)
        return int(self._lib.trtx_yolo_decode_enqueue(C.byref(self.params), int(batchSize), ptrs, _ptr(outputs[0]),
                                                      _ptr(workspace), ws_bytes, _stream(stream)))

    def supportsFormatCombination(self, pos, inOut, nbInputs, nbOutputs) -> bool:
        fmt, dtype = inOut[pos]
        if pos < nbInputs:
            return fmt == "kLINEAR" and dtype in (("kFLOAT",) if self.in_dtype == L.F32 else ("kHALF",))
        return fmt == "kLINEAR" and dtype == "kFLOAT"

    def getPluginType(self) -> str:
        return self.PLUGIN_TYPE

    def getPluginVersion(self) -> str:
        return self.PLUGIN_VERSION

    def getOutputDataType(self, index, inputTypes, nbInputs) -> str:
        return "kFLOAT"

    def setPluginNamespace(self, ns: str) -> None:
        self.mPluginNamespace = ns

    def getPluginNamespace(self) -> str:
        return self.mPluginNamespace

    def destroy(self) -> None:
        pass

    def clone(self) -> "YoloLayerPlugin":
        p = YoloLayerPlugin(self.mClassCount, self.mNumberofpoints, self.mConfthreshkeypoints, self.mYoloV8NetWidth,
                            self.mYoloV8netHeight, self.mMaxOutObject, self.is_segmentation_, self.is_pose_,
                            self.is_obb_, self.mStrides, self.in_dtype)
        p.setPluginNamespace(self.mPluginNamespace)
        return p

    def getSerializationSize(self) -> int:
        return 4 * 8 + 4 * len(self.mStrides) + 3

    def serialize(self) -> bytes:
        d = struct.pack("<iifiiiii", self.mClassCount, self.mNumberofpoints, self.mConfthreshkeypoints,
                        self.mThreadCount, self.mYoloV8NetWidth, self.mYoloV8netHeight, self.mMaxOutObject,
                        len(self.mStrides))
        d += struct.pack(f"<{len(self.mStrides)}i", *self.mStrides)
        d += struct.pack("<???", self.is_segmentation_, self.is_pose_, self.is_obb_)
        assert len(d) == self.getSerializationSize()
        return d

    @classmethod
    def deserialize(cls, data: bytes) -> "YoloLayerPlugin":
        cc, nk, kt, tc, w, h, mo, ns = struct.unpack_from("<iifiiiii", data, 0)
        strides = struct.unpack_from(f"<{ns}i", data, 32)
        seg, pose, obb = struct.unpack_from("<???", data, 32 + 4 * ns)
        if 32 + 4 * ns + 3 != len(data):
            raise L.TrtxError("YoloLayerPlugin.deserialize: length mismatch")
        p = cls(cc, nk, kt, w, h, mo, seg, pose, obb, strides)
        p.mThreadCount = tc
        return p


class YoloPluginCreator:

    def __init__(self):
        self.mNamespace = ""

    def getPluginName(self) -> str:
        return "YoloLayer_TRT"

    def getPluginVersion(self) -> str:
        return "1"

    def getFieldNames(self):
        return []

    def setPluginNamespace(self, ns: str) -> None:
        self.mNamespace = ns

    def getPluginNamespace(self) -> str:
        return self.mNamespace

    def createPlugin(self, name: str, fc: dict) -> YoloLayerPlugin:
        if len(fc) != 1 or "combinedInfo" not in fc:
            raise L.TrtxError("YoloPluginCreator.createPlugin expects exactly one field 'combinedInfo'")
        ci = [int(v) for v in fc["combinedInfo"]]
        if len(ci) < 10:
            raise L.TrtxError("combinedInfo needs 9 net-info ints + at least one stride")
        obj = YoloLayerPlugin(ci[0], ci[1], float(ci[2]), ci[3], ci[4], ci[5], bool(ci[6]), bool(ci[7]), bool(ci[8]), ci[9:])
        obj.setPluginNamespace(self.mNamespace)
        return obj

    def deserializePlugin(self, name: str, data: bytes) -> YoloLayerPlugin:
        obj = YoloLayerPlugin.deserialize(data)
        obj.setPluginNamespace(self.mNamespace)
        return obj


class YoloKernel:

    def __init__(self, width: int, height: int, anchors: Sequence[float]):
        self.width, self.height = int(width), int(height)
        self.anchors = [float(a) for a in anchors]
        assert len(self.anchors) == 6


class YoloLayerPluginV5:
    PLUGIN_TYPE = "YoloLayer_TRT"
    PLUGIN_VERSION = "1"
    DET_FLOATS = 38

    def __init__(self, classCount: int, netWidth: int, netHeight: int, maxOut: int, is_segmentation: bool,
                 vYoloKernel: Sequence[YoloKernel], in_dtype: int = L.F32):
        self.mClassCount, self.mYoloV5NetWidth, self.mYoloV5NetHeight = int(classCount), int(netWidth), int(netHeight)
        self.mMaxOutObject = int(maxOut)
        self.is_segmentation_ = bool(is_segmentation)
        self.mYoloKernel = list(vYoloKernel)
        self.mKernelCount = len(self.mYoloKernel)
        self.mThreadCount = 256
        self.mPluginNamespace = ""
        self._lib = L.load()
        p = L.YoloParams()
        p.variant = L.YOLO_V5
        p.num_classes = self.mClassCount
        p.net_w, p.net_h = self.mYoloV5NetWidth, self.mYoloV5NetHeight
        p.max_out = self.mMaxOutObject
        p.det_floats = self.DET_FLOATS
        p.num_levels = self.mKernelCount
        for i, k in enumerate(self.mYoloKernel):
            p.grid_w[i], p.grid_h[i] = k.width, k.height
            for j in range(6):
                p.anchors[i][j] = k.anchors[j]
        p.is_seg = int(self.is_segmentation_)
        p.gate = 0.1
        p.in_dtype = in_dtype
        self.params = p

    def tune(self, **kw) -> "YoloLayerPlugin":
        _tune(self.params, **kw)
        return self

    def getNbOutputs(self) -> int:
        return 1

    def output_elems(self) -> int:
        return 1 + self.mMaxOutObject * self.DET_FLOATS

    def getOutputDimensions(self, index=0, inputs=None, nbInputDims=0):
        return (self.mMaxOutObject * self.DET_FLOATS + 1, 1, 1)

    def getWorkspaceSize(self, maxBatchSize: int) -> int:
        return int(self._lib.trtx_yolo_workspace_size(C.byref(self.params), int(maxBatchSize)))

    def enqueue(self, batchSize: int, inputs, outputs, workspace, stream=None) -> int:
        ptrs = L.ptr_array([_ptr(t) for t in inputs])
        ws_bytes = workspace.numel() * workspace.element_size()
        return int(self._lib.trtx_yolo_decode_enqueue(C.byref(self.params), int(batchSize), ptrs, _ptr(outputs[0]),
                                                      _ptr(workspace), ws_bytes, _stream(stream)))

    def getPluginType(self) -> str:
        return self.PLUGIN_TYPE

    def getPluginVersion(self) -> str:
        return self.PLUGIN_VERSION

    def clone(self) -> "YoloLayerPluginV5":
        p = YoloLayerPluginV5(self.mClassCount, self.mYoloV5NetWidth, self.mYoloV5NetHeight, self.mMaxOutObject,
                              self.is_segmentation_, self.mYoloKernel, self.params.in_dtype)
        p.mPluginNamespace = self.mPluginNamespace
        return p

    def serialize(self) -> bytes:
        d = struct.pack("<iiiiii?", self.mClassCount, self.mThreadCount, self.mKernelCount, self.mYoloV5NetWidth,
                        self.mYoloV5NetHeight, self.mMaxOutObject, self.is_segmentation_)
        for k in self.mYoloKernel:
            d += struct.pack("<ii6f", k.width, k.height, *k.anchors)
        return d

    def getSerializationSize(self) -> int:
        return 25 + 32 * self.mKernelCount

    @classmethod
    def deserialize(cls, data: bytes) -> "YoloLayerPluginV5":
        cc, tc, kc, w, h, mo, seg = struct.unpack_from("<iiiiii?", data, 0)
        ks = []
        for i in range(kc):
            v = struct.unpack_from("<ii6f", data, 25 + 32 * i)
            ks.append(YoloKernel(v[0], v[1], v[2:]))
        if 25 + 32 * kc != len(data):
            raise L.TrtxError("YoloLayerPluginV5.deserialize: length mismatch")
        p = cls(cc, w, h, mo, seg, ks)
        p.mThreadCount = tc
        return p


class YoloLayerPluginV7(YoloLayerPluginV5):
    DET_FLOATS = 6

    def __init__(self, classCount: int, netWidth: int, netHeight: int, maxOut: int, vYoloKernel: Sequence[YoloKernel],
                 in_dtype: int = L.F32):
        super().__init__(classCount, netWidth, netHeight, maxOut, False, vYoloKernel, in_dtype)

    def clone(self) -> "YoloLayerPluginV7":
        p = YoloLayerPluginV7(self.mClassCount, self.mYoloV5NetWidth, self.mYoloV5NetHeight, self.mMaxOutObject,
                              self.mYoloKernel, self.params.in_dtype)
        p.mPluginNamespace = self.mPluginNamespace
        return p

    def serialize(self) -> bytes:
        d = struct.pack("<iiiiii", self.mClassCount, self.mThreadCount, self.mKernelCount, self.mYoloV5NetWidth,
                        self.mYoloV5NetHeight, self.mMaxOutObject)
        for k in self.mYoloKernel:
            d += struct.pack("<ii6f", k.width, k.height, *k.anchors)
        return d

    def getSerializationSize(self) -> int:
        return 24 + 32 * self.mKernelCount

    @classmethod
    def deserialize(cls, data: bytes) -> "YoloLayerPluginV7":
        cc, tc, kc, w, h, mo = struct.unpack_from("<iiiiii", data, 0)
        if 24 + 32 * kc != len(data):
            raise L.TrtxError("YoloLayerPluginV7.deserialize: length mismatch")
        ks = []
        for i in range(kc):
            v = struct.unpack_from("<ii6f", data, 24 + 32 * i)
            ks.append(YoloKernel(v[0], v[1], v[2:]))
        p = cls(cc, w, h, mo, ks)
        p.mThreadCount = tc
        return p


class YoloKernelV3:

    def __init__(self, width: int, height: int, stride: int, anchors: Sequence[float]):
        self.width, self.height, self.stride = int(width), int(height), int(stride)
        self.anchors = [float(a) for a in anchors]
# ... 565 lines not shown
```

Before: 564,200.

## Add PDL overlap between scan and NMS, optional 512-thread NMS, timeline probes

```diff
diff --git a/include/trtx_hot.h b/include/trtx_hot.h
--- a/include/trtx_hot.h
+++ b/include/trtx_hot.h
@@ -62,6 +62,7 @@
     int32_t tune_tma_pipeline;
     int32_t tune_tma_stages;
     int32_t tune_box_prefetch;
+    int32_t tune_nms_threads;
 } trtx_yolo_params;
 
 TRTX_API int trtx_yolo_params_init_v8(trtx_yolo_params* p, int num_classes, int net_w, int net_h, int max_out,
diff --git a/tensorrtx_b200/_lib.py b/tensorrtx_b200/_lib.py
--- a/tensorrtx_b200/_lib.py
+++ b/tensorrtx_b200/_lib.py
@@ -46,6 +46,7 @@
         ("tune_tma_pipeline", C.c_int32),
         ("tune_tma_stages", C.c_int32),
         ("tune_box_prefetch", C.c_int32),
+        ("tune_nms_threads", C.c_int32),
     ]
 
 
diff --git a/tensorrtx_b200/csrc/common.cuh b/tensorrtx_b200/csrc/common.cuh
--- a/tensorrtx_b200/csrc/common.cuh
+++ b/tensorrtx_b200/csrc/common.cuh
@@ -11,6 +11,44 @@
 constexpr size_t kAlign = 256;
 
 __host__ __device__ inline size_t align_up(size_t v, size_t a = kAlign) { return (v + a - 1) / a * a; }
+
+#ifdef TRTX_NMS_PROBE
+enum TlKind { kTlScan = 1, kTlNms = 2, kTlLetterbox = 3 };
+constexpr int kTlMaxCtas = 8192;
+constexpr size_t kTlRecordWords = 2 + 2 * (size_t)kTlMaxCtas;
+unsigned long long* tl_take();
+__device__ __forceinline__ unsigned long long tl_now() {
+    unsigned long long t;
+    asm volatile("mov.u64 %0, %%globaltimer;" : "=l"(t));
+    return t;
+}
+struct TlStamp {
+    unsigned long long* r;
+    __device__ __forceinline__ TlStamp(unsigned long long* rec, int kind) : r(nullptr) {
+        const unsigned ncta = gridDim.x * gridDim.y * gridDim.z;
+        if (!rec || ncta > (unsigned)kTlMaxCtas) return;
+        const unsigned cta = blockIdx.x + gridDim.x * (blockIdx.y + gridDim.y * blockIdx.z);
+        r = rec + 2 + 2 * (size_t)cta;
+        if (threadIdx.x + threadIdx.y + threadIdx.z == 0) {
+            r[0] = tl_now();
+            if (cta == 0) {
+                rec[0] = (unsigned long long)kind;
+                rec[1] = ncta;
+            }
+        }
+    }
+    __device__ __forceinline__ ~TlStamp() {
+        if (r && (threadIdx.x & 31) == (unsigned)(__ffs(__activemask()) - 1)) atomicMax(r + 1, tl_now());
+    }
+};
+#define TRTX_TL_FIELD unsigned long long* tl;
+#define TRTX_TL(args, kind) TlStamp tl_stamp_((args).tl, (kind))
+#define TRTX_TL_TAKE(args) ((args).tl = tl_take())
+#else
+#define TRTX_TL_FIELD
+#define TRTX_TL(args, kind) do { } while (0)
+#define TRTX_TL_TAKE(args) do { } while (0)
+#endif
 
 extern thread_local int g_last_cuda_error;
 inline int check_launch() {
diff --git a/tensorrtx_b200/csrc/nms.cu b/tensorrtx_b200/csrc/nms.cu
--- a/tensorrtx_b200/csrc/nms.cu
+++ b/tensorrtx_b200/csrc/nms.cu
@@ -6,14 +6,20 @@
 
 #ifdef TRTX_NMS_PROBE
 static thread_local long long* t_nms_stamps = nullptr;
+static thread_local unsigned long long* t_tl_buf = nullptr;
+static thread_local int t_tl_records = 0, t_tl_next = 0;
+unsigned long long* tl_take() {
+    if (!t_tl_buf || t_tl_next >= t_tl_records) return nullptr;
+    return t_tl_buf + kTlRecordWords * (size_t)t_tl_next++;
+}
 #define TRTX_STAMP(k) do { if (a.dbg && threadIdx.x == 0) a.dbg[blockIdx.x * 16 + (k)] = clock64(); } while (0)
 #else
 #define TRTX_STAMP(k) do { } while (0)
 #endif
 
 constexpr int kNmsThreads = 1024;
+constexpr int kNmsThreadsHalf = 512;
 constexpr int kMaxSort = TRTX_NMS_MAX_ROWS;
-constexpr int kClassBins = kNmsThreads;
 constexpr int kMaxBucket = 256;
 constexpr int kShortSeg = 96;
 
@@ -38,6 +44,7 @@
 #ifdef TRTX_NMS_PROBE
     long long* dbg;
 #endif
+    TRTX_TL_FIELD
     float* out;
     int32_t* keep_index;
     struct Gather {
@@ -193,7 +200,12 @@
     return G * (m - 1) - 4 * G * (G - 1);
 }
 
-__global__ void __launch_bounds__(kNmsThreads, 1) nms_kernel(const __grid_constant__ NmsArgs a) {
+template <int NT>
+__global__ void __launch_bounds__(NT, kNmsThreads / NT) nms_kernel(const __grid_constant__ NmsArgs a) {
+    constexpr int NW = NT / 32;
+    static_assert(NT % 32 == 0 && NT >= 256 && NT <= 1024, "the 256-bin histograms need >= 256 threads");
+    TRTX_TL(a, kTlNms);
+    asm volatile("griddepcontrol.wait;" ::: "memory");
     extern __shared__ __align__(16) unsigned char smem_raw[];
     const int S = a.pre_topk <= 1024 ? 1024 : kMaxSort;
     float4* u_box = reinterpret_cast<float4*>(smem_raw);
@@ -219,7 +231,7 @@
     unsigned long long* k_lo = k_hi + S;
 
     __shared__ int s_hist[256];
-    __shared__ int s_chist[kClassBins], s_cstart[kClassBins];
+    __shared__ int s_chist[NT], s_cstart[NT];
     __shared__ int s_n, s_need, s_bucket, s_nkept, s_nshort, s_nmed, s_nlong, s_cursor, s_bad, s_nunit;
     __shared__ unsigned s_rem;
     __shared__ unsigned s_sup[32];
@@ -250,7 +262,7 @@
         const int T = a.tiles_per_image;
         const int* cnt = a.tile_count + (size_t)b * T;
         int carry = 0;
-        for (int base = 0; base < T; base += kNmsThreads) {
+        for (int base = 0; base < T; base += NT) {
             const int t = base + tid;
             const int v = t < T ? cnt[t] : 0;
             int tot;
@@ -258,7 +270,7 @@
             if (lane == 0) s_wsum[warp] = tot;
             __syncthreads();
             if (warp == 0) {
-                int w = s_wsum[lane], wt;
+                int w = lane < NW ? s_wsum[lane] : 0, wt;
                 const int wex = warp_excl_scan(w, lane, &wt);
                 s_wsum[lane] = wex;
                 if (lane == 0) s_need = wt;
@@ -271,7 +283,7 @@
         if (tid == 0) s_tpre[T] = carry;
         __syncthreads();
         const int n_in = min(carry, a.pre_topk);
-        for (int r = tid; r < n_in; r += kNmsThreads) {
+        for (int r = tid; r < n_in; r += NT) {
             int lo = 0, hi = T;
             while (hi - lo > 1) {
                 const int mid = (lo + hi) >> 1;
@@ -289,7 +301,7 @@
         const float* img = a.rows + (size_t)b * (1 + (size_t)a.max_rows * a.det_floats);
         int n_in = (int)img[0];
         n_in = max(0, min(n_in, a.max_rows));
-        for (int i = tid; i < n_in; i += kNmsThreads) {
+        for (int i = tid; i < n_in; i += NT) {
             const Row row = fetch_row(a, b, (uint32_t)i);
             if (a.mode == TRTX_NMS_ONESHOT ? row.conf >= a.conf_thresh : row.conf > a.conf_thresh) stash(row, (uint32_t)i);
         }
@@ -306,7 +318,7 @@
             const int shift = 24 - 8 * pass;
             if (tid < 256) s_hist[tid] = 0;
             __syncthreads();
-            for (int i = tid; i < n_valid; i += kNmsThreads) {
+            for (int i = tid; i < n_valid; i += NT) {
                 uint32_t k = list[i].x;
                 if ((k & mask) == prefix) atomicAdd(&s_hist[(k >> shift) & 255], 1);
             }
@@ -330,7 +342,7 @@
             const int shift = 24 - 8 * pass;
             if (tid < 256) s_hist[tid] = 0;
             __syncthreads();
-            for (int i = tid; i < n_valid; i += kNmsThreads) {
+            for (int i = tid; i < n_valid; i += NT) {
                 uint2 e = list[i];
                 if (e.x == key_cut && (e.y & im) == ip) atomicAdd(&s_hist[(e.y >> shift) & 255], 1);
             }
@@ -351,7 +363,7 @@
             s_bad = 0;
         }
         __syncthreads();
-        for (int i = tid; i < n_valid; i += kNmsThreads) {
+        for (int i = tid; i < n_valid; i += NT) {
             const uint2 e = list[i];
             if (e.x > key_cut || (e.x == key_cut && e.y <= id_cut)) {
                 const Row r = fetch_row(a, b, e.y);
@@ -377,14 +389,14 @@
         s_chist[tid] = 0;
         __syncthreads();
         bool big = false;
-        for (int base = 0; base < M; base += kNmsThreads) {
+        for (int base = 0; base < M; base += NT) {
             const int i = base + tid;
             const int c = i < M ? u_cls[i] : -1;
             const unsigned peers = __match_any_sync(0xffffffffu, c);
             const int leader = __ffs(peers) - 1;
             int first = 0;
-            if (c >= kClassBins) big = true;
-            if (lane == leader && c >= 0 && c < kClassBins) first = atomicAdd(&s_chist[c], __popc(peers));
+            if (c >= NT) big = true;
+            if (lane == leader && c >= 0 && c < NT) first = atomicAdd(&s_chist[c], __popc(peers));
             first = __shfl_sync(0xffffffffu, first, leader);
             if (i < M) s_pos[i] = (unsigned short)(first + __popc(peers & ((1u << lane) - 1u)));
         }
@@ -395,20 +407,20 @@
         if (lane == 0) s_wsum[warp] = tot;
         if (!__syncthreads_or(big || h > kMaxBucket ? 1 : 0)) {
             if (warp == 0) {
-                int w = s_wsum[lane], wt;
+                int w = lane < NW ? s_wsum[lane] : 0, wt;
                 const int wex = warp_excl_scan(w, lane, &wt);
                 s_wsum[lane] = wex;
             }
             __syncthreads();
             s_cstart[tid] = s_wsum[warp] + ex;
             __syncthreads();
-            for (int i = tid; i < M; i += kNmsThreads) {
+            for (int i = tid; i < M; i += NT) {
                 const int c = u_cls[i];
                 kb[s_cstart[c] + s_pos[i]] =
                     ((unsigned long long)(uint32_t)c << 48) | ((unsigned long long)(uint32_t)(~float_key(u_conf[i])) << 16) | (uint32_t)i;
             }
             __syncthreads();
-            for (int p = tid; p < M; p += kNmsThreads) {
+            for (int p = tid; p < M; p += NT) {
                 const unsigned long long mk = kb[p];
                 const int c = (int)(mk >> 48);
                 const int s0 = s_cstart[c], m = s_chist[c];
@@ -419,18 +431,18 @@
             }
             __syncthreads();
             bool tie = false;
-            for (int i = tid; i < M; i += kNmsThreads)
+            for (int i = tid; i < M; i += NT)
                 if (i > 0 && (k64[i] >> 16) == (k64[i - 1] >> 16)) tie = true;
             generic = __syncthreads_or(tie ? 1 : 0) != 0;
             bucketed = !generic;
         }
     }
     if (!generic && !bucketed) {
-        for (int i = tid; i < S_eff; i += kNmsThreads)
+        for (int i = tid; i < S_eff; i += NT)
             k64[i] = i < M ? ((unsigned long long)(uint32_t)u_cls[i] << 48) | ((unsigned long long)(uint32_t)(~float_key(u_conf[i])) << 16) | (uint32_t)i
                            : ~0ull;
         __syncthreads();
-        if (S_eff <= kNmsThreads) {
+        if (S_eff <= NT) {
             unsigned long long* ex = reinterpret_cast<unsigned long long*>(s_box);
             unsigned long long mk = tid < S_eff ? k64[tid] : ~0ull;
             int pp = 0;
@@ -438,9 +450,9 @@
                 for (int jj = k >> 1; jj > 0; jj >>= 1) {
                     unsigned long long ok;
                     if (jj >= 32) {
-                        ex[pp * kNmsThreads + tid] = mk;
+                        ex[pp * NT + tid] = mk;
                         __syncthreads();
-                        ok = ex[pp * kNmsThreads + (tid ^ jj)];
+                        ok = ex[pp * NT + (tid ^ jj)];
                         pp ^= 1;
                     } else {
                         ok = __shfl_xor_sync(0xffffffffu, mk, jj);
@@ -455,7 +467,7 @@
         } else {
             for (int k = 2; k <= S_eff; k <<= 1) {
                 for (int jj = k >> 1; jj > 0; jj >>= 1) {
-                    for (int i = tid; i < S_eff; i += kNmsThreads) {
+                    for (int i = tid; i < S_eff; i += NT) {
                         const int ixj = i ^ jj;
                         if (ixj > i) {
                             const unsigned long long x = k64[i], y = k64[ixj];
@@ -470,12 +482,12 @@
             }
         }
         bool tie = false;
-        for (int i = tid; i < M; i += kNmsThreads)
+        for (int i = tid; i < M; i += NT)
             if (i > 0 && (k64[i] >> 16) == (k64[i - 1] >> 16)) tie = true;
         generic = __syncthreads_or(tie ? 1 : 0) != 0;
     }
     if (generic) {
-        for (int i = tid; i < S_eff; i += kNmsThreads) {
+        for (int i = tid; i < S_eff; i += NT) {
             if (i < M) {
                 k_hi[i] = ((unsigned long long)(uint32_t)u_cls[i] << 32) | (uint32_t)(~float_key(u_conf[i]));
                 k_lo[i] = ((unsigned long long)(a.tie_break_x0 ? float_key(u_box[i].x) : 0u) << 32) | u_id[i];
@@ -488,7 +500,7 @@
         __syncthreads();
         for (int k = 2; k <= S_eff; k <<= 1) {
             for (int jj = k >> 1; jj > 0; jj >>= 1) {
-                for (int i = tid; i < S_eff; i += kNmsThreads) {
+                for (int i = tid; i < S_eff; i += NT) {
                     const int ixj = i ^ jj;
                     if (ixj > i) {
                         const unsigned long long ah = k_hi[i], al = k_lo[i], bh = k_hi[ixj], bl = k_lo[ixj];
@@ -507,7 +519,7 @@
                 __syncthreads();
             }
         }
-        for (int i = tid; i < M; i += kNmsThreads) k64[i] = s_pos[i];
+        for (int i = tid; i < M; i += NT) k64[i] = s_pos[i];
         __syncthreads();
     }
 
@@ -519,7 +531,7 @@
     iq.retina = a.box_format == TRTX_BOX_RETINA;
     iq.zero_hit = 0.0f > a.nms_thresh;
     iq.fast_ok = fabsf(a.nms_thresh) <= 4.0f;
-    for (int i = tid; i < M; i += kNmsThreads) {
+    for (int i = tid; i < M; i += NT) {
         const int pos = (int)(k64[i] & 0xffffull);
         const float4 bx = u_box[pos];
         if (a.box_format == TRTX_BOX_OBB) {
@@ -563,7 +575,7 @@
 
     if (greedy) {
         if (bucketed) {
-            for (int i = tid; i < M; i += kNmsThreads) {
+            for (int i = tid; i < M; i += NT) {
                 const int c = s_cls[i], m = s_chist[c];
                 s_rowseg[i] = m > kShortSeg ? 0 : ((s_cstart[c] << 16) | m);
             }
@@ -576,7 +588,7 @@
                 s_seg[atomicAdd(&s_nshort, 1)] = (p0 << 16) | m;
             if (m > 1 && m <= kShortSeg) s_pos[p0] = (unsigned short)atomicAdd(&s_nunit, seg_units(m));
         } else
-        for (int i = tid; i < M; i += kNmsThreads) {
+        for (int i = tid; i < M; i += NT) {
             if (i == 0 || s_cls[i] != s_cls[i - 1]) {
                 int e = i + 1;
                 while (e < M && s_cls[e] == s_cls[i]) ++e;
@@ -600,14 +612,14 @@
             for (int c0 = 0; c0 < m; c0 += 32) {
                 const int nchunk = min(32, m - c0);
                 const int P = 32 * n_kept;
-                for (int p = tid; p < P; p += kNmsThreads) {
+                for (int p = tid; p < P; p += NT) {
                     const int i = p & 31, k = p >> 5;
                     const int kr = s_krow[k];
                     if (i < nchunk && overlaps(iq, s_box[kr], s_area[kr], s_box[p0 + c0 + i], s_area[p0 + c0 + i]))
                         atomicOr(&s_rem, 1u << i);
                 }
-                {
-                    const int i = warp, jx = lane;
+                for (int i = warp; i < 32; i += NW) {
+                    const int jx = lane;
                     bool hit = false;
                     if (i < nchunk && jx < i)
                         hit = overlaps(iq, s_box[p0 + c0 + jx], s_area[p0 + c0 + jx], s_box[p0 + c0 + i], s_area[p0 + c0 + i]);
@@ -639,7 +651,7 @@
             }
         }
         TRTX_STAMP(4);
-        for (int i = tid; i < M; i += kNmsThreads) {
+        for (int i = tid; i < M; i += NT) {
             const int rs = s_rowseg[i];
             if (rs == 0) continue;
             const int p0 = rs >> 16, m = rs & 0xffff, li = i - p0;
@@ -654,7 +666,7 @@
         {
             const int n_unit = s_nunit;
             unsigned char* mask_bytes = reinterpret_cast<unsigned char*>(s_mask);
-            for (int u = tid; u < n_unit; u += kNmsThreads) {
+            for (int u = tid; u < n_unit; u += NT) {
                 const int e = s_unit[u], i = e >> 4, g = e & 15;
                 const int p0 = s_rowseg[i] >> 16, li = i - p0;
                 const float4 bi = s_box[i];
@@ -707,7 +719,7 @@
         }
         __syncthreads();
     } else {
-        for (int i = tid; i < M; i += kNmsThreads) {
+        for (int i = tid; i < M; i += NT) {
             const int ci = s_cls[i];
             const float4 bi = s_box[i];
             bool keep = true;
@@ -725,14 +737,14 @@
 
     TRTX_STAMP(5);
     int carry = 0;
-    for (int base = 0; base < M; base += kNmsThreads) {
+    for (int base = 0; base < M; base += NT) {
         const int i = base + tid;
         const bool emit = i < M && (a.mode == TRTX_NMS_ONESHOT || s_keep[i]);
         const unsigned bal = __ballot_sync(0xffffffffu, emit);
         if (lane == 0) s_wsum[warp] = __popc(bal);
         __syncthreads();
         if (warp == 0) {
-            int v = s_wsum[lane], tot;
+            int v = lane < NW ? s_wsum[lane] : 0, tot;
             const int ex = warp_excl_scan(v, lane, &tot);
             s_wsum[lane] = ex;
             if (lane == 0) s_nkept = tot;
@@ -764,15 +776,15 @@
     }
     const int n_rows_out = min(carry, a.max_det);
     if (tid == 0) o[0] = (float)n_rows_out;
-    for (int i = n_rows_out * R + tid; i < a.max_det * R; i += kNmsThreads) o[1 + i] = 0.0f;
+    for (int i = n_rows_out * R + tid; i < a.max_det * R; i += NT) o[1 + i] = 0.0f;
     if (oidx)
-        for (int i = n_rows_out + tid; i < a.max_det; i += kNmsThreads) oidx[i] = -1;
+        for (int i = n_rows_out + tid; i < a.max_det; i += NT) oidx[i] = -1;
     if (gworld) {
         __syncthreads();
         const int live = 1 + n_rows_out * R;
         for (int p = 0; p < gworld; ++p) {
             float* dstp = a.g.out[p] + goff;
-            for (int i = tid; i < live; i += kNmsThreads) dstp[i] = i == 0 ? (float)n_rows_out : o[i];
+            for (int i = tid; i < live; i += NT) dstp[i] = i == 0 ? (float)n_rows_out : o[i];
         }
         __syncthreads();
         if (tid == 0) {
@@ -859,16 +871,53 @@
     return TRTX_OK;
 }
 
-static int nms_launch(NmsArgs& a, int batch, cudaStream_t st) {
+static bool nms_half_ok(const NmsArgs& a) {
+    return a.from_tiles && a.mode == TRTX_NMS_GREEDY && a.box_format != TRTX_BOX_OBB && a.pre_topk <= 1024 && a.g.world == 0;
+}
+
+template <int NT>
+static cudaError_t nms_launch_nt(const NmsArgs& a, int batch, size_t smem, cudaStream_t st) {
+    constexpr size_t kMaxDynSmem = (227 - 20) * 1024;
+    cudaFuncSetAttribute(nms_kernel<NT>, cudaFuncAttributeMaxDynamicSharedMemorySize, (int)kMaxDynSmem);
+    cudaLaunchConfig_t cfg{};
+    cfg.gridDim = dim3(batch);
+    cfg.blockDim = dim3(NT);
+    cfg.dynamicSmemBytes = smem;
+    cfg.stream = st;
+    cudaLaunchAttribute at[1];
+    at[0].id = cudaLaunchAttributeProgrammaticStreamSerialization;
+    at[0].val.programmaticStreamSerializationAllowed = 1;
+    cfg.attrs = at;
+    cfg.numAttrs = 1;
+#ifdef TRTX_NMS_NO_PDL
+    cfg.numAttrs = 0;
+#endif
+    cudaError_t e = cudaLaunchKernelEx(&cfg, nms_kernel<NT>, a);
+    if (e == cudaErrorNotSupported || e == cudaErrorInvalidValue) {
+        (void)cudaGetLastError();
+        cfg.numAttrs = 0;
+        e = cudaLaunchKernelEx(&cfg, nms_kernel<NT>, a);
+    }
+    return e;
+}
+
+static int nms_launch(NmsArgs& a, int batch, cudaStream_t st, int threads = 0) {
 #ifdef TRTX_NMS_PROBE
     a.dbg = t_nms_stamps;
 #endif
+    TRTX_TL_TAKE(a);
     if (a.pre_topk > kMaxSort) return TRTX_ERR_UNSUPPORTED;
+    if (threads != 0 && threads != kNmsThreads && threads != kNmsThreadsHalf) return TRTX_ERR_UNSUPPORTED;
+    const bool half = threads == kNmsThreadsHalf;
+    if (half && !nms_half_ok(a)) return TRTX_ERR_UNSUPPORTED;
     const size_t smem = nms_smem_bytes(a.pre_topk, a.from_tiles ? a.tiles_per_image : 0);
-    constexpr size_t kMaxDynSmem = (227 - 20) * 1024;
-    if (smem > kMaxDynSmem) return TRTX_ERR_UNSUPPORTED;
-    cudaFuncSetAttribute(nms_kernel, cudaFuncAttributeMaxDynamicSharedMemorySize, (int)kMaxDynSmem);
-    nms_kernel<<<batch, kNmsThreads, smem, st>>>(a);
+    if (smem > (227 - 20) * 1024) return TRTX_ERR_UNSUPPORTED;
+    const cudaError_t e = half ? nms_launch_nt<kNmsThreadsHalf>(a, batch, smem, st) : nms_launch_nt<kNmsThreads>(a, batch, smem, st);
+    if (e != cudaSuccess) {
+        (void)cudaGetLastError();
+        g_last_cuda_error = (int)e;
+        return TRTX_ERR_CUDA;
+    }
     return check_launch();
 }
 
@@ -883,6 +932,13 @@
     t_nms_stamps = static_cast<long long*>(p);
     return TRTX_OK;
 }
+TRTX_API int trtx_probe_set_timeline(void* p, int records) {
+    t_tl_buf = static_cast<unsigned long long*>(p);
+    t_tl_records = p ? records : 0;
+    t_tl_next = 0;
+    return TRTX_OK;
+}
+TRTX_API size_t trtx_probe_timeline_record_words() { return kTlRecordWords; }
 #endif
 
 TRTX_API size_t trtx_nms_workspace_size(const trtx_nms_params* p, int batch, int max_rows) {
@@ -971,7 +1027,7 @@
     a.keep_index = keep_index_dev;
     const int rc = fill_gather(gather, &a.g);
     if (rc) return rc;
-    return nms_launch(a, batch, st);
+    return nms_launch(a, batch, st, p->tune_nms_threads);
 }
 
 TRTX_API int trtx_yolo_decode_nms_enqueue(const trtx_yolo_params* p, const trtx_nms_params* q, int batch,
diff --git a/tensorrtx_b200/csrc/preprocess.cu b/tensorrtx_b200/csrc/preprocess.cu
--- a/tensorrtx_b200/csrc/preprocess.cu
+++ b/tensorrtx_b200/csrc/preprocess.cu
@@ -17,6 +17,7 @@
 struct PreArgs {
     PreImage img[kMaxImagesPerLaunch];
     int dw, dh;
+    TRTX_TL_FIELD
 };
 
 __device__ __forceinline__ float div255(float x) {
@@ -32,6 +33,7 @@
 
 template <typename OutT>
 __global__ void __launch_bounds__(256, 8) letterbox_kernel(const __grid_constant__ PreArgs a, OutT* __restrict__ dst) {
+    TRTX_TL(a, kTlLetterbox);
     constexpr int R = kRowsPerThread;
     const int b = blockIdx.z;
     const PreImage& im = a.img[b];
@@ -151,10 +153,12 @@
     CUtensorMap map[kMaxUnitImages];
     UnitImage img[kMaxUnitImages];
     int dw, dh;
+    TRTX_TL_FIELD
 };
 
 template <typename OutT, int WARPS>
 __global__ void __launch_bounds__(WARPS * 32) letterbox_unit_kernel(const __grid_constant__ UnitArgs a, OutT* __restrict__ dst) {
+    TRTX_TL(a, kTlLetterbox);
     constexpr int TW = kUnitTW, TH = WARPS * 8, BOXW = kUnitBoxBytes, ROWS = TH + 1;
     __shared__ __align__(128) uint8_t box[ROWS * BOXW];
     __shared__ uint64_t bar;
@@ -308,6 +312,7 @@
         a.img[i] = u[i];
     }
     dim3 grid((dw + kUnitTW - 1) / kUnitTW, (dh + kUnitWarps * 8 - 1) / (kUnitWarps * 8), n);
+    TRTX_TL_TAKE(a);
     if (out_dtype == TRTX_F32)
         letterbox_unit_kernel<float, kUnitWarps><<<grid, kUnitWarps * 32, 0, st>>>(a, static_cast<float*>(dst));
     else
@@ -514,6 +519,7 @@
         constexpr int R = kRowsPerThread;
         dim3 block(128, 2, 1);
         dim3 grid((dst_w + 127) / 128, (dst_h + 2 * R - 1) / (2 * R), ng);
+        TRTX_TL_TAKE(g);
         if (out_dtype == TRTX_F32)
             letterbox_kernel<float><<<grid, block, 0, st>>>(g, static_cast<float*>(dst_dev));
         else
diff --git a/tensorrtx_b200/csrc/yolo_decode.cu b/tensorrtx_b200/csrc/yolo_decode.cu
--- a/tensorrtx_b200/csrc/yolo_decode.cu
+++ b/tensorrtx_b200/csrc/yolo_decode.cu
@@ -126,6 +126,7 @@
 
 template <typename T, int VEC, int SLICES, int U>
 __global__ void __launch_bounds__(32 * SLICES) yolo_v8_scan_kernel(const __grid_constant__ YoloArgs a) {
+    TRTX_TL(a, kTlScan);
     constexpr int TILE = 32 * VEC;
     __shared__ float s_m[SLICES > 1 ? SLICES - 1 : 1][TILE];
     __shared__ float s_m2[SLICES > 1 ? SLICES - 1 : 1][TILE];
@@ -193,6 +194,7 @@
         else
             scan_classes<T, VEC, U>(base + (size_t)(4 + c0) * g + a0, g, c1 - c0, c0, s);
     }
+    asm volatile("griddepcontrol.launch_dependents;");
 
     if constexpr (SLICES > 1) {
         bool mine = false;
@@ -756,7 +758,9 @@
     return TRTX_ERR_UNSUPPORTED;
 }
 
-int yolo_scan_launch(const YoloArgs& a, const YoloLayout& L, int in_dtype, int batch, cudaStream_t st) {
+int yolo_scan_launch(const YoloArgs& a_in, const YoloLayout& L, int in_dtype, int batch, cudaStream_t st) {
+    YoloArgs a = a_in;
+    TRTX_TL_TAKE(a);
     const int grid = batch * L.tiles_per_image;
     if (L.pipe) {
         const int rc = yolo_scan_pipe_launch(a, L, in_dtype, batch, st);
diff --git a/tensorrtx_b200/csrc/yolo_layout.cuh b/tensorrtx_b200/csrc/yolo_layout.cuh
--- a/tensorrtx_b200/csrc/yolo_layout.cuh
+++ b/tensorrtx_b200/csrc/yolo_layout.cuh
@@ -34,6 +34,7 @@
     int prefetch_box;
     int* tile_count;
     float4* cand;
+    TRTX_TL_FIELD
 };
 
 struct YoloLayout {
diff --git a/tensorrtx_b200/csrc/yolo_scan_pipe.cu b/tensorrtx_b200/csrc/yolo_scan_pipe.cu
--- a/tensorrtx_b200/csrc/yolo_scan_pipe.cu
+++ b/tensorrtx_b200/csrc/yolo_scan_pipe.cu
@@ -45,6 +45,7 @@
 __global__ void __launch_bounds__(1024, 1)
         yolo_v8_scan_pipe_kernel(const __grid_constant__ YoloArgs a, const __grid_constant__ TmaMaps maps,
                                  const __grid_constant__ PipeGeom geo, int total_stiles, int stages, int stage_bytes) {
+    TRTX_TL(a, kTlScan);
     extern __shared__ __align__(128) unsigned char smem[];
     unsigned char* stage_base = smem;
     uint64_t* full_bar = reinterpret_cast<uint64_t*>(smem + (size_t)stages * stage_bytes);
@@ -78,6 +79,7 @@
                     tma_load_3d(dst + (size_t)ch * kTileAnchors * sizeof(T), &maps.m[l], col0, ch, b, &full_bar[s]);
             }
         }
+        asm volatile("griddepcontrol.launch_dependents;");
         return;
     }
 
@@ -140,6 +142,7 @@
         __syncwarp();
         if (lane == 0) mbar_arrive(&empty_bar[s]);
     }
+    asm volatile("griddepcontrol.launch_dependents;");
 }
 
 
diff --git a/tensorrtx_b200/plugins.py b/tensorrtx_b200/plugins.py
--- a/tensorrtx_b200/plugins.py
+++ b/tensorrtx_b200/plugins.py
@@ -28,9 +28,10 @@
     return int(stream)
 
 
-def _tune(params, slices: int = 0, rows: int = 0, tma: int = 0, stages: int = 0, box: int = 0) -> None:
+def _tune(params, slices: int = 0, rows: int = 0, tma: int = 0, stages: int = 0, box: int = 0, nms_threads: int = 0) -> None:
     params.tune_class_slices, params.tune_rows_in_flight = int(slices), int(rows)
     params.tune_tma_pipeline, params.tune_tma_stages, params.tune_box_prefetch = int(tma), int(stages), int(box)
+    params.tune_nms_threads = int(nms_threads)
 
 
 def float_le_threshold(x: float) -> float:
```

Result: faster. 605,900 (median of 6 runs) (+7.4%).
